# chsl/PLADE

Hardware: AMD Instinct MI355X
Metric: scan-pair registrations/sec, 1M-pt synthetic pairs (higher is better)
Workload: dtype f32

## Files before the change

### include/plade_hip.h

```cpp
#ifndef PLADE_HIP_H
#define PLADE_HIP_H
#include <stddef.h>
#include <stdint.h>
#ifdef __cplusplus
extern "C" {
#endif

#define PLADE_OK 0
#define PLADE_EINVAL (-1)
#define PLADE_EDEVICE (-2)
#define PLADE_ECAP (-3)
#define PLADE_EFAIL (-4)
#define PLADE_ELIMIT (-5)

#define PLADE_GROUP_MAX 8

typedef struct plade_ctx plade_ctx;
typedef struct plade_cloud plade_cloud;
typedef struct plade_comm plade_comm;

int plade_ctx_create(int device, plade_ctx **out);
void plade_ctx_destroy(plade_ctx *ctx);
const char *plade_last_error(const plade_ctx *ctx);
const char *plade_version(void);
// ... 101 lines not shown
int plade_estimate_normals(plade_ctx *ctx, const float *xyz, uint32_t n, uint32_t stride, int32_t k, const float *viewpoint,
                           float *pos_nrm_out, float *curvature_out, int32_t *nbr_out);
int plade_cloud_upload_xyz(plade_ctx *ctx, const float *xyz, uint32_t n, uint32_t stride, int32_t k, const float *viewpoint,
                           plade_cloud **out);

#define PLADE_ICP_TOO_FEW 1
#define PLADE_ICP_DEGENERATE 2
typedef struct plade_icp_params {
    double source_leaf;
    double max_dist;
    double min_dist;
    double eps_rotation;
    double eps_translation;
    int32_t max_iterations;
    int32_t min_correspondences;
} plade_icp_params;
typedef struct plade_icp_result {
    int32_t iterations;
    int32_t stages;
    int32_t converged;
    int32_t failure;
    uint32_t correspondences;
    uint32_t samples;
    double rmse, fitness;
    double final_dist;
} plade_icp_result;
void plade_icp_default_params(plade_icp_params *p);
int plade_refine_icp(plade_ctx *ctx, const float *tgt_pos_nrm, uint32_t n_t, const float *src_pos_nrm, uint32_t n_s,
                     const float *T_in16, const plade_icp_params *params, float *T_out16, plade_icp_result *result);
int plade_refine_icp_dev(plade_ctx *ctx, plade_cloud *tgt, plade_cloud *src, const float *T_in16, const plade_icp_params *params,
                         float *T_out16, plade_icp_result *result);
int plade_icp_linearize(plade_ctx *ctx, const float *tgt_pos_nrm, uint32_t n_t, const float *src_xyz, uint32_t n_s, uint32_t stride,
                        const double *T16, const double *center, float dist, int32_t *corr_out, double *moments_out);

typedef struct plade_gicp_params {
    double source_leaf;
    double max_dist;
    double min_dist;
    double eps_rotation;
    double eps_translation;
    int32_t max_iterations;
    int32_t min_correspondences;
    double epsilon;
} plade_gicp_params;
typedef struct plade_gicp_result {
    int32_t iterations;
    int32_t stages;
    int32_t converged;
    int32_t failure;
    uint32_t correspondences;
    uint32_t samples;
    double rmse, fitness;
    double final_dist;
    double cost;
} plade_gicp_result;
void plade_gicp_default_params(plade_gicp_params *p);
int plade_refine_gicp(plade_ctx *ctx, const float *tgt_pos_nrm, uint32_t n_t, const float *src_pos_nrm, uint32_t n_s,
                      const float *T_in16, const plade_gicp_params *params, float *T_out16, plade_gicp_result *result);
int plade_refine_gicp_dev(plade_ctx *ctx, plade_cloud *tgt, plade_cloud *src, const float *T_in16, const plade_gicp_params *params,
                          float *T_out16, plade_gicp_result *result);
int plade_gicp_linearize(plade_ctx *ctx, const float *tgt_pos_nrm, uint32_t n_t, const float *src_pos_nrm, uint32_t n_s,
                         const double *T16, const double *center, float dist, double epsilon, int32_t *corr_out, double *moments_out);

typedef struct plade_distance_summary {
    uint64_t n, count, plane_count;
    double fitness, rmse, mean, max, plane_rmse;
} plade_distance_summary;
int plade_cloud_distances(plade_ctx *ctx, const float *tgt_pos_nrm, uint32_t n_t, const float *src_xyz, uint32_t n_s,
                          uint32_t stride, const float *T16, float max_dist, int32_t *idx_out, float *d2_out,
                          float *plane_out, plade_distance_summary *summary);
int plade_cloud_distances_dev(plade_ctx *ctx, plade_cloud *tgt, plade_cloud *src, const float *T16, float max_dist,
                              int32_t *idx_out, float *d2_out, float *plane_out, plade_distance_summary *summary);

#define PLADE_OUTLIER_STATISTICAL 0
#define PLADE_OUTLIER_RADIUS 1
typedef struct plade_outlier_params {
    int32_t mode;
    int32_t k;
    double alpha;
    double radius;
    int32_t min_neighbours;
    int32_t reserved;
} plade_outlier_params;
typedef struct plade_outlier_summary {
    uint64_t n, kept;
    double mu, sigma, threshold;
} plade_outlier_summary;
void plade_outlier_default_params(plade_outlier_params *p);
int plade_filter_outliers(plade_ctx *ctx, const float *rows, uint32_t n, uint32_t stride, const plade_outlier_params *params,
                          uint8_t *keep_out, uint32_t *kept_index_out, float *rows_out, double *mean_dist_out, uint32_t *count_out,
                          plade_outlier_summary *summary);
int plade_cloud_filter_outliers_dev(plade_ctx *ctx, plade_cloud *cloud, const plade_outlier_params *params, plade_cloud **out,
                                    uint8_t *keep_out, uint32_t *kept_index_out, plade_outlier_summary *summary);

typedef struct plade_component_params {
    double radius;
    int32_t min_size;
    int32_t max_size;
    int32_t keep_largest;
    int32_t reserved;
} plade_component_params;
typedef struct plade_component_summary {
    uint64_t n, components, kept_components, kept;
    uint32_t largest;
    uint32_t reserved;
} plade_component_summary;
void plade_component_default_params(plade_component_params *p);
int plade_label_components(plade_ctx *ctx, const float *rows, uint32_t n, uint32_t stride, const plade_component_params *params,
                           int32_t *label_out, uint32_t *size_out, uint8_t *keep_out, uint32_t *kept_index_out, float *rows_out,
                           plade_component_summary *summary);
int plade_cloud_filter_components_dev(plade_ctx *ctx, plade_cloud *cloud, const plade_component_params *params, plade_cloud **out,
                                      int32_t *label_out, uint32_t *kept_index_out, plade_component_summary *summary);

typedef struct plade_smooth_params {
    double radius;
    int32_t min_neighbours;
    float viewpoint[3];
    int32_t reserved;
} plade_smooth_params;
typedef struct plade_smooth_summary {
    uint64_t n, fitted;
    double rms, max;
    uint32_t max_count;
    uint32_t reserved;
} plade_smooth_summary;
void plade_smooth_default_params(plade_smooth_params *p);
int plade_smooth_cloud(plade_ctx *ctx, const float *rows, uint32_t n, uint32_t stride, const plade_smooth_params *params,
                       float *out_xyz, float *out_normal, float *curvature_out, double *displacement_out, uint32_t *count_out,
                       uint8_t *fitted_out, double *moments_out, plade_smooth_summary *summary);
int plade_cloud_smooth_dev(plade_ctx *ctx, plade_cloud *cloud, const plade_smooth_params *params, int32_t use_fit_normals,
                           plade_cloud **out, plade_smooth_summary *summary);

typedef struct plade_merge_summary {
    uint64_t n_in, n_out, n_shared;
    uint32_t max_count;
    uint32_t reserved;
} plade_merge_summary;
int plade_merge_clouds(plade_ctx *ctx, uint32_t k, const float *const *clouds, const uint32_t *n, const float *T ,
                       float leaf, float *out_rows, uint32_t *out_count, uint32_t *out_mask, plade_merge_summary *summary);
int plade_merge_clouds_dev(plade_ctx *ctx, uint32_t k, plade_cloud *const *clouds, const float *T , float leaf,
                           plade_cloud **out, uint32_t *out_count, uint32_t *out_mask, plade_merge_summary *summary);
int plade_cloud_download(plade_ctx *ctx, const plade_cloud *cloud, float *rows, uint32_t capacity_rows, uint32_t *n);

int plade_dump_get(plade_ctx *ctx, const char *name, const void **ptr, int64_t *nbytes);
int plade_stats_get(plade_ctx *ctx, const char **names, const double **values, int32_t *count);
int plade_sort_pairs(plade_ctx *ctx, const void *keys, const uint32_t *vals, uint32_t n, int key_bytes, int bits,
                     void *keys_out, uint32_t *vals_out);
int plade_sort_segments(plade_ctx *ctx, const uint32_t *keys, const uint32_t *vals, const uint32_t *seg_off, uint32_t nseg, int bits,
                        uint32_t *keys_out, uint32_t *vals_out);

int plade_selftest_readback(plade_ctx *ctx, uint32_t n_ranges, uint32_t words, uint32_t *mismatches);

int plade_diag_launches(plade_ctx *ctx, uint32_t count, uint32_t blocks, uint32_t mbytes);
int plade_ply_read(const char *path, float **pos_nrm, uint64_t *n, char *err, size_t err_cap);
int plade_ply_read_points(const char *path, float **pos_nrm, uint64_t *n, int32_t *has_normals, char *err, size_t err_cap);
void plade_ply_free(float *pos_nrm);
int plade_diag_cluster_order(const float *sizes, uint32_t n, int32_t mode, int32_t depth_limit, int32_t *order);
int plade_diag_line_solver_host(int32_t kind, const float *a, const float *b, const float *c, const float *d, uint32_t n,
                                float *o1, float *o2, int32_t *ok);
int plade_kernel_time(plade_ctx *ctx, const char *which, int iters, double *avg_seconds,
                      double *algorithmic_bytes_per_launch);

#ifdef __cplusplus
}
#endif
#endif
```

### plade_amd/__init__.py

```python
import ctypes as C
import os
import numpy as np

_HERE = os.path.dirname(os.path.abspath(__file__))
LIB_PATH = os.path.join(_HERE, "libplade_hip.so")

PLADE_OK = 0
PLADE_EINVAL, PLADE_EDEVICE, PLADE_ECAP, PLADE_EFAIL, PLADE_ELIMIT = -1, -2, -3, -4, -5

ABI_SYMBOLS = [
    "plade_ctx_create", "plade_ctx_destroy", "plade_last_error", "plade_version", "plade_default_params",
    "plade_set_params", "plade_score_planes", "plade_extract_planes", "plade_match_descriptors",
    "plade_overlap_counts", "plade_average_spacing", "plade_voxel_downsample", "plade_registration_planes",
    "plade_registration", "plade_registration_minsupport", "plade_cloud_upload", "plade_cloud_free",
    "plade_registration_dev", "plade_dump_get", "plade_stats_get", "plade_kernel_time", "plade_plane_component",
    "plade_sort_pairs", "plade_host_pin", "plade_host_unpin", "plade_score_planes_subset", "plade_registration_next", "plade_cluster_transforms", "plade_device_synchronize", "plade_selftest_readback",
    "plade_registration_pairs", "plade_registration_pairs_dev", "plade_pair_ctx", "plade_set_candidate_shard", "plade_diag_launches", "plade_diag_cluster_order", "plade_diag_line_solver_host", "plade_sort_segments",
    "plade_closest_points", "plade_lines_meet", "plade_ply_read", "plade_ply_free",
    "plade_device_count", "plade_comm_unique_id", "plade_comm_create", "plade_comm_all_gather", "plade_comm_destroy", "plade_comm_last_error",
    "plade_set_candidate_shard_comm",
    "plade_estimate_normals", "plade_cloud_upload_xyz", "plade_ply_read_points",
    "plade_icp_default_params", "plade_refine_icp", "plade_refine_icp_dev", "plade_icp_linearize",
    "plade_cloud_distances", "plade_cloud_distances_dev",
    "plade_outlier_default_params", "plade_filter_outliers", "plade_cloud_filter_outliers_dev",
    "plade_merge_clouds", "plade_merge_clouds_dev", "plade_cloud_download",
    "plade_component_default_params", "plade_label_components", "plade_cloud_filter_components_dev",
    "plade_smooth_default_params", "plade_smooth_cloud", "plade_cloud_smooth_dev",
    "plade_gicp_default_params", "plade_refine_gicp", "plade_refine_gicp_dev", "plade_gicp_linearize",
]


class PladeError(RuntimeError):
    def __init__(self, code, msg):
        super().__init__(f"libplade_hip error {code}: {msg}")
        self.code = code


class Params(C.Structure):
    _fields_ = [("max_planes", C.c_int32), ("min_planes", C.c_int32), ("max_candidates", C.c_int32),
                ("init_min_support", C.c_int32), ("orient_normals", C.c_int32), ("dump", C.c_int32),
                ("ransac_seed", C.c_uint64), ("host_wait", C.c_int32), ("unoriented_normals", C.c_int32),
                ("ransac_topup", C.c_int32), ("match_window", C.c_int32), ("match_cell_budget", C.c_uint32),
                ("group_max_points", C.c_uint32), ("prepare_sides", C.c_int32), ("closest_point_mode", C.c_int32)]


class IcpParams(C.Structure):
    _fields_ = [("source_leaf", C.c_double), ("max_dist", C.c_double), ("min_dist", C.c_double), ("eps_rotation", C.c_double),
                ("eps_translation", C.c_double), ("max_iterations", C.c_int32), ("min_correspondences", C.c_int32)]


class IcpResult(C.Structure):
    _fields_ = [("iterations", C.c_int32), ("stages", C.c_int32), ("converged", C.c_int32), ("failure", C.c_int32),
                ("correspondences", C.c_uint32), ("samples", C.c_uint32), ("rmse", C.c_double), ("fitness", C.c_double),
                ("final_dist", C.c_double)]


class GicpParams(C.Structure):
    _fields_ = IcpParams._fields_ + [("epsilon", C.c_double)]


class GicpResult(C.Structure):
    _fields_ = IcpResult._fields_ + [("cost", C.c_double)]


class DistanceSummary(C.Structure):
    _fields_ = [("n", C.c_uint64), ("count", C.c_uint64), ("plane_count", C.c_uint64), ("fitness", C.c_double), ("rmse", C.c_double),
                ("mean", C.c_double), ("max", C.c_double), ("plane_rmse", C.c_double)]


class OutlierParams(C.Structure):
    _fields_ = [("mode", C.c_int32), ("k", C.c_int32), ("alpha", C.c_double), ("radius", C.c_double), ("min_neighbours", C.c_int32),
                ("reserved", C.c_int32)]


class OutlierSummary(C.Structure):
    _fields_ = [("n", C.c_uint64), ("kept", C.c_uint64), ("mu", C.c_double), ("sigma", C.c_double), ("threshold", C.c_double)]


class MergeSummary(C.Structure):
    _fields_ = [("n_in", C.c_uint64), ("n_out", C.c_uint64), ("n_shared", C.c_uint64), ("max_count", C.c_uint32),
                ("reserved", C.c_uint32)]


class ComponentParams(C.Structure):
    _fields_ = [("radius", C.c_double), ("min_size", C.c_int32), ("max_size", C.c_int32), ("keep_largest", C.c_int32),
                ("reserved", C.c_int32)]


class ComponentSummary(C.Structure):
    _fields_ = [("n", C.c_uint64), ("components", C.c_uint64), ("kept_components", C.c_uint64), ("kept", C.c_uint64),
                ("largest", C.c_uint32), ("reserved", C.c_uint32)]


class SmoothParams(C.Structure):
    _fields_ = [("radius", C.c_double), ("min_neighbours", C.c_int32), ("viewpoint", C.c_float * 3), ("reserved", C.c_int32)]


class SmoothSummary(C.Structure):
    _fields_ = [("n", C.c_uint64), ("fitted", C.c_uint64), ("rms", C.c_double), ("max", C.c_double), ("max_count", C.c_uint32),
                ("reserved", C.c_uint32)]


PLADE_OUTLIER_STATISTICAL, PLADE_OUTLIER_RADIUS = 0, 1
OUTLIER_MODES = {"statistical": PLADE_OUTLIER_STATISTICAL, "radius": PLADE_OUTLIER_RADIUS}

PLADE_ICP_TOO_FEW, PLADE_ICP_DEGENERATE = 1, 2
ICP_FAILURES = {0: None, PLADE_ICP_TOO_FEW: "too few correspondences", PLADE_ICP_DEGENERATE: "degenerate"}

EXCHANGE_FN = C.CFUNCTYPE(C.c_int, C.c_void_p, C.POINTER(C.c_int32), C.c_uint32, C.c_uint32, C.c_uint32)

_lib = None


def load_library(path=LIB_PATH):
    global _lib
    if _lib is not None:
        return _lib
    if not os.path.exists(path):
        raise FileNotFoundError(f"{path} is missing: build it with `make lib` or __graft_entry__.build(); "
                                "plade_amd has no CPU fallback")
    L = C.CDLL(path)
    p, f, i32, u32, u64 = C.c_void_p, C.c_float, C.c_int32, C.c_uint32, C.c_uint64
    def sig(name, argtypes=None, restype=None):
        fn = getattr(L, name, None)
        if fn is None:
            return
        if argtypes is not None:
            fn.argtypes = argtypes
        if restype is not None:
            fn.restype = restype

    sig("plade_version", restype=C.c_char_p)
    sig("plade_last_error", restype=C.c_char_p)
    sig("plade_last_error", argtypes=[p])
    sig("plade_device_synchronize", argtypes=[C.c_int])
    sig("plade_ctx_create", argtypes=[C.c_int, C.POINTER(p)])
    sig("plade_ctx_destroy", argtypes=[p])
    sig("plade_default_params", argtypes=[C.POINTER(Params)])
    sig("plade_set_params", argtypes=[p, C.POINTER(Params)])
    sig("plade_score_planes", argtypes=[p, p, p, u32, p, u32, f, f, p, p, u32])
    sig("plade_score_planes_subset", argtypes=[p, p, p, u32, p, u32, p, u32, f, f, p, p])
    sig("plade_extract_planes", argtypes=[p, p, u32, u32, f, f, f, f, p, p, p, u32, p])
    sig("plade_match_descriptors", argtypes=[p, p, u32, p, u32, f, p, p, p, u64, p])
    sig("plade_cluster_transforms", argtypes=[p, p, p, u32, f, f, p, p])
    sig("plade_overlap_counts", argtypes=[p, p, u32, p, u32, p, u32, p, f, f, p])
    sig("plade_average_spacing", argtypes=[p, p, u32, u32, u32, u32, p])
    sig("plade_voxel_downsample", argtypes=[p, p, u32, u32, f, p, p])
    sig("plade_registration_planes", argtypes=[p, p, u32, p, u32, p, p, p, u32, p, p, p, u32, p])
    sig("plade_registration", argtypes=[p, p, u32, p, u32, p])
    sig("plade_registration_next", argtypes=[p, p, u32, p, u32, p, u32, p, u32, p])
    sig("plade_registration_pairs", argtypes=[p, u32, p, p, p, p, u32, p, p, p, p, p, p])
    sig("plade_registration_pairs_dev", argtypes=[p, u32, p, p, p, p])
    sig("plade_pair_ctx", argtypes=[p, u32], restype=p)
    sig("plade_closest_points", argtypes=[p, i32, p, p, p, p, u32, p, p, p, p])
    sig("plade_lines_meet", argtypes=[p, i32, p, p, p, p, u32, p, p])
    sig("plade_diag_launches", argtypes=[p, u32, u32, u32])
    sig("plade_diag_cluster_order", argtypes=[p, u32, i32, i32, p])
    sig("plade_diag_line_solver_host", argtypes=[i32, p, p, p, p, u32, p, p, p])
    sig("plade_ply_read", argtypes=[C.c_char_p, C.POINTER(C.POINTER(C.c_float)), C.POINTER(u64), C.c_char_p, C.c_size_t])
    sig("plade_ply_free", argtypes=[C.POINTER(C.c_float)], restype=None)
    sig("plade_ply_read_points", argtypes=[C.c_char_p, C.POINTER(C.POINTER(C.c_float)), C.POINTER(u64), C.POINTER(i32), C.c_char_p,
                                           C.c_size_t])
    sig("plade_estimate_normals", argtypes=[p, p, u32, u32, i32, p, p, p, p])
    sig("plade_cloud_upload_xyz", argtypes=[p, p, u32, u32, i32, p, C.POINTER(p)])
    sig("plade_icp_default_params", argtypes=[C.POINTER(IcpParams)], restype=None)
    sig("plade_refine_icp", argtypes=[p, p, u32, p, u32, p, C.POINTER(IcpParams), p, C.POINTER(IcpResult)])
    sig("plade_refine_icp_dev", argtypes=[p, p, p, p, C.POINTER(IcpParams), p, C.POINTER(IcpResult)])
    sig("plade_icp_linearize", argtypes=[p, p, u32, p, u32, u32, p, p, f, p, p])
    sig("plade_gicp_default_params", argtypes=[C.POINTER(GicpParams)], restype=None)
    sig("plade_refine_gicp", argtypes=[p, p, u32, p, u32, p, C.POINTER(GicpParams), p, C.POINTER(GicpResult)])
    sig("plade_refine_gicp_dev", argtypes=[p, p, p, p, C.POINTER(GicpParams), p, C.POINTER(GicpResult)])
    sig("plade_gicp_linearize", argtypes=[p, p, u32, p, u32, p, p, f, C.c_double, p, p])
    sig("plade_cloud_distances", argtypes=[p, p, u32, p, u32, u32, p, f, p, p, p, C.POINTER(DistanceSummary)])
    sig("plade_cloud_distances_dev", argtypes=[p, p, p, p, f, p, p, p, C.POINTER(DistanceSummary)])
    sig("plade_outlier_default_params", argtypes=[C.POINTER(OutlierParams)], restype=None)
    sig("plade_filter_outliers", argtypes=[p, p, u32, u32, C.POINTER(OutlierParams), p, p, p, p, p, C.POINTER(OutlierSummary)])
    sig("plade_cloud_filter_outliers_dev", argtypes=[p, p, C.POINTER(OutlierParams), C.POINTER(p), p, p, C.POINTER(OutlierSummary)])
    sig("plade_merge_clouds", argtypes=[p, u32, p, p, p, f, p, p, p, C.POINTER(MergeSummary)])
    sig("plade_merge_clouds_dev", argtypes=[p, u32, p, p, f, C.POINTER(p), p, p, C.POINTER(MergeSummary)])
    sig("plade_cloud_download", argtypes=[p, p, p, u32, C.POINTER(u32)])
    sig("plade_component_default_params", argtypes=[C.POINTER(ComponentParams)], restype=None)
    sig("plade_label_components", argtypes=[p, p, u32, u32, C.POINTER(ComponentParams), p, p, p, p, p, C.POINTER(ComponentSummary)])
    sig("plade_cloud_filter_components_dev", argtypes=[p, p, C.POINTER(ComponentParams), C.POINTER(p), p, p, C.POINTER(ComponentSummary)])
    sig("plade_smooth_default_params", argtypes=[C.POINTER(SmoothParams)], restype=None)
    sig("plade_smooth_cloud", argtypes=[p, p, u32, u32, C.POINTER(SmoothParams), p, p, p, p, p, p, p, C.POINTER(SmoothSummary)])
    sig("plade_cloud_smooth_dev", argtypes=[p, p, C.POINTER(SmoothParams), i32, C.POINTER(p), C.POINTER(SmoothSummary)])
    sig("plade_sort_segments", argtypes=[p, p, p, p, u32, C.c_int, p, p])
    sig("plade_set_candidate_shard", argtypes=[p, u32, u32, u32, EXCHANGE_FN, p])
    sig("plade_registration_minsupport", argtypes=[p, p, u32, p, u32, i32, i32, p])
    sig("plade_cloud_upload", argtypes=[p, p, u32, C.POINTER(p)])
    sig("plade_cloud_free", argtypes=[p, p])
    sig("plade_registration_dev", argtypes=[p, p, p, p])
    sig("plade_dump_get", argtypes=[p, C.c_char_p, C.POINTER(p), C.POINTER(C.c_int64)])
    sig("plade_stats_get", argtypes=[p, C.POINTER(C.c_char_p), C.POINTER(C.POINTER(C.c_double)), C.POINTER(i32)])
    sig("plade_kernel_time", argtypes=[p, C.c_char_p, C.c_int, C.POINTER(C.c_double), C.POINTER(C.c_double)])
    sig("plade_plane_component", argtypes=[p, p, u32, p, p, p, u32, f, C.c_int, f, p, p, p, p])
    sig("plade_sort_pairs", argtypes=[p, p, p, u32, C.c_int, C.c_int, p, p])
    sig("plade_selftest_readback", argtypes=[p, u32, u32, C.POINTER(u32)])
    sig("plade_host_pin", argtypes=[p, p, C.c_size_t])
    sig("plade_host_unpin", argtypes=[p, p])
    _lib = L
    return L


def _f32(a):
    return np.ascontiguousarray(a, dtype=np.float32)


def _i32(a):
    return np.ascontiguousarray(a, dtype=np.int32)


def _ptr(a):
    return a.ctypes.data_as(C.c_void_p) if a is not None else None


DUMP_FIELDS = {
    "average_spacing": np.float32, "scale": np.float32,
    "tgt_ds": np.float32, "src_ds": np.float32, "tgt_bcenter": np.float32, "src_bcenter": np.float32,
    "tgt_radius": np.float64, "src_radius": np.float64,
    "tgt_plane_center_radius": np.float32, "src_plane_center_radius": np.float32,
    "tgt_plane_four": np.float32, "src_plane_four": np.float32,
    "tgt_plane_ds_offsets": np.int32, "src_plane_ds_offsets": np.int32,
    "tgt_plane_ds": np.float32, "src_plane_ds": np.float32,
    "tgt_lines": np.float32, "src_lines": np.float32,
    "tgt_desc": np.float32, "src_desc": np.float32,
    "match_offsets": np.int64, "match_nbr": np.int32, "match_dist2": np.float64,
    "initial_RT": np.float32, "cluster_sizes": np.int32, "cluster_seeds": np.int32,
    "plane_match_counts": np.int32, "pen_tested": np.int32, "pen_flags": np.int32,
    "candidates": np.float32, "candidate_centers": np.float32, "overlap_counts": np.int32,
    "scores": np.float32, "best_index": np.int32,
    "tgt_planes": np.float32, "tgt_plane_offsets": np.int32, "tgt_plane_idx": np.int32,
    "src_planes": np.float32, "src_plane_offsets": np.int32, "src_plane_idx": np.int32,
}


def device_synchronize(device=0):
    rc = load_library().plade_device_synchronize(int(device))
    if rc != 0:
        raise PladeError(rc, "plade_device_synchronize failed")


def default_params():
    prm = Params()
    load_library().plade_default_params(C.byref(prm))
    return prm


def icp_default_params():
    prm = IcpParams()
    load_library().plade_icp_default_params(C.byref(prm))
    return {k: getattr(prm, k) for k, _ in IcpParams._fields_}


def outlier_default_params():
    prm = OutlierParams()
    load_library().plade_outlier_default_params(C.byref(prm))
    return {k: getattr(prm, k) for k, _ in OutlierParams._fields_ if k != "reserved"}


def _outlier_params(mode, k, alpha, radius, min_neighbours):
    prm = OutlierParams()
    load_library().plade_outlier_default_params(C.byref(prm))
    if mode not in OUTLIER_MODES:
        raise ValueError(f"mode: 'statistical' or 'radius', got {mode!r}")
    prm.mode = OUTLIER_MODES[mode]
    if k is not None:
        prm.k = int(k)
    if alpha is not None:
        prm.alpha = float(alpha)
    if radius is not None:
        prm.radius = float(radius)
    if min_neighbours is not None:
        prm.min_neighbours = int(min_neighbours)
    return prm


def _outlier_info(summ, keep):
    info = {k: getattr(summ, k) for k, _ in OutlierSummary._fields_}
    info["keep"] = keep.view(np.bool_)
    return info


def component_default_params():
    prm = ComponentParams()
    load_library().plade_component_default_params(C.byref(prm))
    return {k: getattr(prm, k) for k, _ in ComponentParams._fields_ if k != "reserved"}


def _component_params(radius, min_size, max_size, keep_largest):
    prm = ComponentParams()
    load_library().plade_component_default_params(C.byref(prm))
    prm.radius = float(radius)
    prm.min_size, prm.max_size, prm.keep_largest = int(min_size), int(max_size), int(keep_largest)
    return prm


def _component_info(summ, label, size, keep):
    info = {k: getattr(summ, k) for k, _ in ComponentSummary._fields_ if k != "reserved"}
    info["label"] = label
    if size is not None:
        info["size"] = size[:summ.components].copy()
    if keep is not None:
        info["keep"] = keep.view(np.bool_)
    return info


def smooth_default_params():
    prm = SmoothParams()
# ... 267 lines not shown
                                                C.byref(npl)))
        p = npl.value
        return planes[:p].copy(), offs[: p + 1].copy(), idx[: offs[p]].copy()

    def match_descriptors(self, qry, tgt, radius=0.04):
        q = _f32(qry).reshape(-1, 8)
        t = _f32(tgt).reshape(-1, 8)
        off = np.zeros(len(q) + 1, np.int64)
        total = C.c_uint64()
        self._check(self.L.plade_match_descriptors(self.h, _ptr(q), len(q), _ptr(t), len(t), radius, _ptr(off), None,
                                                   None, 0, C.byref(total)))
        m = total.value
        nbr = np.zeros(max(m, 1), np.uint32)
        d2 = np.zeros(max(m, 1), np.float64)
        self._check(self.L.plade_match_descriptors(self.h, _ptr(q), len(q), _ptr(t), len(t), radius, _ptr(off),
                                                   _ptr(nbr), _ptr(d2), m, C.byref(total)))
        return off, nbr[:m].astype(np.int32), d2[:m]

    def cluster_transforms(self, t_xyz, euler, dist_threshold, angle_gate):
        t, e = _f32(t_xyz).reshape(-1, 3), _f32(euler).reshape(-1, 3)
        out = np.full(len(t), -1, np.int32)
        n = C.c_uint32()
        self._check(self.L.plade_cluster_transforms(self.h, _ptr(t), _ptr(e), len(t), dist_threshold, angle_gate, _ptr(out), C.byref(n)))
        return out, n.value

    def overlap_counts(self, src_ds, tgt_ds, T, centers, src_radius, inlier_dist):
        s, t = _f32(src_ds), _f32(tgt_ds)
        T = _f32(T).reshape(-1, 16)
        c = _f32(centers).reshape(-1, 3)
        counts = np.zeros(len(T), np.int32)
        self._check(self.L.plade_overlap_counts(self.h, _ptr(s), len(s), _ptr(t), len(t), _ptr(T), len(T), _ptr(c),
                                                src_radius, inlier_dist, _ptr(counts)))
        return counts

    def average_spacing(self, pts, k=6, samples=10000):
        a = _f32(pts)
        out = C.c_float()
        self._check(self.L.plade_average_spacing(self.h, _ptr(a), len(a), a.shape[1], k, samples, C.byref(out)))
        return np.float32(out.value)

    def voxel_downsample(self, pts, leaf):
        a = _f32(pts)
        out = np.zeros((len(a), 3), np.float32)
        n = C.c_uint32()
        self._check(self.L.plade_voxel_downsample(self.h, _ptr(a), len(a), a.shape[1], leaf, _ptr(out), C.byref(n)))
        return out[: n.value].copy()

    def registration_planes(self, tgt, src, tgt_planes, src_planes):
        tgt, src = _f32(tgt), _f32(src)
        tc, to, ti = _f32(tgt_planes[0]), _i32(tgt_planes[1]), _i32(tgt_planes[2])
        sc, so, si = _f32(src_planes[0]), _i32(src_planes[1]), _i32(src_planes[2])
        T = np.zeros((4, 4), np.float32)
        rc = self._check(self.L.plade_registration_planes(self.h, _ptr(tgt), len(tgt), _ptr(src), len(src), _ptr(tc),
                                                          _ptr(to), _ptr(ti), len(tc), _ptr(sc), _ptr(so), _ptr(si),
                                                          len(sc), _ptr(T)), allow=(PLADE_EFAIL,))
        return rc == 0, T

    def registration(self, tgt, src):
        tgt, src = _f32(tgt), _f32(src)
        self._check_cloud(tgt, "registration"); self._check_cloud(src, "registration")
        T = np.zeros((4, 4), np.float32)
        rc = self._check(self.L.plade_registration(self.h, _ptr(tgt), len(tgt), _ptr(src), len(src), _ptr(T)),
                         allow=(PLADE_EFAIL,))
        return rc == 0, T

    def registration_next(self, tgt, src, next_tgt=None, next_src=None):
        for a in (tgt, src, next_tgt, next_src):
            if a is not None:
                self._check_cloud(a, "registration_next")
        T = np.zeros((4, 4), np.float32)
        nt, ns = (next_tgt, next_src) if next_tgt is not None and next_src is not None else (None, None)
        self._announced = [(nt, ns)] if nt is not None else None
        rc = self._check(self.L.plade_registration_next(self.h, _ptr(tgt), len(tgt), _ptr(src), len(src), _ptr(nt),
                                                        len(nt) if nt is not None else 0, _ptr(ns),
                                                        len(ns) if ns is not None else 0, _ptr(T)), allow=(PLADE_EFAIL,))
        return rc == 0, T

    @staticmethod
    def _cloud_table(arrs):
        ptrs = (C.c_void_p * len(arrs))(*[a.ctypes.data for a in arrs])
        ns = (C.c_uint32 * len(arrs))(*[len(a) for a in arrs])
        return ptrs, ns

    @staticmethod
    def _check_cloud(a, what):
        if not isinstance(a, np.ndarray) or a.dtype != np.float32 or a.ndim != 2 or a.shape[1] != 6 or not a.flags["C_CONTIGUOUS"]:
            raise ValueError(f"{what}: a C-contiguous float32 array of shape (N, 6) is required, got "
                             f"{getattr(a, 'dtype', type(a))} {getattr(a, 'shape', '')}")
        if len(a) == 0:
            raise ValueError(f"{what}: empty cloud")

    def registration_pairs(self, pairs, next_pairs=None, raise_on_error=True):
        if not 1 <= len(pairs) <= 8 or (next_pairs and len(next_pairs) > 8):
            raise ValueError("registration_pairs: a group holds 1..8 pairs")
        for pr in list(pairs) + list(next_pairs or []):
            for a in pr[:2]:
                self._check_cloud(a, "registration_pairs")
        self._announced = [(p[0], p[1]) for p in next_pairs] if next_pairs else None
        k = len(pairs)
        tp, tn = self._cloud_table([p[0] for p in pairs])
        sp, sn = self._cloud_table([p[1] for p in pairs])
        nk = len(next_pairs) if next_pairs else 0
        if nk:
            ntp, ntn = self._cloud_table([p[0] for p in next_pairs])
            nsp, nsn = self._cloud_table([p[1] for p in next_pairs])
        else:
            ntp = ntn = nsp = nsn = None
        T = np.zeros((k, 4, 4), np.float32)
        st = np.zeros(k, np.int32)
        self._check(self.L.plade_registration_pairs(self.h, k, tp, tn, sp, sn, nk, ntp, ntn, nsp, nsn, _ptr(T), _ptr(st)))
        if not raise_on_error:
            return [(int(st[i]), T[i].copy()) for i in range(k)]
        for i in range(k):
            if st[i] not in (0, PLADE_EFAIL):
                raise PladeError(int(st[i]), self.pair_error(i))
        return [(bool(st[i] == 0), T[i].copy()) for i in range(k)]

    def registration_pairs_dev(self, clouds, raise_on_error=True):
        k = len(clouds)
        if not 1 <= k <= 8:
            raise ValueError("registration_pairs_dev: a group holds 1..8 pairs")
        tp = (C.c_void_p * k)(*[c[0].h.value for c in clouds])
        sp = (C.c_void_p * k)(*[c[1].h.value for c in clouds])
        T = np.zeros((k, 4, 4), np.float32)
        st = np.zeros(k, np.int32)
        self._check(self.L.plade_registration_pairs_dev(self.h, k, tp, sp, _ptr(T), _ptr(st)))
        if not raise_on_error:
            return [(int(st[i]), T[i].copy()) for i in range(k)]
        for i in range(k):
            if st[i] not in (0, PLADE_EFAIL):
                raise PladeError(int(st[i]), self.pair_error(i))
        return [(bool(st[i] == 0), T[i].copy()) for i in range(k)]

    def set_candidate_shard(self, rank, world, exchange=None, min_candidates=0):
        if world <= 1 or exchange is None:
            self._shard_cb = None
            self._check(self.L.plade_set_candidate_shard(self.h, 0, 1, 0, EXCHANGE_FN(0), None))
            return

        def cb(user, values, count, r, w):
            try:
                exchange(np.ctypeslib.as_array(values, shape=(count,)), int(r), int(w))
                return 0
            except Exception:
                import traceback
                traceback.print_exc()
                return -1
        self._shard_cb = EXCHANGE_FN(cb)
        self._check(self.L.plade_set_candidate_shard(self.h, int(rank), int(world), int(min_candidates), self._shard_cb, None))

    def diag_launches(self, count, blocks=1, mbytes=0):
        self._check(self.L.plade_diag_launches(self.h, int(count), int(blocks), int(mbytes)))

    def _pair_handle(self, index):
        h = self.L.plade_pair_ctx(self.h, int(index))
        if not h:
            raise PladeError(PLADE_EINVAL, f"no pair {index} on this context")
        return C.c_void_p(h)

    def pair_error(self, index):
        return self.L.plade_last_error(self._pair_handle(index)).decode(errors="replace")

    def registration_minsupport(self, tgt, src, ms_t, ms_s):
        tgt, src = _f32(tgt), _f32(src)
        T = np.zeros((4, 4), np.float32)
        rc = self._check(self.L.plade_registration_minsupport(self.h, _ptr(tgt), len(tgt), _ptr(src), len(src), ms_t,
                                                              ms_s, _ptr(T)), allow=(PLADE_EFAIL,))
        return rc == 0, T

    def upload(self, pos_nrm):
        return Cloud(self, pos_nrm)

    def estimate_normals(self, xyz, k=16, viewpoint=(0.0, 0.0, 0.0), curvature=False, neighbours=False):
        a, n, stride = _xyz_view(xyz)
        v = _viewpoint(viewpoint)
        out = np.empty((n, 6), np.float32)
        curv = np.empty(n, np.float32) if curvature else None
        nbr = np.empty((n, max(int(k), 0)), np.int32) if neighbours else None
        self._check(self.L.plade_estimate_normals(self.h, _ptr(a), n, stride, int(k), _ptr(v), _ptr(out), _ptr(curv), _ptr(nbr)))
        res = (out,) + ((curv,) if curvature else ()) + ((nbr,) if neighbours else ())
        return res[0] if len(res) == 1 else res

    def upload_xyz(self, xyz, k=16, viewpoint=(0.0, 0.0, 0.0)):
        a, n, stride = _xyz_view(xyz)
        v = _viewpoint(viewpoint)
        h = C.c_void_p()
        self._check(self.L.plade_cloud_upload_xyz(self.h, _ptr(a), n, stride, int(k), _ptr(v), C.byref(h)))
        return Cloud(self, None, handle=(n, h))

    def _refine(self, call, T, icp_params):
        T_in = _f32(T).reshape(4, 4).copy()
        prm = _icp_params(icp_params)
        T_out = np.zeros((4, 4), np.float32)
        res = IcpResult()
        rc = call(T_in, prm, T_out, res)
        info = _icp_info(res)
        if rc != 0:
            err = PladeError(rc, self.L.plade_last_error(self.h).decode(errors="replace"))
            err.info, err.T = info, T_out
            raise err
        return T_out, info

    def refine_icp(self, tgt, src, T, **icp_params):
        tgt, src = _f32(tgt), _f32(src)
        self._check_cloud(tgt, "refine_icp"); self._check_cloud(src, "refine_icp")
        return self._refine(lambda T_in, prm, T_out, res: self.L.plade_refine_icp(
            self.h, _ptr(tgt), len(tgt), _ptr(src), len(src), _ptr(T_in), C.byref(prm), _ptr(T_out), C.byref(res)), T, icp_params)

    def refine_icp_dev(self, tgt_cloud, src_cloud, T, **icp_params):
        return self._refine(lambda T_in, prm, T_out, res: self.L.plade_refine_icp_dev(
            self.h, tgt_cloud.h, src_cloud.h, _ptr(T_in), C.byref(prm), _ptr(T_out), C.byref(res)), T, icp_params)

    def icp_linearize(self, tgt, src_xyz, T, dist, center=None):
        tgt = _f32(tgt)
        self._check_cloud(tgt, "icp_linearize")
        a, n, stride = _xyz_view(src_xyz)
        T64 = np.ascontiguousarray(T, dtype=np.float64).reshape(4, 4)
        c64 = np.ascontiguousarray((0.0, 0.0, 0.0) if center is None else center, dtype=np.float64).reshape(3)
        corr = np.empty(n, np.int32)
        mom = np.zeros(29, np.float64)
        self._check(self.L.plade_icp_linearize(self.h, _ptr(tgt), len(tgt), _ptr(a), n, stride, _ptr(T64), _ptr(c64), float(dist),
                                               _ptr(corr), _ptr(mom)))
        return corr, mom

    def _refine_gicp(self, call, T, gicp_params):
        T_in = _f32(T).reshape(4, 4).copy()
        prm = _gicp_params(gicp_params)
        T_out = np.zeros((4, 4), np.float32)
        res = GicpResult()
        rc = call(T_in, prm, T_out, res)
        info = _gicp_info(res)
        if rc != 0:
            err = PladeError(rc, self.L.plade_last_error(self.h).decode(errors="replace"))
            err.info, err.T = info, T_out
            raise err
        return T_out, info

    def refine_gicp(self, tgt, src, T, **gicp_params):
        tgt, src = _f32(tgt), _f32(src)
        self._check_cloud(tgt, "refine_gicp"); self._check_cloud(src, "refine_gicp")
        return self._refine_gicp(lambda T_in, prm, T_out, res: self.L.plade_refine_gicp(
            self.h, _ptr(tgt), len(tgt), _ptr(src), len(src), _ptr(T_in), C.byref(prm), _ptr(T_out), C.byref(res)), T, gicp_params)

    def refine_gicp_dev(self, tgt_cloud, src_cloud, T, **gicp_params):
        return self._refine_gicp(lambda T_in, prm, T_out, res: self.L.plade_refine_gicp_dev(
            self.h, tgt_cloud.h, src_cloud.h, _ptr(T_in), C.byref(prm), _ptr(T_out), C.byref(res)), T, gicp_params)

    def gicp_linearize(self, tgt, src, T, dist, epsilon=0.0, center=None):
        tgt, src = _f32(tgt), _f32(src)
        self._check_cloud(tgt, "gicp_linearize"); self._check_cloud(src, "gicp_linearize")
        T64 = np.ascontiguousarray(T, dtype=np.float64).reshape(4, 4)
        c64 = np.ascontiguousarray((0.0, 0.0, 0.0) if center is None else center, dtype=np.float64).reshape(3)
        corr = np.empty(len(src), np.int32)
        mom = np.zeros(30, np.float64)
        self._check(self.L.plade_gicp_linearize(self.h, _ptr(tgt), len(tgt), _ptr(src), len(src), _ptr(T64), _ptr(c64), float(dist),
                                                float(epsilon), _ptr(corr), _ptr(mom)))
        return corr, mom

    def _distances(self, call, n, max_dist, T, per_point):
        T_in = None if T is None else _f32(T).reshape(4, 4).copy()
        idx = np.empty(n, np.int32) if per_point else None
        d2 = np.empty(n, np.float32) if per_point else None
        plane = np.empty(n, np.float32) if per_point else None
        summ = DistanceSummary()
        self._check(call(_ptr(T_in), float(max_dist), _ptr(idx), _ptr(d2), _ptr(plane), C.byref(summ)))
        return idx, d2, plane, {k: getattr(summ, k) for k, _ in DistanceSummary._fields_}

    def cloud_distances(self, tgt, src, max_dist, T=None, per_point=True):
        tgt = _f32(tgt)
        self._check_cloud(tgt, "cloud_distances")
        a, n, stride = _xyz_view(src)
        return self._distances(lambda T_in, d, i, d2, pl, summ: self.L.plade_cloud_distances(
            self.h, _ptr(tgt), len(tgt), _ptr(a), n, stride, T_in, d, i, d2, pl, summ), n, max_dist, T, per_point)

    def cloud_distances_dev(self, tgt_cloud, src_cloud, max_dist, T=None, per_point=True):
        return self._distances(lambda T_in, d, i, d2, pl, summ: self.L.plade_cloud_distances_dev(
            self.h, tgt_cloud.h, src_cloud.h, T_in, d, i, d2, pl, summ), src_cloud.n, max_dist, T, per_point)

    def evaluate_registration(self, tgt, src, T, max_dist):
        return self.cloud_distances(tgt, src, max_dist, T=T, per_point=False)[3]

    def remove_outliers(self, points, mode="statistical", k=None, alpha=None, radius=None, min_neighbours=None, per_point=True):
        a, n, stride = _xyz_view(points)
        prm = _outlier_params(mode, k, alpha, radius, min_neighbours)
        stat = prm.mode == PLADE_OUTLIER_STATISTICAL
        keep = np.zeros(n, np.uint8)
        kept = np.empty(n, np.uint32)
        rows = np.empty((n, stride), np.float32)
        mean = np.empty(n, np.float64) if per_point and stat else None
        count = np.empty(n, np.uint32) if per_point and not stat else None
        summ = OutlierSummary()
        self._check(self.L.plade_filter_outliers(self.h, _ptr(a), n, stride, C.byref(prm), _ptr(keep), _ptr(kept), _ptr(rows),
                                                 _ptr(mean), _ptr(count), C.byref(summ)))
        info = _outlier_info(summ, keep)
        if mean is not None:
            info["mean_dist"] = mean
        if count is not None:
            info["count"] = count
        return rows[:summ.kept].copy(), kept[:summ.kept].copy(), info

    def remove_outliers_dev(self, cloud, mode="statistical", k=None, alpha=None, radius=None, min_neighbours=None, info=False):
        prm = _outlier_params(mode, k, alpha, radius, min_neighbours)
        keep = np.zeros(cloud.n, np.uint8) if info else None
        kept = np.empty(cloud.n, np.uint32) if info else None
        summ = OutlierSummary()
        h = C.c_void_p()
# ... 150 lines not shown
```

### plade_amd/csrc/api.hip

```cpp
#include "ctx.h"
#include "components.h"
#include "distances.h"
#include "exact_sort.h"
#include "icp.h"
#include "merge.h"
#include "normals.h"
#include "outliers.h"
#include "pipeline.h"
#include "ransac.h"
#include "smooth.h"
#include "gicp.h"

using namespace plade;

extern "C" void plade_default_params(plade_params *p) {
    if (!p) return;
    p->max_planes = 40;
    p->min_planes = 10;
    p->max_candidates = 200;
    p->init_min_support = 10000;
    p->orient_normals = 0;
    p->dump = 0;
    p->ransac_seed = 0x9E3779B97F4A7C15ull;
    p->host_wait = 0;
    p->unoriented_normals = 0;
    p->ransac_topup = 1;
    p->match_window = 0;
    p->match_cell_budget = 0;
    p->group_max_points = 48000000u;
    p->prepare_sides = 0;
    p->closest_point_mode = 1;
}

namespace plade {
namespace {
struct Slab { char *base = nullptr; size_t used = 0; uint32_t live = 0; int device = 0; };
struct SmallPool {
    static constexpr size_t SLAB = 32u << 20, SMALL = 1u << 20, GRAN = 256;
    std::mutex m;
    std::vector<Slab> slabs;
    std::vector<size_t> empty;
    std::map<int, size_t> current;
    bool enabled = getenv("PLADE_EXP_NO_POOL") == nullptr;
    void *alloc(size_t bytes) {
        int dev = 0;
        HIP_TRY(hipGetDevice(&dev));
        const size_t need = (bytes + GRAN - 1) & ~(GRAN - 1);
        std::lock_guard<std::mutex> lk(m);
        auto it = current.find(dev);
        if (it == current.end() || slabs[it->second].used + need > SLAB) {
            size_t pick = (size_t)-1;
            if (it != current.end() && slabs[it->second].live == 0) pick = it->second;
            for (size_t q = 0; q < empty.size() && pick == (size_t)-1; ++q)
                if (slabs[empty[q]].device == dev) { pick = empty[q]; empty.erase(empty.begin() + (long)q); }
            if (pick == (size_t)-1) {
                Slab s;
                s.device = dev;
                HIP_TRY(hipMalloc((void **)&s.base, SLAB));
                slabs.push_back(s);
                pick = slabs.size() - 1;
            } else {
                HIP_TRY(hipDeviceSynchronize());
                slabs[pick].used = 0;
            }
            if (it != current.end() && it->second != pick && slabs[it->second].live == 0) empty.push_back(it->second);
            current[dev] = pick;
            it = current.find(dev);
        }
        Slab &s = slabs[it->second];
        void *p = s.base + s.used;
        s.used += need;
        ++s.live;
        return p;
    }
    bool release(void *p) {
        std::lock_guard<std::mutex> lk(m);
        for (size_t q = 0; q < slabs.size(); ++q) {
            Slab &s = slabs[q];
            if ((char *)p >= s.base && (char *)p < s.base + SLAB) {
                if (--s.live == 0) {
                    auto it = current.find(s.device);
                    if (it == current.end() || it->second != q) empty.push_back(q);
                }
                return true;
            }
        }
        return false;
    }
};
SmallPool &small_pool() { static SmallPool *p = new SmallPool; return *p; }
}

void *dev_alloc(size_t bytes) {
    const auto t0 = std::chrono::steady_clock::now();
    void *p = nullptr;
    SmallPool &sp = small_pool();
    if (sp.enabled && bytes <= SmallPool::SMALL) p = sp.alloc(bytes);
    else HIP_TRY(hipMalloc(&p, bytes));
    AllocStats &as = alloc_stats();
    as.calls += 1; as.bytes += bytes;
    as.nanos += (uint64_t)std::chrono::duration_cast<std::chrono::nanoseconds>(std::chrono::steady_clock::now() - t0).count();
    return p;
}
void dev_free(void *p) {
    if (!p) return;
    if (small_pool().release(p)) return;
    (void)hipFree(p);
}
}

extern "C" const char *plade_version(void) { return "plade-hip 0.1 (gfx950)"; }

extern "C" int plade_ctx_create(int device, plade_ctx **out) {
    if (!out) return PLADE_EINVAL;
    *out = nullptr;
    int count = 0;
    if (hipGetDeviceCount(&count) != hipSuccess || count <= 0 || device < 0 || device >= count) return PLADE_EDEVICE;
    if (hipSetDevice(device) != hipSuccess) return PLADE_EDEVICE;
    plade_ctx *c = new plade_ctx;
    c->device = device;
    plade_default_params(&c->params);
    if (hipStreamCreateWithFlags(&c->stream, hipStreamNonBlocking) != hipSuccess) { delete c; return PLADE_EDEVICE; }
    *out = c;
    return PLADE_OK;
}

extern "C" void plade_ctx_destroy(plade_ctx *ctx) {
    if (!ctx) return;
    if (ctx->aux) { plade_ctx_destroy(ctx->aux); ctx->aux = nullptr; }
    for (plade_ctx *&p : ctx->peers) if (p) { plade_ctx_destroy(p); p = nullptr; }
    if (ctx->ev_group) { (void)hipEventDestroy(ctx->ev_group); ctx->ev_group = nullptr; }
    (void)hipSetDevice(ctx->device);
    (void)hipStreamSynchronize(ctx->stream);
    if (ctx->reg_work) plade::registration_work_destroy(ctx->reg_work);
    if (ctx->ransac_work) plade::ransac_work_destroy(ctx->ransac_work);
    if (ctx->normals_work) plade::normals_work_destroy(ctx->normals_work);
    if (ctx->icp_work) plade::icp_work_destroy(ctx->icp_work);
    if (ctx->dist_work) plade::dist_work_destroy(ctx->dist_work);
    if (ctx->outlier_work) plade::outlier_work_destroy(ctx->outlier_work);
    if (ctx->merge_work) plade::merge_work_destroy(ctx->merge_work);
    if (ctx->component_work) plade::component_work_destroy(ctx->component_work);
    if (ctx->smooth_work) plade::smooth_work_destroy(ctx->smooth_work);
    if (ctx->gicp_work) plade::gicp_work_destroy(ctx->gicp_work);
    (void)hipStreamDestroy(ctx->stream);
    if (ctx->pf.stream) { (void)hipStreamSynchronize(ctx->pf.stream); (void)hipStreamDestroy(ctx->pf.stream); }
    delete ctx;
    if (getenv("PLADE_DEBUG_ALLOC")) {
        plade::AllocStats &as = plade::alloc_stats();
        fprintf(stderr, "[plade] device allocations so far: %llu calls, %.1f MB, %.1f ms in hipMalloc\n", (unsigned long long)as.calls.load(),
                as.bytes.load() / 1e6, as.nanos.load() / 1e6);
    }
}

extern "C" int plade_device_synchronize(int device) {
    if (hipSetDevice(device) != hipSuccess) return PLADE_EDEVICE;
    return hipDeviceSynchronize() == hipSuccess ? PLADE_OK : PLADE_EDEVICE;
}

extern "C" int plade_device_count(void) {
    int count = 0;
    return hipGetDeviceCount(&count) == hipSuccess && count > 0 ? count : 0;
}

extern "C" const char *plade_last_error(const plade_ctx *ctx) { return ctx ? ctx->last_error.c_str() : "null ctx"; }

extern "C" int plade_set_params(plade_ctx *ctx, const plade_params *p) {
    if (!ctx || !p) return PLADE_EINVAL;
    if (p->max_planes < 1 || p->min_planes < 0 || p->max_candidates < 1 || p->init_min_support < 1 || p->match_window < -1 || p->match_window > 1 ||
        p->closest_point_mode < 0 || p->closest_point_mode > 1) return PLADE_EINVAL;
    ctx->params = *p;
    return PLADE_OK;
}

extern "C" int plade_set_candidate_shard(plade_ctx *ctx, uint32_t rank, uint32_t world, uint32_t min_candidates, plade_exchange_fn exchange,
                                         void *user) {
    if (!ctx || (world > 1 && (rank >= world || !exchange))) return PLADE_EINVAL;
    ctx->shard.rank = world > 1 ? rank : 0; ctx->shard.world = world > 1 ? world : 1; ctx->shard.min_candidates = min_candidates;
    ctx->shard.exchange = world > 1 ? exchange : nullptr; ctx->shard.user = user;
    return PLADE_OK;
}

namespace plade {
__global__ void k_diag_load(const float4 *__restrict__ buf, size_t n16, float *__restrict__ sink) {
    float acc = 0.f;
    for (size_t i = (size_t)blockIdx.x * blockDim.x + threadIdx.x; i < n16; i += (size_t)gridDim.x * blockDim.x) { const float4 v = buf[i]; acc += v.x + v.y + v.z + v.w; }
    if (acc == 12345.678f) *sink = acc;
}
}
extern "C" int plade_diag_launches(plade_ctx *ctx, uint32_t count, uint32_t blocks, uint32_t mbytes) {
    return guarded(ctx, [&]() -> int {
        PLADE_REQUIRE(blocks >= 1 && blocks <= (1u << 20) && mbytes <= 4096, PLADE_EINVAL, "plade_diag_launches: bad argument");
        const size_t n16 = (size_t)mbytes << 16;
        float4 *buf = reinterpret_cast<float4 *>(ctx->scratch[0].ensure(n16 * 16 + 256));
        for (uint32_t i = 0; i < count; ++i)
            hipLaunchKernelGGL(plade::k_diag_load, dim3(blocks), dim3(256), 0, ctx->stream, buf, n16, reinterpret_cast<float *>(buf));
        HIP_TRY(hipGetLastError());
        ctx->sync();
        return PLADE_OK;
    });
}

extern "C" int plade_diag_cluster_order(const float *sizes, uint32_t n, int32_t mode, int32_t depth_limit, int32_t *order) {
    if ((n && (!sizes || !order)) || mode < 0 || mode > 3) return PLADE_EINVAL;
    try {
        std::vector<plade::exact_sort::Item> v(n);
        for (uint32_t i = 0; i < n; ++i) { v[i].index = (int)i; v[i].length = sizes[i]; }
        if (mode == 0) plade::exact_sort::sort_descending(v.data(), v.data() + n);
        else if (mode == 1) std::sort(v.begin(), v.end(), plade::exact_sort::greater);
        else if (mode == 2) plade::exact_sort::sort_descending<true>(v.data(), v.data() + n, depth_limit);
        else plade::exact_sort::sort_descending<false>(v.data(), v.data() + n, depth_limit);
        for (uint32_t i = 0; i < n; ++i) order[i] = v[i].index;
    } catch (...) { return PLADE_ELIMIT; }
    return PLADE_OK;
}

extern "C" int plade_dump_get(plade_ctx *ctx, const char *name, const void **ptr, int64_t *nbytes) {
    if (!ctx || !name || !ptr || !nbytes) return PLADE_EINVAL;
    auto it = ctx->dump.find(name);
    if (it == ctx->dump.end()) return PLADE_EINVAL;
    *ptr = it->second.data();
    *nbytes = (int64_t)it->second.size();
    return PLADE_OK;
}

extern "C" int plade_stats_get(plade_ctx *ctx, const char **names, const double **values, int32_t *count) {
    if (!ctx || !names || !values || !count) return PLADE_EINVAL;
    ctx->stats.joined.clear();
    for (auto &n : ctx->stats.names) { ctx->stats.joined += n; ctx->stats.joined += ";"; }
    *names = ctx->stats.joined.c_str();
    *values = ctx->stats.values.data();
    *count = (int32_t)ctx->stats.values.size();
    return PLADE_OK;
}
```

### plade_amd/csrc/cloud.hip

```cpp
#include "ctx.h"
#include "voxel.h"
#include <utility>

namespace plade {

namespace {
void shape_cloud(CloudDev &out, uint32_t n) {
    out.n = n;
    out.pitch = ((size_t)n + 3) & ~(size_t)3;
    out.soa.ensure(6 * out.pitch + 4);
    out.aos.ensure((size_t)n * 6 + 8);
}
struct FinishArgs {
    const float *aos[2 * PLADE_GROUP_MAX];
    float *soa[2 * PLADE_GROUP_MAX];
    uint32_t n[2 * PLADE_GROUP_MAX];
    uint32_t pitch[2 * PLADE_GROUP_MAX];
};
__global__ __launch_bounds__(256) void k_finish_uploads(const FinishArgs A, int *__restrict__ slots ) {
    __shared__ float s_lds[6][8];
    const int c = blockIdx.y;
    const uint32_t n = A.n[c];
    const float *__restrict__ aos = A.aos[c];
    float *__restrict__ soa = A.soa[c];
    const size_t pitch = A.pitch[c];
    int *out = slots + 8 * c;
    float mn[3] = {INFINITY, INFINITY, INFINITY}, mx[3] = {-INFINITY, -INFINITY, -INFINITY};
    bool bad = false;
    for (uint32_t i = blockIdx.x * blockDim.x + threadIdx.x; i < n; i += gridDim.x * blockDim.x) {
        const float2 *p = reinterpret_cast<const float2 *>(aos + 6 * (size_t)i);
        const float2 a = p[0], b = p[1], d = p[2];
        soa[i] = a.x; soa[pitch + i] = a.y; soa[2 * pitch + i] = b.x;
        soa[3 * pitch + i] = b.y; soa[4 * pitch + i] = d.x; soa[5 * pitch + i] = d.y;
        const float v[3] = {a.x, a.y, b.x};
        for (int k = 0; k < 3; ++k) {
            bad = bad || !(fabsf(v[k]) <= FLT_MAX);
            mn[k] = fminf(mn[k], v[k]);
            mx[k] = fmaxf(mx[k], v[k]);
        }
    }
    if (bad) out[6] = 1;
    block_minmax_commit<3>(mn, mx, out, s_lds);
}

void finish_uploads(plade_ctx *ctx, CloudDev *const clouds[], int count) {
    plade_ctx::Prefetch &P = ctx->pf;
    constexpr int MAXC = 2 * PLADE_GROUP_MAX;
    if (!P.h.p) {
        int *h = P.h.ensure(8 * MAXC + 8 * MAXC);
        for (int i = 0; i < MAXC; ++i) bbox_init_pattern(h + 8 * i);
        P.d.ensure(8 * MAXC);
    }
    PLADE_REQUIRE(count >= 1 && count <= MAXC, PLADE_EINVAL, "finish_uploads: too many clouds");
    FinishArgs A;
    memset(&A, 0, sizeof(A));
    uint32_t n_max = 0;
    for (int i = 0; i < count; ++i) {
        A.aos[i] = clouds[i]->aos.p; A.soa[i] = clouds[i]->soa.p; A.n[i] = clouds[i]->n; A.pitch[i] = (uint32_t)clouds[i]->pitch;
        n_max = std::max(n_max, clouds[i]->n);
    }
    int *h_out = P.h.p + 8 * MAXC;
    HIP_TRY(hipMemcpyAsync(P.d.p, P.h.p, 32 * (size_t)count, hipMemcpyHostToDevice, ctx->stream));
    if (n_max) hipLaunchKernelGGL(k_finish_uploads, dim3(std::min(cdiv(n_max, 1024), 1024u), count), dim3(256), 0, ctx->stream, A, P.d.p);
    HIP_TRY(hipMemcpyAsync(h_out, P.d.p, 32 * (size_t)count, hipMemcpyDeviceToHost, ctx->stream));
    HIP_TRY(hipGetLastError());
    ctx->sync();
    for (int i = 0; i < count; ++i) bbox_decode(h_out + 8 * i, clouds[i]->bbmin, clouds[i]->bbmax);
}
}

void cloud_upload(plade_ctx *ctx, const float *pos_nrm, uint32_t n, CloudDev &out) {
    shape_cloud(out, n);
    if (n == 0) return;
    HIP_TRY(hipMemcpyAsync(out.aos.p, pos_nrm, (size_t)n * 24, hipMemcpyHostToDevice, ctx->stream));
    ctx->sync();
    CloudDev *cl[1] = {&out};
    finish_uploads(ctx, cl, 1);
}

void cloud_shape(CloudDev &out, uint32_t n) { shape_cloud(out, n); }

void cloud_finish_device(plade_ctx *ctx, CloudDev &out) {
    CloudDev *cl[1] = {&out};
    finish_uploads(ctx, cl, 1);
}

void cloud_upload_many(plade_ctx *ctx, int count, const float *const ptr[], const uint32_t n[], CloudDev *const out[]) {
    PLADE_REQUIRE(count >= 1 && count <= 2 * PLADE_GROUP_MAX, PLADE_EINVAL, "cloud_upload_many: too many clouds");
    for (int i = 0; i < count; ++i) {
        shape_cloud(*out[i], n[i]);
        if (n[i]) HIP_TRY(hipMemcpyAsync(out[i]->aos.p, ptr[i], (size_t)n[i] * 24, hipMemcpyHostToDevice, ctx->stream));
    }
    ctx->sync();
    CloudDev *cl[2 * PLADE_GROUP_MAX];
    for (int i = 0; i < count; ++i) cl[i] = out[i];
    finish_uploads(ctx, cl, count);
}

void cloud_upload_pair(plade_ctx *ctx, const float *tgt, uint32_t n_t, CloudDev &out_t, const float *src, uint32_t n_s, CloudDev &out_s) {
    const float *ptr[2] = {tgt, src};
    const uint32_t n[2] = {n_t, n_s};
    CloudDev *out[2] = {&out_t, &out_s};
    cloud_upload_many(ctx, 2, ptr, n, out);
}

namespace {
void swap_clouds(CloudDev &a, CloudDev &b) {
    std::swap(a.n, b.n);
    std::swap(a.pitch, b.pitch);
    a.soa.swap(b.soa);
    a.aos.swap(b.aos);
    for (int k = 0; k < 3; ++k) { std::swap(a.bbmin[k], b.bbmin[k]); std::swap(a.bbmax[k], b.bbmax[k]); }
}
}

void cloud_drop_prefetch(plade_ctx *ctx) {
    plade_ctx::Prefetch &P = ctx->pf;
    if (!P.valid) return;
    P.valid = false;
    if (P.stream) ctx->sync(P.stream);
}

void cloud_prefetch(plade_ctx *ctx, int count, const float *const ptr[], const uint32_t n[]) {
    plade_ctx::Prefetch &P = ctx->pf;
    cloud_drop_prefetch(ctx);
    if (count < 2 || count > 2 * PLADE_GROUP_MAX || (count & 1)) return;
    for (int i = 0; i < count; ++i) if (!ptr[i] || !n[i]) return;
    if (!P.stream) HIP_TRY(hipStreamCreateWithFlags(&P.stream, hipStreamNonBlocking));
    for (int i = 0; i < count; ++i) {
        shape_cloud(P.cl[i], n[i]);
        HIP_TRY(hipMemcpyAsync(P.cl[i].aos.p, ptr[i], (size_t)n[i] * 24, hipMemcpyHostToDevice, P.stream));
        P.ptr[i] = ptr[i]; P.n[i] = n[i];
    }
    P.count = count;
    P.valid = true;
}

bool cloud_take_prefetched(plade_ctx *ctx, int count, const float *const ptr[], const uint32_t n[], CloudDev *const out[]) {
    plade_ctx::Prefetch &P = ctx->pf;
    if (!P.valid) return false;
    P.valid = false;
    ctx->sync(P.stream);
    if (P.count != count) return false;
    for (int i = 0; i < count; ++i) if (P.ptr[i] != ptr[i] || P.n[i] != n[i]) return false;
    CloudDev *cl[2 * PLADE_GROUP_MAX];
    for (int i = 0; i < count; ++i) { swap_clouds(*out[i], P.cl[i]); cl[i] = out[i]; }
    finish_uploads(ctx, cl, count);
    return true;
}

}
```

### plade_amd/csrc/k_voxel.hip

```cpp
#include "voxel.h"
#include "overlap.h"
#include "prims.h"

namespace plade {

template <class K>
__global__ void k_voxel_keys(const float *__restrict__ xyz, uint32_t stride, const float *__restrict__ sx,
                             const float *__restrict__ sy, const float *__restrict__ sz, int soa_indexed,
                             const uint32_t *__restrict__ item_point, const uint32_t *__restrict__ item_group,
                             uint32_t n_items, float inv, int lminx, int lminy, int lminz, int bx, int by, int bz,
                             K *__restrict__ keys, uint32_t *__restrict__ vals, uint32_t n_group_offsets) {
    __shared__ uint32_t s_off[1026];
    if (n_group_offsets) {
        for (uint32_t q = threadIdx.x; q < n_group_offsets; q += blockDim.x) s_off[q] = item_group[q];
        __syncthreads();
    }
    uint32_t i = blockIdx.x * blockDim.x + threadIdx.x;
    if (i >= n_items) return;
    float x, y, z;
    if (!item_point && sx) { x = sx[i]; y = sy[i]; z = sz[i]; }
    else if (soa_indexed) { const uint32_t p = item_point[i]; x = sx[p]; y = sy[p]; z = sz[p]; }
    else {
        const uint32_t p = item_point ? item_point[i] : i;
        x = xyz[(size_t)p * stride]; y = xyz[(size_t)p * stride + 1]; z = xyz[(size_t)p * stride + 2];
// ... 93 lines not shown
    }
    __syncthreads();
    uint32_t rank = s_excl + woff + incl - sum;
#pragma unroll
    for (int q = 0; q < VR_I; ++q)
        if (fl & (1u << q)) {
            heads[rank] = first + q;
            seg_group[rank] = (uint32_t)(k[q + 1] >> group_shift);
            ++rank;
        }
    if ((uint64_t)tile * VR_TILE + VR_TILE >= n && tid == VR_T - 1) *n_seg = s_excl + agg;
#pragma unroll
    for (int q = 0; q < VR_I; ++q) {
        const uint32_t j = tile * VR_TILE + q * VR_T + tid;
        if (j < n) { ox[j] = gx[q]; oy[j] = gy[q]; oz[j] = gz[q]; }
    }
}

__global__ __launch_bounds__(128) void k_voxel_centroids(const float *__restrict__ sx, const float *__restrict__ sy,
                                                         const float *__restrict__ sz, const uint32_t *__restrict__ heads,
                                                         const uint32_t *__restrict__ seg_group, const uint32_t *__restrict__ n_seg_p,
                                                         uint32_t n_items, uint32_t n_groups, float *__restrict__ out_xyz,
                                                         uint32_t *__restrict__ group_offsets, float *__restrict__ out_soa) {
    const uint32_t n_seg = *n_seg_p;
    if (blockIdx.x == 0)
        for (uint32_t g = threadIdx.x; g <= n_groups; g += blockDim.x) {
            uint32_t lo = 0, hi = n_seg;
            while (lo < hi) { const uint32_t mid = (lo + hi) >> 1; if (seg_group[mid] < g) lo = mid + 1; else hi = mid; }
            group_offsets[g] = lo;
        }
    constexpr uint32_t CH = 2048;
    __shared__ float s_x[CH], s_y[CH], s_z[CH];
    __shared__ uint32_t s_span[2];
    const uint32_t s0 = blockIdx.x * blockDim.x;
    if (s0 >= n_seg) return;
    const uint32_t s = s0 + threadIdx.x;
    const bool live = s < n_seg;
    const uint32_t b = live ? heads[s] : 0u, e = live ? ((s + 1 < n_seg) ? heads[s + 1] : n_items) : 0u;
    if (threadIdx.x == 0) s_span[0] = b;
    if (s == min(n_seg, s0 + (uint32_t)blockDim.x) - 1) s_span[1] = e;
    __syncthreads();
    const uint32_t span_b = s_span[0], span_e = s_span[1];
    float ax = 0.f, ay = 0.f, az = 0.f;
    for (uint32_t c0 = span_b; c0 < span_e; c0 += CH) {
        const uint32_t c1 = min(span_e, c0 + CH);
        for (uint32_t j = c0 + threadIdx.x; j < c1; j += blockDim.x) { s_x[j - c0] = sx[j]; s_y[j - c0] = sy[j]; s_z[j - c0] = sz[j]; }
        __syncthreads();
        const uint32_t jb = max(b, c0), je = min(e, c1);
        for (uint32_t j = jb; j < je; ++j) { ax += s_x[j - c0]; ay += s_y[j - c0]; az += s_z[j - c0]; }
        __syncthreads();
    }
    if (!live) return;
    const float cnt = (float)(e - b);
    const float cx = ax / cnt, cy = ay / cnt, cz = az / cnt;
    out_xyz[3 * (size_t)s] = cx;
    out_xyz[3 * (size_t)s + 1] = cy;
    out_xyz[3 * (size_t)s + 2] = cz;
    if (out_soa) { out_soa[s] = cx; out_soa[(size_t)n_seg + s] = cy; out_soa[2 * (size_t)n_seg + s] = cz; }
}

void VoxelWork::enqueue(plade_ctx *ctx, const float *d_xyz, uint32_t stride, const float *d_soa_x, const float *d_soa_y,
                        const float *d_soa_z, const uint32_t *d_item_point, const uint32_t *d_item_group, uint32_t n_items,
                        uint32_t n_groups, float leaf, const float bbox_min[3], const float bbox_max[3], bool soa_indexed,
                        bool groups_are_offsets, float *d_out_soa) {
    PLADE_REQUIRE(!soa_indexed || (d_item_point && d_soa_x), PLADE_EINVAL, "voxel: an indexed SoA source needs items and planes");
    n_out = 0;
    n_pending = 0;
    PLADE_REQUIRE(leaf > 0.f, PLADE_EINVAL, "voxel: leaf must be positive");
    PLADE_REQUIRE(n_groups >= 1 && n_groups <= 1024, PLADE_ELIMIT, "voxel: at most 1024 point groups");
    if (n_items == 0) {
        group_offsets.ensure((size_t)n_groups + 2);
        count.ensure(4);
        out_xyz.ensure(4);
        ctx->fill_async(group_offsets.p, 0, ((size_t)n_groups + 2) * 4);
        ctx->fill_async(count.p, 0, 4);
        return;
    }
    const float inv = 1.f / leaf;
    const int lmin[3] = {(int)floorf(bbox_min[0] * inv), (int)floorf(bbox_min[1] * inv), (int)floorf(bbox_min[2] * inv)};
    const int lmax[3] = {(int)floorf(bbox_max[0] * inv), (int)floorf(bbox_max[1] * inv), (int)floorf(bbox_max[2] * inv)};
    for (int k = 0; k < 3; ++k)
        PLADE_REQUIRE((int64_t)lmax[k] - lmin[k] < (1 << 18), PLADE_ELIMIT,
                      "voxel: more than 2^18 leaves along one axis (PCL would refuse this leaf size too)");
    {
        int64_t dx = (int64_t)((bbox_max[0] - bbox_min[0]) * inv) + 1, dy = (int64_t)((bbox_max[1] - bbox_min[1]) * inv) + 1,
                dz = (int64_t)((bbox_max[2] - bbox_min[2]) * inv) + 1;
        PLADE_REQUIRE(dx * dy * dz <= (int64_t)INT32_MAX, PLADE_ELIMIT, "voxel: leaf size too small for the data extent");
    }
    auto bits_for = [](int64_t range) { int b = 1; while (((int64_t)1 << b) <= range) ++b; return b; };
    const int bx = bits_for((int64_t)lmax[0] - lmin[0]), by = bits_for((int64_t)lmax[1] - lmin[1]), bz = bits_for((int64_t)lmax[2] - lmin[2]);
    keys.ensure(n_items); keys2.ensure(n_items); vals.ensure(n_items); vals2.ensure(n_items);
    sorted_xyz.ensure(3 * (size_t)n_items + 4);
    heads.ensure((size_t)n_items + 1);
    seg_group.ensure((size_t)n_items + 1);
    out_xyz.ensure((size_t)n_items * 3 + 4);
    group_offsets.ensure((size_t)n_groups + 2);
    count.ensure(4);
    const unsigned nb = cdiv(n_items, 256);
    int gbits = 0;
    while ((1u << gbits) < n_groups) ++gbits;
    const int key_bits = bx + by + bz + gbits;
    const bool narrow = key_bits <= 31;
    uint32_t *k32 = reinterpret_cast<uint32_t *>(keys.p), *k32b = reinterpret_cast<uint32_t *>(keys2.p);
    if (narrow)
        launch_raw(ctx, k_voxel_keys<uint32_t>, dim3(nb), dim3(256), 0, d_xyz, stride, d_soa_x, d_soa_y, d_soa_z, soa_indexed ? 1 : 0,
                           d_item_point, d_item_group, n_items, inv, lmin[0], lmin[1], lmin[2], bx, by, bz, k32, vals.p,
                           groups_are_offsets ? n_groups + 1 : 0u);
    else
        launch_raw(ctx, k_voxel_keys<uint64_t>, dim3(nb), dim3(256), 0, d_xyz, stride, d_soa_x, d_soa_y, d_soa_z, soa_indexed ? 1 : 0,
                           d_item_point, d_item_group, n_items, inv, lmin[0], lmin[1], lmin[2], bx, by, bz, keys.p, vals.p,
                           groups_are_offsets ? n_groups + 1 : 0u);
    if (narrow) sort_pairs_u32(ctx, k32, k32b, vals.p, vals2.p, n_items, key_bits);
    else sort_pairs_u64(ctx, keys.p, keys2.p, vals.p, vals2.p, n_items, key_bits);
    const ScanTicket t = scan_ticket(ctx, n_items, VR_TILE);
    float *ox = sorted_xyz.p, *oy = ox + n_items, *oz = oy + n_items;
    if (narrow)
        launch_raw(ctx, k_voxel_runs<uint32_t>, dim3(t.tiles), dim3(VR_T), 0, k32b, vals2.p, n_items, d_xyz, stride,
                           soa_indexed ? d_soa_x : nullptr, soa_indexed ? d_soa_y : nullptr, soa_indexed ? d_soa_z : nullptr, d_item_point,
                           bx + by + bz, t.state, t.ticket, t.base, t.gen, heads.p, seg_group.p, count.p, ox, oy, oz);
    else
        launch_raw(ctx, k_voxel_runs<uint64_t>, dim3(t.tiles), dim3(VR_T), 0, keys2.p, vals2.p, n_items, d_xyz, stride,
                           soa_indexed ? d_soa_x : nullptr, soa_indexed ? d_soa_y : nullptr, soa_indexed ? d_soa_z : nullptr, d_item_point,
                           bx + by + bz, t.state, t.ticket, t.base, t.gen, heads.p, seg_group.p, count.p, ox, oy, oz);
    launch_raw(ctx, k_voxel_centroids, dim3(cdiv(n_items, 128)), dim3(128), 0, ox, oy, oz, heads.p, seg_group.p,
                       count.p, n_items, n_groups, out_xyz.p, group_offsets.p, d_out_soa);
    HIP_TRY(hipGetLastError());
    ctx->d2h(&n_pending_host, count.p, 4);
    n_pending = 1;
}

void VoxelWork::adopt_batch(plade_ctx *ctx) {
    n_out = 0;
    ctx->d2h(&n_pending_host, count.p, 4);
    n_pending = 1;
}

constexpr int VB_MAX = 16;
struct VBCloud {
    const float *sx, *sy, *sz, *aos;
    const uint32_t *items;
    const uint32_t *offs;
    uint32_t n, P;
    float inv;
    int lminx, lminy, lminz, bx, by, gshift;
    float *out_xyz, *out_soa;
    uint32_t *count, *group_offsets;
};
struct VBArgs {
    VBCloud c[VB_MAX];
    uint32_t ncl;
    uint32_t start[VB_MAX + 1];
    uint32_t tile_start[VB_MAX + 1];
    uint32_t cblk_start[VB_MAX + 1];
    uint32_t total;
};
__device__ __forceinline__ uint32_t vb_find(const uint32_t *start, uint32_t ncl, uint32_t v) {
    uint32_t g = 0;
#pragma unroll
    for (int q = 1; q < VB_MAX; ++q) g += (q < (int)ncl && v >= start[q]) ? 1u : 0u;
    return g;
}

__global__ void k_vb_keys(const VBArgs A, uint32_t *__restrict__ keys, uint32_t *__restrict__ vals) {
    const uint32_t t = blockIdx.x * blockDim.x + threadIdx.x;
    if (t >= A.total) return;
    const uint32_t g = vb_find(A.start, A.ncl, t);
    const VBCloud &C = A.c[g];
    const uint32_t i = t - A.start[g];
    const uint32_t p = C.items ? C.items[i] : i;
    const float x = C.sx[p], y = C.sy[p], z = C.sz[p];
    const uint32_t lx = (uint32_t)((int)floorf(x * C.inv) - C.lminx);
    const uint32_t ly = (uint32_t)((int)floorf(y * C.inv) - C.lminy);
    const uint32_t lz = (uint32_t)((int)floorf(z * C.inv) - C.lminz);
    uint32_t grp = 0;
    if (C.offs) {
        uint32_t lo = 0, hi = C.P;
        while (lo < hi) { const uint32_t mid = (lo + hi + 1) >> 1; if (C.offs[mid] <= i) lo = mid; else hi = mid - 1; }
        grp = lo;
    }
    keys[t] = (grp << C.gshift) | (lz << (C.bx + C.by)) | (ly << C.bx) | lx;
    vals[t] = i;
}

__global__ __launch_bounds__(VR_T) void k_vb_runs(const VBArgs A, const uint32_t *__restrict__ keys_all, const uint32_t *__restrict__ vals_all,
                                                  uint64_t *__restrict__ state_all, uint32_t *__restrict__ ticket, uint32_t base, uint32_t gen,
                                                  uint32_t *__restrict__ heads_all, uint32_t *__restrict__ seg_group_all,
                                                  float *__restrict__ sorted_all) {
    __shared__ uint32_t s_tile, s_w[VR_T / 64], s_excl;
    const int tid = threadIdx.x, lane = tid & 63, wave = tid >> 6;
    if (tid == 0) s_tile = atomicAdd(ticket, 1u) - base;
    __syncthreads();
    const uint32_t gtile = s_tile;
    const uint32_t g = vb_find(A.tile_start, A.ncl, gtile);
    const VBCloud &C = A.c[g];
    const uint32_t tile = gtile - A.tile_start[g], n = C.n;
    const uint32_t *__restrict__ keys = keys_all + A.start[g];
    const uint32_t *__restrict__ vals = vals_all + A.start[g];
    uint64_t *__restrict__ state = state_all + A.tile_start[g];
    uint32_t *__restrict__ heads = heads_all + A.start[g] + g;
    uint32_t *__restrict__ seg_group = seg_group_all + A.start[g] + g;
    float *__restrict__ ox = sorted_all + A.start[g], *__restrict__ oy = ox + A.total, *__restrict__ oz = oy + A.total;
    float gx[VR_I], gy[VR_I], gz[VR_I];
#pragma unroll
    for (int q = 0; q < VR_I; ++q) {
        const uint32_t j = tile * VR_TILE + q * VR_T + tid;
        if (j < n) {
            if (C.items) { const uint32_t p = C.items[vals[j]]; gx[q] = C.sx[p]; gy[q] = C.sy[p]; gz[q] = C.sz[p]; }
            else { const float *r = C.aos + (size_t)vals[j] * 6; gx[q] = r[0]; gy[q] = r[1]; gz[q] = r[2]; }
        }
    }
    const uint32_t first = tile * VR_TILE + tid * VR_I;
    uint32_t k[VR_I + 1];
    k[0] = (first > 0 && first <= n) ? keys[first - 1] : 0xffffffffu;
#pragma unroll
    for (int q = 0; q < VR_I; ++q) k[q + 1] = first + q < n ? keys[first + q] : 0xffffffffu;
    uint32_t fl = 0, sum = 0;
#pragma unroll
    for (int q = 0; q < VR_I; ++q) {
        const bool head = first + q < n && (first + q == 0 || k[q + 1] != k[q]);
        fl |= (head ? 1u : 0u) << q;
        sum += head;
    }
    uint32_t incl = sum;
#pragma unroll
    for (int d = 1; d < 64; d <<= 1) {
        const uint32_t o = __shfl_up(incl, d, 64);
        if (lane >= d) incl += o;
    }
    if (lane == 63) s_w[wave] = incl;
    __syncthreads();
    uint32_t agg = 0, woff = 0;
    for (int w = 0; w < VR_T / 64; ++w) { if (w < wave) woff += s_w[w]; agg += s_w[w]; }
    const uint64_t tag = (uint64_t)gen << 34;
    if (wave == 0) {
        if (lane == 0)
            __hip_atomic_store(state + tile, tag | (tile == 0 ? VR_PREFIX : VR_AGG) | agg, __ATOMIC_RELAXED, __HIP_MEMORY_SCOPE_AGENT);
        uint32_t excl = 0;
        if (tile > 0) {
            int t = (int)tile - 1;
            for (;;) {
                const int idx = t - lane;
                uint64_t st = tag | VR_PREFIX;
                if (idx >= 0) st = __hip_atomic_load(state + idx, __ATOMIC_RELAXED, __HIP_MEMORY_SCOPE_AGENT);
                const bool ready = (st >> 34) == gen && (st & VR_STATUS) != 0ull;
                const unsigned long long not_ready = __ballot(!ready), is_prefix = __ballot(ready && (st & VR_PREFIX));
                const int first_bad = not_ready ? __ffsll((long long)not_ready) - 1 : 64;
                const int first_pre = is_prefix ? __ffsll((long long)is_prefix) - 1 : 64;
                const int take = first_pre < first_bad ? first_pre + 1 : first_bad;
                uint32_t part = lane < take ? (uint32_t)st : 0u;
                for (int d = 32; d >= 1; d >>= 1) part += __shfl_xor(part, d, 64);
                excl += part;
                if (first_pre < first_bad) break;
                t -= take;
            }
            if (lane == 0)
                __hip_atomic_store(state + tile, tag | VR_PREFIX | (uint64_t)(excl + agg), __ATOMIC_RELAXED, __HIP_MEMORY_SCOPE_AGENT);
        }
        if (lane == 0) s_excl = excl;
    }
    __syncthreads();
    uint32_t rank = s_excl + woff + incl - sum;
#pragma unroll
    for (int q = 0; q < VR_I; ++q)
        if (fl & (1u << q)) { heads[rank] = first + q; seg_group[rank] = k[q + 1] >> C.gshift; ++rank; }
    if ((uint64_t)tile * VR_TILE + VR_TILE >= n && tid == VR_T - 1) *C.count = s_excl + agg;
#pragma unroll
    for (int q = 0; q < VR_I; ++q) {
        const uint32_t j = tile * VR_TILE + q * VR_T + tid;
        if (j < n) { ox[j] = gx[q]; oy[j] = gy[q]; oz[j] = gz[q]; }
    }
}

__global__ __launch_bounds__(128) void k_vb_centroids(const VBArgs A, const uint32_t *__restrict__ heads_all,
                                                      const uint32_t *__restrict__ seg_group_all, const float *__restrict__ sorted_all) {
    constexpr uint32_t CH = 2048;
    __shared__ float s_x[CH], s_y[CH], s_z[CH];
    __shared__ uint32_t s_span[2];
    const uint32_t g = vb_find(A.cblk_start, A.ncl, blockIdx.x);
    const VBCloud &C = A.c[g];
    const uint32_t blk = blockIdx.x - A.cblk_start[g];
    const uint32_t n_seg = *C.count, n_items = C.n;
    const uint32_t *__restrict__ heads = heads_all + A.start[g] + g;
    if (blk == 0) {
        const uint32_t *__restrict__ seg_group = seg_group_all + A.start[g] + g;
        for (uint32_t q = threadIdx.x; q <= C.P; q += blockDim.x) {
            uint32_t lo = 0, hi = n_seg;
            while (lo < hi) { const uint32_t mid = (lo + hi) >> 1; if (seg_group[mid] < q) lo = mid + 1; else hi = mid; }
            C.group_offsets[q] = lo;
        }
    }
    const float *__restrict__ sx = sorted_all + A.start[g], *__restrict__ sy = sx + A.total, *__restrict__ sz = sy + A.total;
    const uint32_t s0 = blk * blockDim.x;
    if (s0 >= n_seg) return;
    const uint32_t s = s0 + threadIdx.x;
    const bool live = s < n_seg;
    const uint32_t b = live ? heads[s] : 0u, e = live ? ((s + 1 < n_seg) ? heads[s + 1] : n_items) : 0u;
    if (threadIdx.x == 0) s_span[0] = b;
    if (s == min(n_seg, s0 + (uint32_t)blockDim.x) - 1) s_span[1] = e;
    __syncthreads();
    const uint32_t span_b = s_span[0], span_e = s_span[1];
    float ax = 0.f, ay = 0.f, az = 0.f;
    for (uint32_t c0 = span_b; c0 < span_e; c0 += CH) {
        const uint32_t c1 = min(span_e, c0 + CH);
        for (uint32_t j = c0 + threadIdx.x; j < c1; j += blockDim.x) { s_x[j - c0] = sx[j]; s_y[j - c0] = sy[j]; s_z[j - c0] = sz[j]; }
        __syncthreads();
        const uint32_t jb = max(b, c0), je = min(e, c1);
        for (uint32_t j = jb; j < je; ++j) { ax += s_x[j - c0]; ay += s_y[j - c0]; az += s_z[j - c0]; }
        __syncthreads();
    }
    if (!live) return;
    const float cnt = (float)(e - b);
    const float cx = ax / cnt, cy = ay / cnt, cz = az / cnt;
    C.out_xyz[3 * (size_t)s] = cx; C.out_xyz[3 * (size_t)s + 1] = cy; C.out_xyz[3 * (size_t)s + 2] = cz;
    if (C.out_soa) { C.out_soa[s] = cx; C.out_soa[(size_t)n_seg + s] = cy; C.out_soa[2 * (size_t)n_seg + s] = cz; }
}

bool voxel_whole_batch(plade_ctx *ctx, VoxBatchWork &B, int count, const VoxBatchItem *items) {
    if (count < 1 || count > VB_MAX) return false;
    VBArgs A;
    memset(&A, 0, sizeof(A));
    A.ncl = (uint32_t)count;
    auto bits_for = [](int64_t range) { int b = 1; while (((int64_t)1 << b) <= range) ++b; return b; };
    int max_bits = 1;
    uint64_t total = 0;
    size_t n_offs = 0;
    for (int g = 0; g < count; ++g) {
        const VoxBatchItem &it = items[g];
        if (it.n == 0 || !(it.leaf > 0.f) || !it.work || (!it.items && !it.out_soa)) return false;
        if (it.items && (!it.offsets_host || it.P < 1 || it.P > 1024)) return false;
        const float inv = 1.f / it.leaf;
        const int lmin[3] = {(int)floorf(it.bbmin[0] * inv), (int)floorf(it.bbmin[1] * inv), (int)floorf(it.bbmin[2] * inv)};
        const int lmax[3] = {(int)floorf(it.bbmax[0] * inv), (int)floorf(it.bbmax[1] * inv), (int)floorf(it.bbmax[2] * inv)};
        for (int k = 0; k < 3; ++k)
            if ((int64_t)lmax[k] - lmin[k] >= (1 << 18)) return false;
        const int64_t dx = (int64_t)((it.bbmax[0] - it.bbmin[0]) * inv) + 1, dy = (int64_t)((it.bbmax[1] - it.bbmin[1]) * inv) + 1,
                      dz = (int64_t)((it.bbmax[2] - it.bbmin[2]) * inv) + 1;
        if (dx * dy * dz > (int64_t)INT32_MAX) return false;
        const int bx = bits_for((int64_t)lmax[0] - lmin[0]), by = bits_for((int64_t)lmax[1] - lmin[1]), bz = bits_for((int64_t)lmax[2] - lmin[2]);
        int gbits = 0;
        if (it.items) while ((1u << gbits) < it.P) ++gbits;
        if (bx + by + bz + gbits > 31) return false;
        max_bits = std::max(max_bits, bx + by + bz + gbits);
        n_offs += it.items ? it.P + 1 : 0;
        VBCloud &C = A.c[g];
        C.sx = it.sx; C.sy = it.sy; C.sz = it.sz; C.aos = it.aos; C.n = it.n; C.inv = inv;
        C.items = it.items; C.P = it.items ? it.P : 1u; C.gshift = bx + by + bz;
        C.lminx = lmin[0]; C.lminy = lmin[1]; C.lminz = lmin[2]; C.bx = bx; C.by = by;
        VoxelWork &w = *it.work;
        w.out_xyz.ensure((size_t)it.n * 3 + 4);
        w.group_offsets.ensure((size_t)C.P + 2);
        w.count.ensure(4);
        w.n_out = 0; w.n_pending = 0;
        C.out_xyz = w.out_xyz.p; C.out_soa = it.out_soa; C.count = w.count.p; C.group_offsets = w.group_offsets.p;
        A.start[g + 1] = A.start[g] + it.n;
        A.tile_start[g + 1] = A.tile_start[g] + cdiv(it.n, VR_TILE);
        A.cblk_start[g + 1] = A.cblk_start[g] + cdiv(it.n, 128);
        total += it.n;
    }
    if (total >= (1ull << 30)) return false;
    for (int g = count; g < VB_MAX; ++g) { A.c[g] = A.c[0]; A.start[g + 1] = A.start[g]; A.tile_start[g + 1] = A.tile_start[g]; A.cblk_start[g + 1] = A.cblk_start[g]; }
    A.total = (uint32_t)total;
    B.keys.ensure(total); B.keys2.ensure(total); B.vals.ensure(total); B.vals2.ensure(total);
    B.heads.ensure(total + VB_MAX + 1);
    B.seg_group.ensure(total + VB_MAX + 1);
    B.sorted_xyz.ensure(3 * total + 4);
    hipStream_t st = ctx->stream;
    if (n_offs) {
        B.offs.ensure(n_offs + 4);
        std::vector<uint32_t> h(n_offs);
        size_t o = 0;
        for (int g = 0; g < count; ++g) {
            if (!items[g].items) continue;
            for (uint32_t q = 0; q <= items[g].P; ++q) h[o + q] = (uint32_t)items[g].offsets_host[q];
            A.c[g].offs = B.offs.p + o;
            o += items[g].P + 1;
        }
        const bool staged = ctx->h2d(B.offs.p, h.data(), 4 * n_offs);
        if (!staged) ctx->sync();
    }
    hipLaunchKernelGGL(k_vb_keys, dim3(cdiv(total, 256)), dim3(256), 0, st, A, B.keys.p, B.vals.p);
    radix_sort_segments_u32(ctx, B.keys.p, B.keys2.p, B.vals.p, B.vals2.p, A.start, count, max_bits);
    const uint32_t tiles = A.tile_start[count];
    const ScanTicket t = scan_ticket(ctx, (size_t)tiles * VR_TILE, VR_TILE);
    hipLaunchKernelGGL(k_vb_runs, dim3(tiles), dim3(VR_T), 0, st, A, B.keys2.p, B.vals2.p, t.state, t.ticket, t.base, t.gen, B.heads.p,
                       B.seg_group.p, B.sorted_xyz.p);
    hipLaunchKernelGGL(k_vb_centroids, dim3(A.cblk_start[count]), dim3(128), 0, st, A, B.heads.p, B.seg_group.p, B.sorted_xyz.p);
    HIP_TRY(hipGetLastError());
    return true;
}

uint32_t VoxelWork::finish(plade_ctx *ctx) {
    if (!n_pending) return n_out;
    ctx->sync();
    n_pending = 0;
    n_out = n_pending_host;
    return n_out;
}

uint32_t VoxelWork::run(plade_ctx *ctx, const float *d_xyz, uint32_t stride, const uint32_t *d_item_point,
                        const uint32_t *d_item_group, uint32_t n_items, uint32_t n_groups, float leaf,
                        const float bbox_min[3], const float bbox_max[3]) {
    enqueue(ctx, d_xyz, stride, nullptr, nullptr, nullptr, d_item_point, d_item_group, n_items, n_groups, leaf, bbox_min, bbox_max);
    return finish(ctx);
}

constexpr int SP_K = 8;

struct SpGrid { float mnx, mny, mnz, inv, cell; int dx, dy, dz; };

__global__ __launch_bounds__(256) void k_knn_grid(const float4 *__restrict__ pts, const uint32_t *__restrict__ cstart,
                                                  const uint32_t *__restrict__ cend, SpGrid g,
                                                  const float *__restrict__ aos, uint32_t stride_f, uint32_t n,
                                                  uint32_t step, uint32_t nq, int k, double *__restrict__ avg_out,
                                                  uint32_t *__restrict__ nbs_out) {
    const int lane = threadIdx.x & 63;
    const uint32_t qi = blockIdx.x * (blockDim.x >> 6) + (threadIdx.x >> 6);
    if (qi >= nq) return;
    const uint32_t pi = min(n - 1, qi * step);
    const f3 q(aos[(size_t)pi * stride_f], aos[(size_t)pi * stride_f + 1], aos[(size_t)pi * stride_f + 2]);
    const int cx = min(max((int)floorf((q.x - g.mnx) * g.inv), 0), g.dx - 1);
    const int cy = min(max((int)floorf((q.y - g.mny) * g.inv), 0), g.dy - 1);
    const int cz = min(max((int)floorf((q.z - g.mnz) * g.inv), 0), g.dz - 1);
    float best[SP_K];
#pragma unroll
    for (int b = 0; b < SP_K; ++b) best[b] = INFINITY;
    float kth[SP_K];
    int found = 0;
    const int max_ring = max(g.dx, max(g.dy, g.dz));
    for (int ring = 0; ring <= max_ring; ++ring) {
        const int w = 2 * ring + 1;
        for (int t = lane; t < w * w * w; t += 64) {
            const int ddx = t % w - ring, ddy = (t / w) % w - ring, ddz = t / (w * w) - ring;
            if (max(abs(ddx), max(abs(ddy), abs(ddz))) != ring) continue;
            const int x = cx + ddx, y = cy + ddy, z = cz + ddz;
            if (x < 0 || y < 0 || z < 0 || x >= g.dx || y >= g.dy || z >= g.dz) continue;
            const int c = x + g.dx * (y + g.dy * z);
            for (uint32_t j = cstart[c]; j < cend[c]; ++j) {
                const float4 p4 = pts[j];
                float d = flann_d2(q, f3(p4.x, p4.y, p4.z));
                if (d < best[SP_K - 1]) {
#pragma unroll
                    for (int b = 0; b < SP_K; ++b)
                        if (d < best[b]) { float tt = best[b]; best[b] = d; d = tt; }
                }
            }
        }
        int head = 0;
        found = 0;
        for (int r = 0; r < k; ++r) {
            float v = INFINITY;
#pragma unroll
            for (int b = 0; b < SP_K; ++b) if (b == head) v = best[b];
            float mv = v;
            int ml = lane;
            for (int d = 32; d >= 1; d >>= 1) {
                const float ov = __shfl_xor(mv, d, 64);
                const int ol = __shfl_xor(ml, d, 64);
                if (ov < mv || (ov == mv && ol < ml)) { mv = ov; ml = ol; }
            }
            if (mv == INFINITY) break;
            if (lane == ml) ++head;
            kth[r] = mv;
            ++found;
        }
        const float bound = (float)ring * g.cell * 0.999f;
        if (found == k && kth[k - 1] < bound * bound) break;
    }
    if (lane == 0) {
        double avg = 0.0;
        for (int r = 1; r < found; ++r) avg += (double)sqrtf(kth[r]);
        avg_out[qi] = avg;
        nbs_out[qi] = (uint32_t)found;
    }
}

__global__ __launch_bounds__(256) void k_grid_occupancy(const uint32_t *__restrict__ keys, uint32_t n, uint32_t run,
                                                        uint32_t *__restrict__ flag) {
    __shared__ uint32_t s_c[4];
    uint32_t c = 0;
    bool dense = false;
    for (uint32_t i = blockIdx.x * blockDim.x + threadIdx.x; i < n; i += gridDim.x * blockDim.x) {
        const uint32_t k = keys[i];
        if (i + run < n && k == keys[i + run]) dense = true;
        c += (i == 0 || k != keys[i - 1]) ? 1u : 0u;
    }
    for (int d = 32; d >= 1; d >>= 1) c += __shfl_xor(c, d, 64);
    if (__ballot(dense) && (threadIdx.x & 63) == 0) flag[0] = 1u;
    if ((threadIdx.x & 63) == 0) s_c[threadIdx.x >> 6] = c;
    __syncthreads();
    if (threadIdx.x == 0) {
        const uint32_t t = s_c[0] + s_c[1] + s_c[2] + s_c[3];
        if (t) atomicAdd(&flag[1], t);
    }
}

float average_spacing_dev(plade_ctx *ctx, const float *d_aos, uint32_t stride_f, uint32_t n, const float *bbmin,
                          const float *bbmax, int k, uint32_t samples, TargetGrid &grid) {
    PLADE_REQUIRE(k >= 1 && k <= SP_K, PLADE_ELIMIT, "average_spacing: k must be in [1, 8]");
    if (n == 0) return 0.f;
    size_t step = 1;
    if (n > samples) step = n / samples;
    const uint32_t nq = (uint32_t)((n + step - 1) / step);
    const double ex = std::max(1e-9, (double)bbmax[0] - bbmin[0]), ey = std::max(1e-9, (double)bbmax[1] - bbmin[1]),
                 ez = std::max(1e-9, (double)bbmax[2] - bbmin[2]);
    const double area = 2 * (ex * ey + ey * ez + ex * ez);
    float cell = (float)(2.0 * std::sqrt(area / (double)n));
    if (!(cell > 0.f)) cell = 1.f;
    int last_dir = 0;
    for (int attempt = 0; attempt < 12; ++attempt) {
        grid.build(ctx, d_aos, n, stride_f, cell, bbmin, bbmax);
        if (n <= 256) break;
        uint32_t *d_flag = reinterpret_cast<uint32_t *>(ctx->scratch[2].ensure(64));
        ctx->fill_async(d_flag, 0, 8);
        launch_raw(ctx, k_grid_occupancy, dim3(std::min(cdiv(n, 1024), 512u)), dim3(256), 0, grid.keys2.p, n, 256u, d_flag);
        uint32_t occ[2] = {0, 0};
        ctx->d2h(occ, d_flag, 8);
        ctx->sync();
        const float built = 1.f / grid.gp.inv;
        int dir = 0;
        if (occ[0] && built <= cell * 1.01f) dir = -1;
        else if (!occ[0] && (double)occ[1] > 0.5 * (double)n) dir = +1;
        if (dir == 0 || dir == -last_dir) break;
        cell = dir < 0 ? built * 0.25f : built * 4.f;
        last_dir = dir;
    }
    SpGrid g{grid.gp.mnx, grid.gp.mny, grid.gp.mnz, grid.gp.inv, 1.f / grid.gp.inv, grid.gp.dx, grid.gp.dy, grid.gp.dz};
    double *d_avg = reinterpret_cast<double *>(ctx->scratch[1].ensure((size_t)nq * 8 + 8));
    uint32_t *d_nbs = reinterpret_cast<uint32_t *>(ctx->scratch[2].ensure((size_t)nq * 4 + 8));
    ctx->ev_begin("knn_spacing", 12.0 * n);
    launch_raw(ctx, k_knn_grid, dim3(cdiv(nq, 4)), dim3(256), 0, grid.sorted.p, grid.cell_start.p,
                       grid.cell_end.p, g, d_aos, stride_f, n, (uint32_t)step, nq, k, d_avg, d_nbs);
    ctx->ev_end();
    HIP_TRY(hipGetLastError());
// ... 117 lines not shown
```

### plade_amd/csrc/radix_sort.hip

```cpp
#include "prims.h"

#if defined(__HIP_DEVICE_COMPILE__) && !defined(__gfx950__)
#error "radix_sort.hip is written for gfx950 (160 KB LDS per workgroup); build with --offload-arch=gfx950"
#endif

namespace plade {

namespace {

constexpr int RS_THREADS = 512;
constexpr int RS_WAVES = RS_THREADS / 64;
constexpr int RS_HBLOCKS = 128;
constexpr int RS_MAXP = 8;
constexpr int RS_LOOK = 8;
constexpr uint32_t RS_VALID = 1u << 31, RS_VALUE = RS_VALID - 1;
constexpr int RS_MAXSEG = 16;
constexpr uint32_t RS_GH_SEG = RS_MAXP * 512;
struct RSSegs {
    uint32_t nseg;
    uint32_t off[RS_MAXSEG + 1];
    uint32_t tile_start[RS_MAXSEG + 1];
    uint32_t sup_start[RS_MAXSEG + 1];
};
__device__ __forceinline__ uint32_t seg_of_tile(const RSSegs &S, uint32_t tile) {
// ... 91 lines not shown
    for (int r = 0; r < RS_IPT; ++r) {
        const bool ok = base + r * 64 + lane < n;
        const uint32_t d = digit_of<DB>(key[r], shift);
        unsigned long long peers = __ballot(ok);
#pragma unroll
        for (int b = 0; b < DB; ++b) {
            const unsigned long long m = __ballot((d >> b) & 1u);
            peers &= ((d >> b) & 1u) ? m : ~m;
        }
        const uint32_t c = ok ? cnt[d] : 0u;
        rank[r] = c + (uint32_t)__popcll(peers & lt);
        if (ok && (peers & lt) == 0ull) cnt[d] = c + (uint32_t)__popcll(peers);
    }
    __syncthreads();

    const uint32_t d = tid & (NB - 1);
    uint32_t tile_count = 0;
    if (owner)
        for (int w = 0; w < RS_WAVES; ++w) { const uint32_t c = s_cnt[w][d]; s_cnt[w][d] = tile_count; tile_count += c; }
    if (owner) {
        __hip_atomic_store(look + (size_t)tile * NB + d, RS_VALID | tile_count, __ATOMIC_RELAXED, __HIP_MEMORY_SCOPE_AGENT);
        __hip_atomic_fetch_add(sup + (size_t)(tile >> st_shift) * NB + d, RS_SUP_ONE | (unsigned long long)tile_count, __ATOMIC_RELAXED,
                               __HIP_MEMORY_SCOPE_AGENT);
    }
    uint32_t inc_g = total, inc_t = tile_count;
    for (int o = 1; o < 64; o <<= 1) {
        const uint32_t a = __shfl_up(inc_g, o, 64), b = __shfl_up(inc_t, o, 64);
        if (lane >= o) { inc_g += a; inc_t += b; }
    }
    __shared__ uint32_t s_wg[NB / 64], s_wt[NB / 64];
    if (owner && lane == 63) { s_wg[wave] = inc_g; s_wt[wave] = inc_t; }
    __syncthreads();
    if (owner) {
        uint32_t off_g = 0, off_t = 0;
        for (int w = 0; w < wave; ++w) { off_g += s_wg[w]; off_t += s_wt[w]; }
        const uint32_t gbase = off_g + inc_g - total;
        const uint32_t tstart = off_t + inc_t - tile_count;
        uint32_t excl = 0;
        const uint32_t my_sup = tile >> st_shift, st_tiles = 1u << st_shift;
        for (uint32_t s0 = 0; s0 < my_sup; s0 += RS_LOOK) {
            unsigned long long w[RS_LOOK];
#pragma unroll
            for (int j = 0; j < RS_LOOK; ++j)
                w[j] = (s0 + j < my_sup) ? __hip_atomic_load(sup + (size_t)(s0 + j) * NB + d, __ATOMIC_RELAXED, __HIP_MEMORY_SCOPE_AGENT)
                                         : ((unsigned long long)st_tiles << 40);
#pragma unroll
            for (int j = 0; j < RS_LOOK; ++j) {
                while ((w[j] >> 40) != st_tiles) w[j] = __hip_atomic_load(sup + (size_t)(s0 + j) * NB + d, __ATOMIC_RELAXED, __HIP_MEMORY_SCOPE_AGENT);
                excl += (uint32_t)(w[j] & RS_SUP_VALUE);
            }
        }
        for (uint32_t t0 = my_sup << st_shift; t0 < tile; t0 += RS_LOOK) {
            uint32_t w[RS_LOOK];
#pragma unroll
            for (int j = 0; j < RS_LOOK; ++j)
                w[j] = (t0 + j < tile) ? __hip_atomic_load(look + (size_t)(t0 + j) * NB + d, __ATOMIC_RELAXED, __HIP_MEMORY_SCOPE_AGENT) : RS_VALID;
#pragma unroll
            for (int j = 0; j < RS_LOOK; ++j) {
                while (!(w[j] & RS_VALID)) w[j] = __hip_atomic_load(look + (size_t)(t0 + j) * NB + d, __ATOMIC_RELAXED, __HIP_MEMORY_SCOPE_AGENT);
                excl += w[j] & RS_VALUE;
            }
        }
        s_start[d] = tstart;
        s_dest[d] = gbase + excl;
    }
    __syncthreads();

#pragma unroll
    for (int r = 0; r < RS_IPT; ++r) {
        if (base + r * 64 + lane < n) {
            const uint32_t dg = digit_of<DB>(key[r], shift);
            const uint32_t pos = s_start[dg] + s_cnt[wave][dg] + rank[r];
            s_keys[pos] = key[r];
            s_vals[pos] = val[r];
        }
    }
    __syncthreads();
    const uint32_t in_tile = min((uint32_t)RS_TILE, n - tile * RS_TILE);
    for (uint32_t pos = tid; pos < in_tile; pos += RS_THREADS) {
        const K k = s_keys[pos];
        const uint32_t dg = digit_of<DB>(k, shift);
        const uint32_t out = s_dest[dg] + (pos - s_start[dg]);
        kout[out] = k;
        vout[out] = s_vals[pos];
    }
}

template <class K, int DB, int RS_IPT>
void radix_sort_run_ipt(plade_ctx *ctx, const K *ki, K *ko, const uint32_t *vi, uint32_t *vo, const uint32_t *seg_off, int nseg, int passes) {
    constexpr int NB = 1 << DB;
    constexpr int RS_TILE = RS_THREADS * RS_IPT;
    const size_t n = seg_off[nseg] - seg_off[0];
    if (n == 0) return;
    RSSegs S;
    memset(&S, 0, sizeof(S));
    S.nseg = (uint32_t)nseg;
    uint32_t max_tiles = 1;
    for (int q = 0; q <= RS_MAXSEG; ++q) S.off[q] = seg_off[std::min(q, nseg)] - seg_off[0];
    for (int q = 0; q < nseg; ++q) {
        const uint32_t t = cdiv(S.off[q + 1] - S.off[q], RS_TILE);
        S.tile_start[q + 1] = S.tile_start[q] + t;
        max_tiles = std::max(max_tiles, t);
    }
    for (int q = nseg; q < RS_MAXSEG; ++q) S.tile_start[q + 1] = S.tile_start[q];
    const uint32_t tiles = S.tile_start[nseg];
    uint32_t st_shift = 2;
    while ((1u << (2 * st_shift)) < max_tiles && st_shift < 8) ++st_shift;
    for (int q = 0; q < RS_MAXSEG; ++q)
        S.sup_start[q + 1] = S.sup_start[q] + (q < nseg ? ((S.tile_start[q + 1] - S.tile_start[q]) >> st_shift) + 1 : 0u);
    const uint32_t nsup = S.sup_start[nseg];
    const size_t pass_words = (size_t)tiles * NB + 2 * (size_t)nsup * NB, look_words = (size_t)passes * pass_words;
    const size_t off_ctr = 0, off_look = off_ctr + 64, off_keys = (off_look + look_words + 3) & ~(size_t)3;
    const size_t key_words = (n * sizeof(K) + 3) / 4, off_vals = (off_keys + key_words + 3) & ~(size_t)3;
    uint32_t *t = reinterpret_cast<uint32_t *>(ctx->scratch[7].ensure((off_vals + n + 64) * 4 + 256));
    K *tk = reinterpret_cast<K *>(t + off_keys);
    uint32_t *tv = t + off_vals;
    hipStream_t st = ctx->stream;
    constexpr size_t GH = (size_t)RS_MAXSEG * RS_GH_SEG;
    if (!ctx->sort_ghist.p) {
        ctx->sort_ghist.ensure(2 * GH);
        ctx->fill_async(ctx->sort_ghist.p, 0, 2 * GH * 4);
        ctx->sort_segs[0] = ctx->sort_segs[1] = 0;
    }
    const uint32_t cur = ctx->sort_seq & 1u, nxt = cur ^ 1u;
    uint32_t *gh = ctx->sort_ghist.p + cur * GH, *gh_next = ctx->sort_ghist.p + nxt * GH;
    const uint32_t zero_words = ctx->sort_segs[nxt] * RS_GH_SEG;
    ctx->sort_segs[nxt] = 0;
    ctx->sort_segs[cur] = (uint32_t)nseg;
    ctx->sort_seq += 1;
    ki += seg_off[0]; ko += seg_off[0]; vi += seg_off[0]; vo += seg_off[0];
    ctx->ev_begin("sort_hist", (double)n * sizeof(K));
    launch<k_rs_histogram<K, DB>, RS_THREADS>(ctx, dim3(RS_HBLOCKS * nseg), 0, ki, S, passes, gh, t + off_ctr,
                       t + off_look, look_words);
    ctx->ev_end();
    const K *src_k = ki;
    const uint32_t *src_v = vi;
    for (int p = 0; p < passes; ++p) {
        const bool to_out = ((passes - 1 - p) & 1) == 0;
        K *dst_k = to_out ? ko : tk;
        uint32_t *dst_v = to_out ? vo : tv;
        uint32_t *pass_look = t + off_look + (size_t)p * pass_words;
        ctx->ev_begin("sort_pass", (double)n * 2.0 * (sizeof(K) + 4));
        launch<k_rs_pass<K, DB, RS_IPT>, RS_THREADS>(ctx, dim3(tiles), 0, src_k, dst_k, src_v, dst_v, S, p, gh,
                           gh_next, zero_words, t + off_ctr, pass_look, reinterpret_cast<unsigned long long *>(pass_look + (size_t)tiles * NB), st_shift);
        ctx->ev_end();
        src_k = dst_k;
        src_v = dst_v;
    }
    HIP_TRY(hipGetLastError());
}

template <class K, int DB>
void radix_sort_run(plade_ctx *ctx, const K *ki, K *ko, const uint32_t *vi, uint32_t *vo, const uint32_t *seg_off, int nseg, int passes) {
    uint32_t largest = 0;
    for (int q = 0; q < nseg; ++q) largest = std::max(largest, seg_off[q + 1] - seg_off[q]);
    if (largest <= 3000000) radix_sort_run_ipt<K, DB, 8>(ctx, ki, ko, vi, vo, seg_off, nseg, passes);
    else radix_sort_run_ipt<K, DB, 16>(ctx, ki, ko, vi, vo, seg_off, nseg, passes);
}

template <class K>
void radix_sort_impl(plade_ctx *ctx, const K *ki, K *ko, const uint32_t *vi, uint32_t *vo, const uint32_t *seg_off, int nseg, int bits) {
    PLADE_REQUIRE(nseg >= 1 && nseg <= RS_MAXSEG, PLADE_EINVAL, "sort: one to sixteen segments");
    for (int q = 0; q < nseg; ++q) PLADE_REQUIRE(seg_off[q] <= seg_off[q + 1], PLADE_EINVAL, "sort: segment offsets must ascend");
    PLADE_REQUIRE((uint64_t)seg_off[nseg] - seg_off[0] < (1ull << 30), PLADE_ELIMIT, "sort: too many items");
    PLADE_REQUIRE(bits >= 1 && bits <= (int)sizeof(K) * 8, PLADE_EINVAL, "sort: bit range");
    const int p8 = (bits + 7) / 8, p9 = (bits + 8) / 9;
    static const bool no9 = getenv("PLADE_SORT_DIGIT8") != nullptr;
    if (p9 < p8 && !no9 && (p9 - 1) * 9 < (int)sizeof(K) * 8) radix_sort_run<K, 9>(ctx, ki, ko, vi, vo, seg_off, nseg, p9);
    else {
        PLADE_REQUIRE(p8 <= RS_MAXP, PLADE_EINVAL, "sort: bit range");
        radix_sort_run<K, 8>(ctx, ki, ko, vi, vo, seg_off, nseg, p8);
    }
}

}

void radix_sort_pairs_u32(plade_ctx *ctx, const uint32_t *ki, uint32_t *ko, const uint32_t *vi, uint32_t *vo, size_t n, int bits) {
    PLADE_REQUIRE(n < (1ull << 30), PLADE_ELIMIT, "sort: too many items");
    const uint32_t off[2] = {0u, (uint32_t)n};
    radix_sort_impl<uint32_t>(ctx, ki, ko, vi, vo, off, 1, bits);
}
void radix_sort_pairs_u64(plade_ctx *ctx, const uint64_t *ki, uint64_t *ko, const uint32_t *vi, uint32_t *vo, size_t n, int bits) {
    PLADE_REQUIRE(n < (1ull << 30), PLADE_ELIMIT, "sort: too many items");
    const uint32_t off[2] = {0u, (uint32_t)n};
    radix_sort_impl<uint64_t>(ctx, ki, ko, vi, vo, off, 1, bits);
}
void radix_sort_segments_u32(plade_ctx *ctx, const uint32_t *ki, uint32_t *ko, const uint32_t *vi, uint32_t *vo, const uint32_t *seg_off,
                             int nseg, int bits) {
    radix_sort_impl<uint32_t>(ctx, ki, ko, vi, vo, seg_off, nseg, bits);
}

}
```

### plade_amd/csrc/ransac.h

```cpp
#pragma once
#include "ctx.h"

namespace plade {

struct RansacParams {
    uint32_t min_support = 10000;
    float dist_rel = 0.005f, bitmap_rel = 0.02f, cos_thresh = 0.8f, overlook_p = 0.001f;
    int orient_normals = 0;
    uint64_t seed = 0;
    bool host_indices = true;
};

struct PlaneSetOut {
    std::vector<float> coef;
    std::vector<int32_t> offsets;
    std::vector<int32_t> idx;
    const uint32_t *d_idx = nullptr;
    const uint32_t *d_pos = nullptr;
    const float *m_x = nullptr, *m_y = nullptr, *m_z = nullptr;
    uint32_t n_score_passes = 0;
    double score_bytes = 0;
    uint32_t remaining = 0;
    uint32_t P() const { return (uint32_t)(coef.size() / 4); }
    void fetch_indices(hipStream_t stream) {
        const size_t m = offsets.empty() ? 0 : (size_t)offsets.back();
        if (idx.size() == m || !d_idx) return;
        idx.resize(m);
        if (m) {
            (void)hipMemcpyAsync(idx.data(), d_idx, 4 * m, hipMemcpyDeviceToHost, stream);
            (void)hipStreamSynchronize(stream);
        }
    }
};

struct RansacWork;
RansacWork *ransac_work_create();
void ransac_work_destroy(RansacWork *w);

struct ComponentOut {
    std::vector<int32_t> kept;
    float fit[7];
    double wscore;
    uint32_t err;
};
void plane_component(plade_ctx *ctx, RansacWork &W, const CloudDev &cloud, const float normal[3], const float point[3],
                     const int32_t *idx, uint32_t m, float bitmap_eps, bool closing_filter, float w_eps, ComponentOut &out);

constexpr int RANSAC_SLOTS = 2 * PLADE_GROUP_MAX;

void ransac_prepare(plade_ctx *ctx, RansacWork &W, const CloudDev *const clouds[RANSAC_SLOTS], int n_clouds);

void ransac_spacing_enqueue(plade_ctx *ctx, RansacWork &W, const int *slots, int count, int k, uint32_t samples);
bool ransac_spacing_finish(plade_ctx *ctx, RansacWork &W, int slot, float *spacing_out);

struct RansacJob {
    bool active = false;
    RansacParams rp;
    PlaneSetOut *out = nullptr;
    Stats *stats = nullptr;
};
void ransac_detect_prepared(plade_ctx *ctx, RansacWork &W, RansacJob jobs[RANSAC_SLOTS]);

void ransac_detect(plade_ctx *ctx, RansacWork &W, const CloudDev &cloud, const RansacParams &rp, PlaneSetOut &out);

void score_planes_seam(plade_ctx *ctx, RansacWork &W, const CloudDev &cloud, const int32_t *d_assigned, const float *planes,
                       uint32_t h, float eps, float cos_t, uint32_t *counts, uint32_t *idx_out, uint32_t cap);
void score_subset_seam(plade_ctx *ctx, RansacWork &W, const CloudDev &cloud, const int32_t *d_assigned, const uint32_t *sub_index,
                       uint32_t m, const float *planes, uint32_t h, float eps, float cos_t, uint32_t *counts, uint32_t *n_unassigned);

}
```

### plade_amd/csrc/ransac.hip

```cpp
#include "ransac.h"
#include "k1_point_test.h"
#include "prims.h"
#include "voxel.h"
#include <algorithm>
#include <map>
#include <memory>

namespace plade {

namespace {

constexpr uint32_t R_H = 4096;
constexpr uint32_t R_TOP = 48;
constexpr int R_B = 8;
constexpr int R_G = RANSAC_SLOTS;
constexpr uint32_t R_MAXP = 4096;
constexpr uint32_t R_MAX_ROUNDS = 4000;
constexpr int R_MIN_LEVEL = 1, R_MAX_LEVEL = 8;
constexpr int TPB = K1_TPB, PPT = K1_PPT, TILE = K1_TILE;
constexpr int HCHUNK = 64;
constexpr int FIT_COLS = 14;
constexpr uint32_t CC_MAXPIX = 1u << 20;
constexpr int CC_LDS_PIX = 4096;

// ... 54 lines not shown
    uint32_t topup;
    float eps, eps3, bitmap_eps, cos_t, overlook_p, bbmin[3], bbmax[3];
    uint64_t seed;
    uint32_t done, sampling, fresh, round, it;
    uint32_t n_remaining, sub_unassigned;
    uint32_t view_sel, view_n, view_dirty, view_next_n;
    float drawn;
    uint32_t npool, nc;
    uint32_t batch_idx[R_B];
    uint32_t pool_cnt[R_TOP];
    float4 pool_pl[R_TOP], pool_pos[R_TOP];
    uint32_t n_acc, out_off, err;
    uint32_t aj_n, aj_chain[R_B], aj_slot[R_B], aj_out[R_B];
    int32_t aj_id[R_B];
    uint32_t n_rounds, n_rescores[2], n_batches, n_accepts, n_mark_launches, n_mark_chains, n_deferred;
    uint32_t n_final[4], n_stop[5];
    float acc_coef[R_MAXP][4];
    uint32_t acc_support[R_MAXP], acc_offset[R_MAXP];
    uint32_t acc_dbg[R_MAXP];
};

struct RResult {
    uint32_t flag;
    uint32_t n_acc, out_off, err, remaining;
    uint32_t n_rounds, n_rescores, n_batches, n_accepts, n_mark_launches, n_mark_chains, pad;
    uint32_t n_final[4], n_stop[5], n_deferred, pad2[2];
    float coef[R_MAXP][4];
    uint32_t support[R_MAXP];
    uint32_t dbg[R_MAXP];
    uint32_t offset[R_MAXP];
};

struct CloudView {
    const float *x, *y, *z, *nx, *ny, *nz;
    uint32_t n;
};

struct RCloudArgs {
    CloudView cv;
    const uint32_t *codes;
    const uint32_t *cells6;
    const uint32_t *orig;
    int32_t *assigned;
    uint8_t *taken;
    const float *tile_box;
    float *view[2];
    uint32_t *view_map[2];
    uint32_t *view_cnt, *view_sup;
    const float *sub;
    const uint32_t *sub_index;
    uint32_t sub_pitch, n_sub;
    int32_t *sub_assigned;
    uint32_t sub_stride, pad0_;
    RState *st;
    RResult *res;
    float4 *hyp, *hyp_pos;
    uint32_t *hyp_counts;
    int32_t *out_idx;
    uint32_t *out_pos;
    char *fixed, *var;
    const uint32_t *list_values;
    ChainLayout L;
};
struct RKArgs {
    const RCloudArgs *c;
    uint32_t ng, topup;
    uint32_t tile_start[R_G + 1];
    uint32_t pad_;
};
typedef const RCloudArgs __attribute__((address_space(4))) RCloudArgsK;
__device__ __forceinline__ RCloudArgsK &cloud_args(const RKArgs &A, uint32_t g) { return *(RCloudArgsK *)(A.c + g); }
struct RArgs {
    RCloudArgs c[R_G];
    uint32_t ng, topup;
    uint32_t tile_start[R_G + 1];
    uint32_t pad_;
    const RCloudArgs *dev;
    operator RKArgs() const {
        RKArgs k;
        k.c = dev; k.ng = ng; k.topup = topup; k.pad_ = 0;
        for (int g = 0; g <= R_G; ++g) k.tile_start[g] = tile_start[g];
        return k;
    }
};

struct ClockScope {
    unsigned long long *p;
    __device__ explicit ClockScope(unsigned long long *q) : p(q ? q + 2 * (blockIdx.x % plade_ctx::CLK_WAYS) : nullptr) {
        if (p && threadIdx.x == 0) atomicMin(p, (unsigned long long)wall_clock64());
    }
    __device__ ~ClockScope() { if (p && (threadIdx.x & 63) == 0) atomicMax(p + 1, (unsigned long long)wall_clock64()); }
};

struct ChainPtr {
    ChainHdr *hdr;
    uint8_t *masks1; uint32_t *bc1; double *part; ChainAgg *agg;
    uint8_t *bmp, *tmp; uint32_t *label, *sizes;
    char *base; const ChainLayout __attribute__((address_space(4))) *L;
    __device__ __forceinline__ uint32_t *idxA(int k) const { return reinterpret_cast<uint32_t *>(base + L->idxA + k * L->idxA_stride); }
    __device__ __forceinline__ uint8_t *masks2(int k) const { return reinterpret_cast<uint8_t *>(base + L->masks2 + k * L->masks2_stride); }
    __device__ __forceinline__ uint32_t *bc2(int k) const { return reinterpret_cast<uint32_t *>(base + L->bc2 + k * L->bc2_stride); }
};
template <class CA>
__device__ __forceinline__ ChainPtr chain_of(const CA &C, uint32_t b) {
    ChainPtr p;
    char *base = C.var + (size_t)b * C.L.bytes, *fx = C.fixed + (size_t)b * F_BYTES;
    p.base = base; p.L = &C.L;
    p.hdr = reinterpret_cast<ChainHdr *>(fx);
    p.masks1 = reinterpret_cast<uint8_t *>(base + C.L.masks1);
    p.bc1 = reinterpret_cast<uint32_t *>(base + C.L.bc1);
    p.agg = reinterpret_cast<ChainAgg *>(fx + F_AGG);
    p.part = reinterpret_cast<double *>(base + C.L.part);
    p.bmp = reinterpret_cast<uint8_t *>(fx + F_BMP);
    p.tmp = reinterpret_cast<uint8_t *>(fx + F_TMP);
    p.label = reinterpret_cast<uint32_t *>(fx + F_LABEL);
    p.sizes = reinterpret_cast<uint32_t *>(fx + F_SIZES);
    return p;
}

ChainLayout make_layout(uint32_t n) {
    ChainLayout L;
    memset(&L, 0, sizeof(L));
    const uint64_t nb = cdiv(n, TILE), n4 = ((uint64_t)n + 7) & ~(uint64_t)3;
    L.nb = (uint32_t)nb;
    static_assert(sizeof(ChainHdr) <= F_BMP, "chain header must fit in front of the bitmap");
    uint64_t o = 0;
    auto take = [&](uint64_t bytes) { const uint64_t at = o; o = (o + bytes + 255) & ~(uint64_t)255; return at; };
    L.masks1 = take(nb * TPB);
    L.bc1 = take((nb + 4) * 4);
    L.part = take((nb + 1) * FIT_COLS * 8);
    L.idxA_stride = (n4 * 4 + 255) & ~(uint64_t)255;
    L.idxA = take(4 * L.idxA_stride);
    L.masks2_stride = (nb * TPB + 255) & ~(uint64_t)255;
    L.masks2 = take(4 * L.masks2_stride);
    L.bc2_stride = ((nb + 4) * 4 + 255) & ~(uint64_t)255;
    L.bc2 = take(4 * L.bc2_stride);
    L.bytes = o;
    return L;
}

__device__ __forceinline__ uint32_t spread3(uint32_t v) {
    v = (v | (v << 16)) & 0x030000FF;
    v = (v | (v << 8)) & 0x0300F00F;
    v = (v | (v << 4)) & 0x030C30C3;
    v = (v | (v << 2)) & 0x09249249;
    return v;
}

struct MortonIn {
    const float *x, *y, *z;
    uint32_t n;
    float mnx, mny, mnz, inv_cube;
};
struct MortonArgs { MortonIn c[R_G]; uint32_t ng; uint32_t start[R_G + 1]; };

__global__ void k_morton(const MortonArgs A, uint32_t *__restrict__ keys, uint32_t *__restrict__ vals) {
    const uint32_t t = blockIdx.x * blockDim.x + threadIdx.x;
    int g = 0;
#pragma unroll
    for (int q = 1; q < R_G; ++q) g += (q < (int)A.ng && t >= A.start[q]) ? 1 : 0;
    const MortonIn &C = A.c[g];
    const uint32_t i = t - A.start[g];
    if (i >= C.n) return;
    const uint32_t qx = min(255u, (uint32_t)max(0.f, (C.x[i] - C.mnx) * C.inv_cube * 256.f));
    const uint32_t qy = min(255u, (uint32_t)max(0.f, (C.y[i] - C.mny) * C.inv_cube * 256.f));
    const uint32_t qz = min(255u, (uint32_t)max(0.f, (C.z[i] - C.mnz) * C.inv_cube * 256.f));
    keys[t] = ((uint32_t)g << 24) | (spread3(qz) << 2) | (spread3(qy) << 1) | spread3(qx);
    vals[t] = t;
}

struct GatherOut {
    const float *aos;
    float *dst; uint32_t pitch;
    uint32_t *codes, *orig;
    int32_t *assigned;
    float *sub; uint32_t sub_pitch, n_sub, stride; uint32_t *sub_index;
    uint32_t n;
};
struct GatherArgs { GatherOut c[R_G]; uint32_t ng; uint32_t start[R_G + 1]; };

__global__ void k_gather_cloud(const GatherArgs A, const uint32_t *__restrict__ keys, const uint32_t *__restrict__ perm) {
    const uint32_t t = blockIdx.x * blockDim.x + threadIdx.x;
    int g = 0;
#pragma unroll
    for (int q = 1; q < R_G; ++q) g += (q < (int)A.ng && t >= A.start[q]) ? 1 : 0;
    const GatherOut &C = A.c[g];
    const uint32_t i = t - A.start[g];
    if (i >= C.n) return;
    const uint32_t src = perm[t] - A.start[g];
    const float2 *p = reinterpret_cast<const float2 *>(C.aos + 6 * (size_t)src);
    const float2 a = p[0], b = p[1], c = p[2];
    const size_t pitch = C.pitch;
    C.dst[i] = a.x; C.dst[pitch + i] = a.y; C.dst[2 * pitch + i] = b.x;
    C.dst[3 * pitch + i] = b.y; C.dst[4 * pitch + i] = c.x; C.dst[5 * pitch + i] = c.y;
    C.codes[i] = keys[t] & 0xffffffu;
    C.orig[i] = src;
    if (i % C.stride == 0) {
        const uint32_t s = i / C.stride;
        if (s < C.n_sub) {
            const size_t sp = C.sub_pitch;
            C.sub_index[s] = i;
            C.sub[s] = a.x; C.sub[sp + s] = a.y; C.sub[2 * sp + s] = b.x;
            C.sub[3 * sp + s] = b.y; C.sub[4 * sp + s] = c.x; C.sub[5 * sp + s] = c.y;
        }
    }
}

struct TileBoxArgs { const float *x[R_G], *y[R_G], *z[R_G]; float *box[R_G]; uint32_t n[R_G]; uint32_t ng; uint32_t tile_start[R_G + 1]; };
__global__ __launch_bounds__(K1_TPB) void k_tile_boxes(const TileBoxArgs A) {
    __shared__ float s_v[6][K1_TPB / 64];
    int g = 0;
#pragma unroll
    for (int q = 1; q < R_G; ++q) g += (q < (int)A.ng && blockIdx.x >= A.tile_start[q]) ? 1 : 0;
    const uint32_t tile = blockIdx.x - A.tile_start[g], n = A.n[g];
    float mn[3] = {INFINITY, INFINITY, INFINITY}, mx[3] = {-INFINITY, -INFINITY, -INFINITY};
    const uint32_t base = tile * K1_TILE + threadIdx.x * K1_PPT;
    for (int q = 0; q < K1_PPT; ++q)
        if (base + q < n) {
            const float v[3] = {A.x[g][base + q], A.y[g][base + q], A.z[g][base + q]};
            for (int k = 0; k < 3; ++k) { mn[k] = fminf(mn[k], v[k]); mx[k] = fmaxf(mx[k], v[k]); }
        }
    for (int k = 0; k < 3; ++k)
        for (int d = 32; d >= 1; d >>= 1) { mn[k] = fminf(mn[k], __shfl_xor(mn[k], d, 64)); mx[k] = fmaxf(mx[k], __shfl_xor(mx[k], d, 64)); }
    const int lane = threadIdx.x & 63, wave = threadIdx.x >> 6;
    if (lane == 0) for (int k = 0; k < 3; ++k) { s_v[k][wave] = mn[k]; s_v[3 + k][wave] = mx[k]; }
    __syncthreads();
    if (threadIdx.x < 6) {
        float v = s_v[threadIdx.x][0];
        for (int w = 1; w < K1_TPB / 64; ++w) v = threadIdx.x < 3 ? fminf(v, s_v[threadIdx.x][w]) : fmaxf(v, s_v[threadIdx.x][w]);
        A.box[g][8 * (size_t)tile + threadIdx.x] = v;
    }
}

__device__ __forceinline__ uint64_t mix64(uint64_t z) {
    z += 0x9E3779B97F4A7C15ull;
    z = (z ^ (z >> 30)) * 0xBF58476D1CE4E5B9ull;
    z = (z ^ (z >> 27)) * 0x94D049BB133111EBull;
    return z ^ (z >> 31);
}
struct Rng {
    uint64_t s;
    __device__ uint32_t next() { s = mix64(s); return (uint32_t)(s >> 32); }
};

__device__ __forceinline__ uint32_t lb_u32(const uint32_t *a, uint32_t n, uint32_t key) {
    uint32_t lo = 0, hi = n;
    while (lo < hi) { uint32_t mid = (lo + hi) >> 1; if (a[mid] < key) lo = mid + 1; else hi = mid; }
    return lo;
}


struct ScanSrc { const float *x, *y, *z, *nx, *ny, *nz; const uint32_t *map; uint32_t n; };
template <class CA>
__device__ __forceinline__ ScanSrc scan_src(const CA &C, const RState *S) {
    ScanSrc v;
    const uint32_t sel = C.view[0] ? S->view_sel : 0u;
    if (sel == 0u) { v.x = C.cv.x; v.y = C.cv.y; v.z = C.cv.z; v.nx = C.cv.nx; v.ny = C.cv.ny; v.nz = C.cv.nz; v.map = nullptr; v.n = C.cv.n; }
    else {
        const float *b = C.view[sel - 1];
        const size_t pitch = ((size_t)C.cv.n + 3) & ~(size_t)3;
        v.x = b; v.y = b + pitch; v.z = b + 2 * pitch; v.nx = b + 3 * pitch; v.ny = b + 4 * pitch; v.nz = b + 5 * pitch;
        v.map = C.view_map[sel - 1]; v.n = S->view_n;
    }
    return v;
}

__device__ __forceinline__ int scan_group(const RKArgs &A, uint32_t &tile) {
    int g = 0;
#pragma unroll
    for (int q = 1; q < R_G; ++q) g += (q < (int)A.ng && blockIdx.x >= A.tile_start[q]) ? 1 : 0;
    tile = blockIdx.x - A.tile_start[g];
    return g;
}

template <class CA>
__device__ __forceinline__ uint32_t scan_n(const CA &C, const RState *S) { return (C.view[0] && S->view_sel) ? S->view_n : C.cv.n; }

constexpr int CH_E = R_G * R_B;
__device__ __forceinline__ uint32_t cdiv_d(uint32_t a, uint32_t b) { return (a + b - 1) / b; }
constexpr uint32_t VGRID_WGS = 2048;
constexpr int OWN_MAX = 8;
__host__ __device__ inline uint32_t loop_grid(uint32_t nb) {
    const uint32_t a = (nb + OWN_MAX - 1) / OWN_MAX;
    return a > 1024u ? 1024u : (a < 32u ? 32u : a);
}
template <class F>
__device__ __forceinline__ uint32_t chain_grid_build(const RKArgs &A, uint32_t *s_start , uint32_t *s_carry, F need) {
    static_assert(CH_E == 128 && TPB >= 128, "one lane per chain, two wavefronts");
    const uint32_t e = threadIdx.x;
    uint32_t n = 0;
    if (e < (uint32_t)CH_E && e / R_B < A.ng) n = need(e / R_B, e % R_B);
    uint32_t incl = n;
    const int lane = threadIdx.x & 63;
#pragma unroll
    for (int d = 1; d < 64; d <<= 1) { const uint32_t o = __shfl_up(incl, d, 64); if (lane >= d) incl += o; }
    if (e == 63) *s_carry = incl;
    __syncthreads();
    if (e >= 64 && e < (uint32_t)CH_E) incl += *s_carry;
    if (e < (uint32_t)CH_E) s_start[e + 1] = incl;
    if (e == 0) s_start[0] = 0;
    __syncthreads();
    return s_start[CH_E];
}
__device__ __forceinline__ uint32_t chain_grid_find(const uint32_t *s_start, uint32_t vt) {
    uint32_t lo = 0, hi = CH_E;
    while (hi - lo > 1) { const uint32_t mid = (lo + hi) >> 1; if (s_start[mid] <= vt) lo = mid; else hi = mid; }
    return lo;
}

template <class F>
__device__ __forceinline__ uint32_t scan_grid_build(const RKArgs &A, uint32_t *s_start , F units) {
    static_assert(R_G <= 64, "one lane of the first wavefront per cloud");
    const uint32_t g = threadIdx.x;
    if (g < 64) {
        const uint32_t n = (g < (uint32_t)R_G && g < A.ng) ? units(g) : 0u;
        uint32_t incl = n;
#pragma unroll
        for (int d = 1; d < R_G; d <<= 1) { const uint32_t o = __shfl_up(incl, d, 64); if (g >= (uint32_t)d) incl += o; }
        if (g < (uint32_t)R_G) s_start[g + 1] = incl;
        if (g == 0) s_start[0] = 0;
    }
    __syncthreads();
    return s_start[R_G];
}
__device__ __forceinline__ int scan_grid_find(const uint32_t *s_start, uint32_t vt) {
    int g = 0;
#pragma unroll
    for (int q = 1; q < R_G; ++q) g += vt >= s_start[q] ? 1 : 0;
    return g;
}

__device__ __forceinline__ void hcs_axes(const float *n, float *a0, float *a1) {
    float t[3];
    if (fabsf(n[0]) < 0.015625f && fabsf(n[1]) < 0.015625f) {
        t[0] = 1.f * n[2] - 0.f * n[1]; t[1] = 0.f * n[0] - 0.f * n[2]; t[2] = 0.f * n[1] - 1.f * n[0];
    } else {
        t[0] = 0.f * n[2] - 1.f * n[1]; t[1] = 1.f * n[0] - 0.f * n[2]; t[2] = 0.f * n[1] - 0.f * n[0];
    }
    float l = t[0] * t[0];
    l += t[1] * t[1];
    l += t[2] * t[2];
    l = sqrtf(l);
    a0[0] = t[0] / l; a0[1] = t[1] / l; a0[2] = t[2] / l;
    float u[3] = {n[1] * a0[2] - n[2] * a0[1], n[2] * a0[0] - n[0] * a0[2], n[0] * a0[1] - n[1] * a0[0]};
    l = u[0] * u[0];
    l += u[1] * u[1];
    l += u[2] * u[2];
    l = sqrtf(l);
    a1[0] = u[0] / l; a1[1] = u[1] / l; a1[2] = u[2] / l;
}

__device__ __forceinline__ void plane_uv(const float *fr, float x, float y, float z, float &u, float &v) {
    const float pp[3] = {x - fr[0], y - fr[1], z - fr[2]};
    u = pp[0] * fr[3] + pp[1] * fr[4] + pp[2] * fr[5];
    v = pp[0] * fr[6] + pp[1] * fr[7] + pp[2] * fr[8];
}

__device__ void state_from_hyp(PlaneState *st, float4 hyp, float4 pos) {
    st->n[0] = hyp.x; st->n[1] = hyp.y; st->n[2] = hyp.z; st->dist = hyp.w;
    st->pos[0] = pos.x; st->pos[1] = pos.y; st->pos[2] = pos.z;
    hcs_axes(st->n, st->a0, st->a1);
    st->err = 0;
    st->converged = 0;
    st->n_list = st->n_kept = 0;
    st->wscore = 0.0;
}

struct RInitCloud {
    uint32_t active, min_support, orient, gen, topup;
    float eps, eps3, bitmap_eps, cos_t, overlook_p, bbmin[3], bbmax[3];
    uint64_t seed;
};
struct RInit { RInitCloud c[R_G]; };

__global__ __launch_bounds__(TPB) void k_r_init(const RKArgs A, const RInit I) {
    uint32_t tile;
    const int g = scan_group(A, tile);
    const RCloudArgsK &C = cloud_args(A, g);
    const RInitCloud &P = I.c[g];
    if (!P.active) {
        if (tile == 0 && threadIdx.x == 0) { C.st->active = 0; C.st->done = 1; C.st->nc = 0; C.st->aj_n = 0; C.st->npool = 0; C.st->sampling = 0; C.st->fresh = 0; }
        return;
    }
// ... 1663 lines not shown
        C.codes = s.codes.p; C.cells6 = s.cells6.p; C.orig = s.orig.p; C.assigned = nullptr; C.taken = s.taken.p; C.tile_box = s.tile_box.p;
        C.view[0] = s.view_a.p; C.view[1] = s.view_b.p; C.view_map[0] = s.view_map_a.p; C.view_map[1] = s.view_map_b.p;
        C.view_cnt = s.view_cnt.p; C.view_sup = s.view_sup.p;
        C.sub = s.sub.p; C.sub_index = s.sub_index.p; C.sub_pitch = s.sub_pitch; C.n_sub = s.n_sub;
        C.sub_assigned = s.sub_assigned.p; C.sub_stride = s.sub_stride;
        C.st = s.state.p; C.res = s.res_dev;
        C.hyp = reinterpret_cast<float4 *>(s.round_block.p);
        C.hyp_pos = C.hyp + R_H;
        C.hyp_counts = reinterpret_cast<uint32_t *>(C.hyp_pos + R_H);
        C.out_idx = s.out_idx.p;
        C.out_pos = s.out_pos.p;
        C.fixed = s.fixed.p; C.var = s.var.p;
        C.list_values = nullptr;
        memcpy(&C.L, &s.L, sizeof(ChainLayout));
    }
    for (int g = 0; g < R_G; ++g) A.tile_start[g + 1] = A.tile_start[g] + (g < ng ? A.c[g].L.nb : 0u);
    A.topup = topup ? 1u : 0u;
    return A;
}

uint64_t hash_bytes(const void *p, size_t n) {
    uint64_t h = 1469598103934665603ull;
    const unsigned char *b = static_cast<const unsigned char *>(p);
    for (size_t i = 0; i < n; ++i) { h ^= b[i]; h *= 1099511628211ull; }
    return h;
}

void args_commit(plade_ctx *ctx, RansacWork &W, RArgs &A) {
    W.args_dev.ensure(R_G);
    A.dev = W.args_dev.p;
    const uint64_t h = hash_bytes(A.c, sizeof(A.c)) | 1ull;
    if (h != W.args_hash) {
        const bool staged = ctx->h2d(W.args_dev.p, A.c, sizeof(A.c));
        if (!staged) ctx->sync();
        W.args_hash = h;
    }
}


void enqueue_iteration(plade_ctx *ctx, const RArgs &A) {
    hipStream_t st = ctx->stream;
    const uint32_t ng = A.ng;
    uint32_t tiles = 0, nb_max = 0, sub_tiles = 0;
    for (uint32_t g = 0; g < ng; ++g) {
        tiles += A.c[g].L.nb;
        nb_max = std::max(nb_max, A.c[g].L.nb);
        sub_tiles = std::max(sub_tiles, cdiv(A.c[g].n_sub, TILE));
    }
    if (!A.topup) {
        ctx->ev_begin("score_multi", 0.0);
        hipLaunchKernelGGL(k_r_rescore, dim3(std::min(VGRID_WGS, tiles)), dim3(TPB), 0, st, A, 0, ctx->ev_clock());
        ctx->ev_end();
        hipLaunchKernelGGL(k_r_select, dim3(ng), dim3(64), 0, st, A, 0);
    }
    hipLaunchKernelGGL(k_r_sample, dim3(cdiv(R_H, 256), ng), dim3(256), 0, st, A);
    hipLaunchKernelGGL(k_r_score_sub, dim3(std::min(VGRID_WGS, sub_tiles * (R_H / HCHUNK) * ng)), dim3(TPB), 0, st, A);
    hipLaunchKernelGGL(k_r_leaders, dim3(ng), dim3(1024), 0, st, A);
    ctx->ev_begin("score_multi", 0.0);
    hipLaunchKernelGGL(k_r_rescore, dim3(std::min(VGRID_WGS, tiles)), dim3(TPB), 0, st, A, 1, ctx->ev_clock());
    ctx->ev_end();
    hipLaunchKernelGGL(k_r_select, dim3(ng), dim3(64), 0, st, A, 1);
    for (int k = 0; k < 4; ++k) {
        ctx->ev_begin("score_mark", 0.0);
        hipLaunchKernelGGL(k_r_mark, dim3(std::min(VGRID_WGS, tiles)), dim3(TPB), 0, st, A, k, ctx->ev_clock());
        ctx->ev_end();
        hipLaunchKernelGGL(k_r_compact_raster, dim3(std::min(VGRID_WGS, loop_grid(nb_max) * R_B * ng)), dim3(TPB), 0, st, A, k);
        hipLaunchKernelGGL(k_r_label, dim3(R_B * ng), dim3(1024), 0, st, A, k, 1);
        hipLaunchKernelGGL(k_r_select_cc, dim3(std::min(VGRID_WGS, loop_grid(nb_max) * R_B * ng)), dim3(TPB), 0, st, A, k);
        hipLaunchKernelGGL(k_r_fit, dim3(R_B * ng), dim3(256), 0, st, A, k);
    }
    hipLaunchKernelGGL(k_r_decide, dim3(ng), dim3(DEC_T), 0, st, A);
    hipLaunchKernelGGL(k_r_assign, dim3(std::min(VGRID_WGS, loop_grid(nb_max) * R_B * ng)), dim3(TPB), 0, st, A);
    hipLaunchKernelGGL(k_view_count, dim3(std::min(VGRID_WGS, tiles)), dim3(TPB), 0, st, A);
    hipLaunchKernelGGL(k_view_compact, dim3(std::min(VGRID_WGS, tiles)), dim3(TPB), 0, st, A);
    hipLaunchKernelGGL(k_view_commit, dim3(ng), dim3(256), 0, st, A);
}

void launch_iteration(plade_ctx *ctx, RansacWork &W, const RArgs &A) {
    const bool stamped = ctx->graph_clocks();
    static const bool no_graph = getenv("PLADE_NO_GRAPH") != nullptr;
    if ((ctx->profiling() && !stamped) || no_graph) { enqueue_iteration(ctx, A); HIP_TRY(hipGetLastError()); return; }
    const uint64_t key = hash_bytes(&A, sizeof(A)) ^ (stamped ? 0x9e3779b97f4a7c15ull : 0ull);
    auto it = W.graphs.find(key);
    if (it == W.graphs.end()) {
        if (W.graphs.size() > 64) {
            for (auto &kv : W.graphs) if (kv.second) (void)hipGraphExecDestroy(kv.second);
            W.graphs.clear();
            W.graph_tags.clear();
        }
        hipGraph_t graph = nullptr;
        if (stamped) { ctx->ensure_clk(); ctx->capturing = true; ctx->cap_slot = 0; ctx->cap_tags.clear(); }
        HIP_TRY(hipStreamBeginCapture(ctx->stream, hipStreamCaptureModeThreadLocal));
        try { enqueue_iteration(ctx, A); }
        catch (...) { ctx->capturing = false; (void)hipStreamEndCapture(ctx->stream, &graph); if (graph) (void)hipGraphDestroy(graph); throw; }
        ctx->capturing = false;
        HIP_TRY(hipStreamEndCapture(ctx->stream, &graph));
        if (stamped) W.graph_tags[key] = ctx->cap_tags;
        hipGraphExec_t e = nullptr;
        HIP_TRY(hipGraphInstantiate(&e, graph, nullptr, nullptr, 0));
        (void)hipGraphDestroy(graph);
        it = W.graphs.emplace(key, e).first;
    }
    HIP_TRY(hipGraphLaunch(it->second, ctx->stream));
    if (stamped) ctx->ev_graph_launched(W.graph_tags[key]);
}

inline bool flag_done(const RResult *r, uint32_t gen) {
    const uint32_t f = *reinterpret_cast<const volatile uint32_t *>(&r->flag);
    return ((f >> 24) & 0x7fu) == (gen & 0x7fu) && (f & 0x80000000u);
}
void wait_iterations(plade_ctx *ctx, RResult *const *res, int nres, uint32_t want, uint32_t gen) {
    auto reached = [&]() {
        for (int i = 0; i < nres; ++i) {
            const uint32_t f = *reinterpret_cast<volatile uint32_t *>(&res[i]->flag);
            if (((f >> 24) & 0x7fu) != (gen & 0x7fu)) return false;
            if (!(f & 0x80000000u) && (f & 0xffffffu) < want) return false;
        }
        return true;
    };
    if (ctx->params.host_wait != 0) relax_timer_slack();
    const double cpu0 = thread_cpu_seconds();
    struct Acc { Stats &st; double c0; ~Acc() { st.add("cpu_ransac_wait_polls", thread_cpu_seconds() - c0); } } acc{ctx->stats, cpu0};
    const uint32_t query_mask = 15u;
    for (uint32_t polls = 0;; ++polls) {
        if (reached()) break;
        if ((polls & 63u) == 63u || (ctx->params.host_wait != 0 && (polls & query_mask) == query_mask)) {
            const hipError_t e = hipStreamQuery(ctx->stream);
            if (e == hipSuccess) { if (reached()) break; throw Err{PLADE_EDEVICE, "plane extraction: the device loop did not report"}; }
            if (e != hipErrorNotReady) throw Err{PLADE_EDEVICE, std::string("hipStreamQuery: ") + hipGetErrorString(e)};
        }
        if (ctx->params.host_wait != 0) poll_sleep((int)polls, ctx->in_group);
    }
    std::atomic_thread_fence(std::memory_order_acquire);
    ++ctx->wait_epoch;
}

}

void ransac_prepare(plade_ctx *ctx, RansacWork &W, const CloudDev *const clouds[RANSAC_SLOTS], int n_clouds) {
    PLADE_REQUIRE(n_clouds >= 1 && n_clouds <= R_G, PLADE_EINVAL, "ransac: too many clouds");
    W.ng = n_clouds;
    MortonArgs M;
    GatherArgs G;
    memset(&M, 0, sizeof(M));
    memset(&G, 0, sizeof(G));
    M.ng = G.ng = (uint32_t)n_clouds;
    uint64_t total = 0;
    for (int g = 0; g < n_clouds; ++g) {
        const CloudDev &c = *clouds[g];
        RansacSlot &s = W.slot[g];
        s.cloud = clouds[g];
        slot_buffers(ctx, s, c.n);
        M.start[g] = G.start[g] = (uint32_t)total;
        total += c.n;
        const float cube = std::max({c.bbmax[0] - c.bbmin[0], c.bbmax[1] - c.bbmin[1], c.bbmax[2] - c.bbmin[2], 1e-30f});
        M.c[g] = MortonIn{c.x(), c.y(), c.z(), c.n, c.bbmin[0], c.bbmin[1], c.bbmin[2], 1.f / cube};
        s.cube = cube; s.cube_inv = 1.f / cube;
        s.sorted.n = c.n;
        s.sorted.pitch = c.pitch;
        s.sorted.soa.ensure(6 * c.pitch + 4);
        for (int k = 0; k < 3; ++k) { s.sorted.bbmin[k] = c.bbmin[k]; s.sorted.bbmax[k] = c.bbmax[k]; }
        s.codes.ensure((size_t)c.n + 4); s.orig.ensure((size_t)c.n + 4);
        const uint32_t stride = std::max(1u, c.n / 16384u);
        s.n_sub = c.n ? (c.n + stride - 1) / stride : 0;
        s.sub_pitch = (s.n_sub + 3) & ~3u;
        s.sub.ensure(6 * (size_t)s.sub_pitch + 4);
        s.sub_index.ensure((size_t)s.sub_pitch + 4);
        s.sub_assigned.ensure((size_t)s.sub_pitch + 8);
        s.sub_stride = stride;
        G.c[g] = GatherOut{c.aos.p, s.sorted.soa.p, (uint32_t)c.pitch, s.codes.p, s.orig.p, nullptr, s.sub.p, s.sub_pitch, s.n_sub,
                           stride, s.sub_index.p, c.n};
    }
    PLADE_REQUIRE(total < (1ull << 31), PLADE_ELIMIT, "ransac: too many points");
    if (total == 0) return;
    for (int g = n_clouds; g < R_G; ++g) { M.c[g] = M.c[0]; G.c[g] = G.c[0]; }
    for (int g = n_clouds; g <= R_G; ++g) M.start[g] = G.start[g] = (uint32_t)total;
    W.keys_in.ensure(total); W.vals_in.ensure(total); W.keys.ensure(total); W.perm.ensure(total);
    hipLaunchKernelGGL(k_morton, dim3(cdiv(total, 256)), dim3(256), 0, ctx->stream, M, W.keys_in.p, W.vals_in.p);
    {
        uint32_t seg_off[R_G + 1];
        int nseg = 0;
        for (int g = 0; g < n_clouds; ++g) {
            if (M.start[g + 1] == M.start[g]) continue;
            seg_off[nseg] = M.start[g];
            seg_off[++nseg] = M.start[g + 1];
        }
        if (nseg) radix_sort_segments_u32(ctx, W.keys_in.p, W.keys.p, W.vals_in.p, W.perm.p, seg_off, nseg, 24);
    }
    hipLaunchKernelGGL(k_gather_cloud, dim3(cdiv(total, 256)), dim3(256), 0, ctx->stream, G, W.keys.p, W.perm.p);
    Cells6Args C6;
    memset(&C6, 0, sizeof(C6));
    for (int g = 0; g < n_clouds; ++g) {
        RansacSlot &s = W.slot[g];
        s.cells6.ensure((1u << 18) + 2);
        C6.codes[g] = s.codes.p; C6.n[g] = s.n; C6.table[g] = s.cells6.p;
    }
    hipLaunchKernelGGL(k_cells6, dim3(cdiv((1u << 18) + 1, 256), n_clouds), dim3(256), 0, ctx->stream, C6);
    TileBoxArgs TB;
    memset(&TB, 0, sizeof(TB));
    TB.ng = (uint32_t)n_clouds;
    for (int g = 0; g < R_G; ++g) {
        RansacSlot &s = W.slot[g < n_clouds ? g : 0];
        if (g < n_clouds) s.tile_box.ensure(8 * (size_t)s.L.nb + 8);
        TB.x[g] = s.sorted.x(); TB.y[g] = s.sorted.y(); TB.z[g] = s.sorted.z(); TB.box[g] = s.tile_box.p; TB.n[g] = s.n;
        TB.tile_start[g + 1] = TB.tile_start[g] + (g < n_clouds ? s.L.nb : 0u);
    }
    if (TB.tile_start[R_G]) hipLaunchKernelGGL(k_tile_boxes, dim3(TB.tile_start[R_G]), dim3(K1_TPB), 0, ctx->stream, TB);
    HIP_TRY(hipGetLastError());
}

void ransac_detect_prepared(plade_ctx *ctx, RansacWork &W, RansacJob jobs[RANSAC_SLOTS]) {
    const int ng = W.ng;
    PLADE_REQUIRE(ng >= 1, PLADE_EINVAL, "ransac: not prepared");
    Clock::time_point t0 = Clock::now();
    RArgs A = make_args(W, ng, ctx->params.ransac_topup != 0);
    args_commit(ctx, W, A);
    RInit I;
    memset(&I, 0, sizeof(I));
    RResult *res[R_G];
    int nres = 0;
    const uint32_t gen = (++W.generation) & 0x7fu;
    for (int g = 0; g < ng; ++g) {
        RansacJob &J = jobs[g];
        RansacSlot &s = W.slot[g];
        if (!J.active || s.n < 3) {
            if (J.active && J.out) {
                J.out->coef.clear(); J.out->offsets.assign(1, 0); J.out->idx.clear(); J.out->d_idx = nullptr; J.out->remaining = s.n;
                J.out->n_score_passes = 0; J.out->score_bytes = 0;
            }
            J.active = false;
            continue;
        }
        const CloudDev &c = *s.cloud;
        const float scale = std::max(c.bbmax[0] - c.bbmin[0], c.bbmax[1] - c.bbmin[1]);
        const float eps = J.rp.dist_rel * scale, bitmap_eps = J.rp.bitmap_rel * scale;
        PLADE_REQUIRE(eps > 0.f && bitmap_eps > 0.f, PLADE_EINVAL, "plane extraction: degenerate bounding box");
        RInitCloud &P = I.c[g];
        P.active = 1; P.min_support = J.rp.min_support; P.orient = J.rp.orient_normals ? 1u : 0u;
        P.eps = eps; P.eps3 = 3 * eps;
        P.bitmap_eps = bitmap_eps; P.cos_t = J.rp.cos_thresh; P.overlook_p = J.rp.overlook_p;
        for (int k = 0; k < 3; ++k) { P.bbmin[k] = c.bbmin[k]; P.bbmax[k] = c.bbmax[k]; }
        P.seed = J.rp.seed;
        P.gen = gen;
        P.topup = A.topup;
        *reinterpret_cast<volatile uint32_t *>(&s.res->flag) = 0u;
        res[nres++] = s.res;
    }
    if (nres == 0) return;
    uint32_t tiles = 0;
    for (int g = 0; g < ng; ++g) tiles += A.c[g].L.nb;
    hipLaunchKernelGGL(k_r_init, dim3(tiles), dim3(TPB), 0, ctx->stream, A, I);
    HIP_TRY(hipGetLastError());
    uint32_t iterations = 0;
    if (ctx->profiling()) {
        uint32_t seen_rescore[R_G][2] = {}, seen_mark[R_G] = {}, seen_chains[R_G] = {};
        const size_t hdr_bytes = offsetof(RState, acc_coef);
        std::vector<char> hdr(R_G * hdr_bytes);
        for (;; ++iterations) {
            const size_t ev0 = ctx->evs.size();
            launch_iteration(ctx, W, A);
            for (int g = 0; g < ng; ++g)
                if (jobs[g].active) ctx->d2h(hdr.data() + g * hdr_bytes, W.slot[g].state.p, hdr_bytes);
            ctx->sync();
            if (ctx->graph_clocks()) ctx->ev_graph_clocks(ev0);
            double rescore_bytes[2] = {0, 0}, mark_bytes = 0;
            uint32_t mark_launches = 0;
            for (int g = 0; g < ng; ++g) {
                if (!jobs[g].active) continue;
                const RState &S = *reinterpret_cast<const RState *>(hdr.data() + g * hdr_bytes);
                const double n = W.slot[g].n;
                for (int ph = 0; ph < 2; ++ph) {
                    rescore_bytes[ph] += 28.0 * n * (S.n_rescores[ph] - seen_rescore[g][ph]);
                    seen_rescore[g][ph] = S.n_rescores[ph];
                }
                mark_bytes += 28.0 * n * (S.n_mark_launches - seen_mark[g]) + 0.25 * n * (S.n_mark_chains - seen_chains[g]);
                mark_launches = std::max(mark_launches, S.n_mark_launches - seen_mark[g]);
                if (getenv("PLADE_TRACE_RANSAC"))
                    fprintf(stderr, "[ransac] it %u cloud %d: round %u sampling %u pool %u accepted %u remaining %u batches %u accepts %u (chains this it: %u) done %u\n",
                            iterations, g, S.round, S.sampling, S.npool, S.n_acc, S.n_remaining, S.n_batches, S.n_accepts,
                            S.n_mark_chains - seen_chains[g] ? (S.n_mark_chains - seen_chains[g]) : 0u, S.done);
                seen_mark[g] = S.n_mark_launches; seen_chains[g] = S.n_mark_chains;
            }
            uint32_t mk = 0, rs = 0;
            for (size_t e = ev0; e < ctx->evs.size(); ++e) {
                plade_ctx::EvRec &r = ctx->evs[e];
                if (r.tag == "score_multi") { r.bytes = rs < 2 && rescore_bytes[rs] > 0 ? rescore_bytes[rs] : -1.0; ++rs; }
                else if (r.tag == "score_mark") { r.bytes = mk < mark_launches ? mark_bytes / mark_launches : -1.0; ++mk; }
            }
            bool all = true;
            for (int i = 0; i < nres; ++i) all = all && flag_done(res[i], gen);
            if (all) break;
        }
    } else {
        const bool speculate = ctx->params.host_wait == 2;
        if (speculate) launch_iteration(ctx, W, A);
        for (;; ++iterations) {
            launch_iteration(ctx, W, A);
            wait_iterations(ctx, res, nres, iterations + 1, gen);
            bool all = true;
            for (int i = 0; i < nres; ++i) all = all && flag_done(res[i], gen);
            if (all) break;
            PLADE_REQUIRE(iterations < 100000, PLADE_EDEVICE, "plane extraction: the device loop does not end");
        }
    }
    std::atomic_thread_fence(std::memory_order_acquire);
    ctx->stats.add("ransac_iterations", iterations + 1);
    ctx->stats.add("ransac_t_detect", secs_since(t0));
    for (int g = 0; g < ng; ++g) {
        RansacJob &J = jobs[g];
        if (!J.active) continue;
        RansacSlot &s = W.slot[g];
        const RResult &R = *s.res;
        PLADE_REQUIRE(R.err != 1, PLADE_ELIMIT, "plane extraction: connected-component bitmap too large");
        PLADE_REQUIRE(R.err != 3, PLADE_ELIMIT, "plane extraction: too many shapes");
        PlaneSetOut &out = *J.out;
        if (getenv("PLADE_TRACE_RANSAC"))
            for (uint32_t i = 0; i < R.n_acc && i < 24; ++i)
                fprintf(stderr, "[ransac] cloud %d shape %u: iteration %u chain %u slot %u support %u offset %u coef %.4f %.4f %.4f %.4f\n", g, i,
                        R.dbg[i] >> 16, (R.dbg[i] >> 8) & 255u, R.dbg[i] & 255u, R.support[i], R.offset[i], R.coef[i][0], R.coef[i][1], R.coef[i][2], R.coef[i][3]);
        out.coef.clear(); out.offsets.assign(1, 0); out.idx.clear();
        for (uint32_t i = 0; i < R.n_acc; ++i) {
            if (!R.support[i]) continue;
            out.coef.insert(out.coef.end(), R.coef[i], R.coef[i] + 4);
            out.offsets.push_back((int32_t)(R.offset[i] + R.support[i]));
        }
        out.d_idx = reinterpret_cast<const uint32_t *>(s.out_idx.p);
        out.d_pos = s.out_pos.p;
        out.m_x = s.sorted.x(); out.m_y = s.sorted.y(); out.m_z = s.sorted.z();
        out.remaining = R.remaining;
        out.n_score_passes = R.n_rescores + R.n_mark_launches;
        out.score_bytes = 28.0 * s.n * (R.n_rescores + R.n_mark_launches) + 0.25 * s.n * R.n_mark_chains;
        Stats &jst = J.stats ? *J.stats : ctx->stats;
        jst.add("ransac_rounds", R.n_rounds);
        jst.add("ransac_accepts", R.n_accepts);
        jst.add("ransac_batches", R.n_batches);
        jst.add("ransac_rescore_launches", R.n_rescores);
        jst.add("ransac_mark_launches", R.n_mark_launches);
        jst.add("ransac_deferred_chains", R.n_deferred);
        for (int q = 0; q < 4; ++q) jst.add("ransac_final_slot" + std::to_string(q), R.n_final[q]);
        for (int q = 1; q < 5; ++q) jst.add("ransac_loop_stops_at" + std::to_string(q), R.n_stop[q]);
        if (J.rp.host_indices) {
            out.idx.resize(R.out_off);
            if (R.out_off) ctx->d2h(out.idx.data(), s.out_idx.p, 4 * (size_t)R.out_off);
        }
    }
    bool any_host = false;
    for (int g = 0; g < ng; ++g) any_host = any_host || (jobs[g].active && jobs[g].rp.host_indices);
    if (any_host) ctx->sync();
}

void ransac_detect(plade_ctx *ctx, RansacWork &W, const CloudDev &cloud, const RansacParams &rp, PlaneSetOut &out) {
    const CloudDev *cl[R_G] = {&cloud};
    ransac_prepare(ctx, W, cl, 1);
    RansacJob jobs[R_G];
    jobs[0].active = true; jobs[0].rp = rp; jobs[0].out = &out;
    ransac_detect_prepared(ctx, W, jobs);
}

void plane_component(plade_ctx *ctx, RansacWork &W, const CloudDev &cloud, const float normal[3], const float point[3],
                     const int32_t *idx, uint32_t m, float bitmap_eps, bool closing_filter, float w_eps, ComponentOut &out) {
    out.kept.clear();
// ... 227 lines not shown
```

Before: 775.6.

## Vectorize prepare kernels and fuse tile-box reduction into gather

The upload kernel now transposes AoS points to SoA four at a time using 16-byte loads and stores. The voxel-key and Morton kernels now handle quads per thread with vectorized reads and writes. The cloud gather is reorganized per tile so it also computes the per-tile bounding boxes, which removes the separate k_tile_boxes launch and its re-read of the sorted arrays. A diagnostic entry point that downloads the prepare outputs is added for validation. The cost is more complex tail and alignment handling in each kernel.

```diff
diff --git a/include/plade_hip.h b/include/plade_hip.h
--- a/include/plade_hip.h
+++ b/include/plade_hip.h
@@ -277,6 +277,16 @@
 int plade_selftest_readback(plade_ctx *ctx, uint32_t n_ranges, uint32_t words, uint32_t *mismatches);
 
 int plade_diag_launches(plade_ctx *ctx, uint32_t count, uint32_t blocks, uint32_t mbytes);
+typedef struct plade_diag_prepare_out {
+    float *soa, *box, *sorted;
+    uint32_t *codes, *orig;
+    float *tile_box, *sub;
+    uint32_t *sub_index;
+    float *voxels;
+    uint32_t n_voxels, reserved;
+} plade_diag_prepare_out;
+int plade_diag_prepare(plade_ctx *ctx, uint32_t count, const float *const *clouds, const uint32_t *n, float leaf,
+                       plade_diag_prepare_out *out);
 int plade_ply_read(const char *path, float **pos_nrm, uint64_t *n, char *err, size_t err_cap);
 int plade_ply_read_points(const char *path, float **pos_nrm, uint64_t *n, int32_t *has_normals, char *err, size_t err_cap);
 void plade_ply_free(float *pos_nrm);
diff --git a/plade_amd/__init__.py b/plade_amd/__init__.py
--- a/plade_amd/__init__.py
+++ b/plade_amd/__init__.py
@@ -15,7 +15,7 @@
     "plade_registration", "plade_registration_minsupport", "plade_cloud_upload", "plade_cloud_free",
     "plade_registration_dev", "plade_dump_get", "plade_stats_get", "plade_kernel_time", "plade_plane_component",
     "plade_sort_pairs", "plade_host_pin", "plade_host_unpin", "plade_score_planes_subset", "plade_registration_next", "plade_cluster_transforms", "plade_device_synchronize", "plade_selftest_readback",
-    "plade_registration_pairs", "plade_registration_pairs_dev", "plade_pair_ctx", "plade_set_candidate_shard", "plade_diag_launches", "plade_diag_cluster_order", "plade_diag_line_solver_host", "plade_sort_segments",
+    "plade_registration_pairs", "plade_registration_pairs_dev", "plade_pair_ctx", "plade_set_candidate_shard", "plade_diag_launches", "plade_diag_prepare", "plade_diag_cluster_order", "plade_diag_line_solver_host", "plade_sort_segments",
     "plade_closest_points", "plade_lines_meet", "plade_ply_read", "plade_ply_free",
     "plade_device_count", "plade_comm_unique_id", "plade_comm_create", "plade_comm_all_gather", "plade_comm_destroy", "plade_comm_last_error",
     "plade_set_candidate_shard_comm",
@@ -99,6 +99,12 @@
 class SmoothSummary(C.Structure):
     _fields_ = [("n", C.c_uint64), ("fitted", C.c_uint64), ("rms", C.c_double), ("max", C.c_double), ("max_count", C.c_uint32),
                 ("reserved", C.c_uint32)]
+
+
+class DiagPrepareOut(C.Structure):
+    _fields_ = [("soa", C.c_void_p), ("box", C.c_void_p), ("sorted", C.c_void_p), ("codes", C.c_void_p), ("orig", C.c_void_p),
+                ("tile_box", C.c_void_p), ("sub", C.c_void_p), ("sub_index", C.c_void_p), ("voxels", C.c_void_p),
+                ("n_voxels", C.c_uint32), ("reserved", C.c_uint32)]
 
 
 PLADE_OUTLIER_STATISTICAL, PLADE_OUTLIER_RADIUS = 0, 1
@@ -155,6 +161,7 @@
     sig("plade_closest_points", argtypes=[p, i32, p, p, p, p, u32, p, p, p, p])
     sig("plade_lines_meet", argtypes=[p, i32, p, p, p, p, u32, p, p])
     sig("plade_diag_launches", argtypes=[p, u32, u32, u32])
+    sig("plade_diag_prepare", argtypes=[p, u32, p, p, f, p])
     sig("plade_diag_cluster_order", argtypes=[p, u32, i32, i32, p])
     sig("plade_diag_line_solver_host", argtypes=[i32, p, p, p, p, u32, p, p, p])
     sig("plade_ply_read", argtypes=[C.c_char_p, C.POINTER(C.POINTER(C.c_float)), C.POINTER(u64), C.c_char_p, C.c_size_t])
@@ -728,6 +735,28 @@
     def diag_launches(self, count, blocks=1, mbytes=0):
         self._check(self.L.plade_diag_launches(self.h, int(count), int(blocks), int(mbytes)))
 
+    def diag_prepare(self, clouds, leaf):
+        cl = [_f32(c).reshape(-1, 6) for c in clouds]
+        count = len(cl)
+        ptrs = (C.c_void_p * count)(*[c.ctypes.data if len(c) else None for c in cl])
+        ns = (C.c_uint32 * count)(*[len(c) for c in cl])
+        outs = (DiagPrepareOut * count)()
+        res = []
+        for i, c in enumerate(cl):
+            n = len(c)
+            stride = max(1, n // 16384)
+            n_sub = (n + stride - 1) // stride
+            r = {"soa": np.zeros((6, n), np.float32), "box": np.zeros(6, np.float32), "sorted": np.zeros((6, n), np.float32),
+                 "codes": np.zeros(n, np.uint32), "orig": np.zeros(n, np.uint32), "tile_box": np.zeros(((n + 1023) // 1024, 6), np.float32),
+                 "sub": np.zeros((6, n_sub), np.float32), "sub_index": np.zeros(n_sub, np.uint32), "voxels": np.zeros((n, 3), np.float32)}
+            for k, a in r.items():
+                setattr(outs[i], k, a.ctypes.data)
+            res.append(r)
+        self._check(self.L.plade_diag_prepare(self.h, count, ptrs, ns, float(leaf), outs))
+        for i, r in enumerate(res):
+            r["voxels"] = r["voxels"][: outs[i].n_voxels].copy()
+        return res
+
     def _pair_handle(self, index):
         h = self.L.plade_pair_ctx(self.h, int(index))
         if not h:
diff --git a/plade_amd/csrc/api.hip b/plade_amd/csrc/api.hip
--- a/plade_amd/csrc/api.hip
+++ b/plade_amd/csrc/api.hip
@@ -9,6 +9,7 @@
 #include "pipeline.h"
 #include "ransac.h"
 #include "smooth.h"
+#include "voxel.h"
 #include "gicp.h"
 
 using namespace plade;
@@ -200,6 +201,52 @@
     });
 }
 
+extern "C" int plade_diag_prepare(plade_ctx *ctx, uint32_t count, const float *const *clouds, const uint32_t *n, float leaf,
+                                  plade_diag_prepare_out *out) {
+    return guarded(ctx, [&]() -> int {
+        PLADE_REQUIRE(count >= 1 && count <= (uint32_t)RANSAC_SLOTS && clouds && n && out && leaf > 0.f, PLADE_EINVAL, "plade_diag_prepare: bad argument");
+        for (uint32_t c = 0; c < count; ++c) PLADE_REQUIRE(clouds[c] || !n[c], PLADE_EINVAL, "plade_diag_prepare: null cloud");
+        std::vector<CloudDev> dev(count);
+        std::vector<VoxelWork> vox(count);
+        std::vector<DBuf<float>> vox_soa(count);
+        CloudDev *up[RANSAC_SLOTS];
+        const CloudDev *cl[RANSAC_SLOTS] = {};
+        for (uint32_t c = 0; c < count; ++c) { up[c] = &dev[c]; cl[c] = &dev[c]; }
+        cloud_upload_many(ctx, (int)count, clouds, n, up);
+        if (!ctx->ransac_work) ctx->ransac_work = ransac_work_create();
+        ransac_prepare(ctx, *ctx->ransac_work, cl, (int)count);
+        VoxBatchItem items[RANSAC_SLOTS];
+        int which[RANSAC_SLOTS], ni = 0;
+        for (uint32_t c = 0; c < count; ++c) {
+            out[c].n_voxels = 0;
+            if (!n[c]) continue;
+            const CloudDev &d = dev[c];
+            VoxBatchItem &it = items[ni];
+            it.aos = d.aos.p; it.sx = d.x(); it.sy = d.y(); it.sz = d.z(); it.n = d.n; it.leaf = leaf;
+            for (int k = 0; k < 3; ++k) { it.bbmin[k] = d.bbmin[k]; it.bbmax[k] = d.bbmax[k]; }
+            it.work = &vox[c]; it.out_soa = vox_soa[c].ensure(3 * (size_t)d.n + 4);
+            which[ni++] = (int)c;
+        }
+        const bool vox_ok = !ni || voxel_whole_batch(ctx, ctx->vox_batch, ni, items);
+        ctx->sync();
+        PLADE_REQUIRE(vox_ok, PLADE_ELIMIT, "plade_diag_prepare: the voxel grids do not fit the batch");
+        for (uint32_t c = 0; c < count; ++c) {
+            const CloudDev &d = dev[c];
+            plade_diag_prepare_out &o = out[c];
+            if (!d.n) continue;
+            if (o.soa) HIP_TRY(hipMemcpy2D(o.soa, (size_t)d.n * 4, d.soa.p, d.pitch * 4, (size_t)d.n * 4, 6, hipMemcpyDeviceToHost));
+            if (o.box) for (int k = 0; k < 3; ++k) { o.box[k] = d.bbmin[k]; o.box[3 + k] = d.bbmax[k]; }
+            ransac_prepared_download(ctx, *ctx->ransac_work, (int)c, o.sorted, o.codes, o.orig, o.sub, o.sub_index, o.tile_box);
+        }
+        for (int q = 0; q < ni; ++q) {
+            plade_diag_prepare_out &o = out[which[q]];
+            HIP_TRY(hipMemcpy(&o.n_voxels, vox[which[q]].count.p, 4, hipMemcpyDeviceToHost));
+            if (o.voxels) HIP_TRY(hipMemcpy(o.voxels, vox[which[q]].out_xyz.p, (size_t)o.n_voxels * 12, hipMemcpyDeviceToHost));
+        }
+        return PLADE_OK;
+    });
+}
+
 extern "C" int plade_diag_cluster_order(const float *sizes, uint32_t n, int32_t mode, int32_t depth_limit, int32_t *order) {
     if ((n && (!sizes || !order)) || mode < 0 || mode > 3) return PLADE_EINVAL;
     try {
diff --git a/plade_amd/csrc/cloud.hip b/plade_amd/csrc/cloud.hip
--- a/plade_amd/csrc/cloud.hip
+++ b/plade_amd/csrc/cloud.hip
@@ -17,6 +17,14 @@
     uint32_t n[2 * PLADE_GROUP_MAX];
     uint32_t pitch[2 * PLADE_GROUP_MAX];
 };
+struct Quad6 { float4 r[6]; };
+__device__ __forceinline__ Quad6 load_quad6(const float *__restrict__ aos, uint32_t q) {
+    const float4 *p = reinterpret_cast<const float4 *>(aos) + 6 * (size_t)q;
+    Quad6 v;
+#pragma unroll
+    for (int k = 0; k < 6; ++k) v.r[k] = p[k];
+    return v;
+}
 __global__ __launch_bounds__(256) void k_finish_uploads(const FinishArgs A, int *__restrict__ slots ) {
     __shared__ float s_lds[6][8];
     const int c = blockIdx.y;
@@ -27,17 +35,43 @@
     int *out = slots + 8 * c;
     float mn[3] = {INFINITY, INFINITY, INFINITY}, mx[3] = {-INFINITY, -INFINITY, -INFINITY};
     bool bad = false;
-    for (uint32_t i = blockIdx.x * blockDim.x + threadIdx.x; i < n; i += gridDim.x * blockDim.x) {
-        const float2 *p = reinterpret_cast<const float2 *>(aos + 6 * (size_t)i);
-        const float2 a = p[0], b = p[1], d = p[2];
-        soa[i] = a.x; soa[pitch + i] = a.y; soa[2 * pitch + i] = b.x;
-        soa[3 * pitch + i] = b.y; soa[4 * pitch + i] = d.x; soa[5 * pitch + i] = d.y;
-        const float v[3] = {a.x, a.y, b.x};
+    auto box = [&](float x, float y, float z) {
+        const float v[3] = {x, y, z};
         for (int k = 0; k < 3; ++k) {
             bad = bad || !(fabsf(v[k]) <= FLT_MAX);
             mn[k] = fminf(mn[k], v[k]);
             mx[k] = fmaxf(mx[k], v[k]);
         }
+    };
+    auto put_quad = [&](uint32_t q, const Quad6 &v) {
+        const float4 *r = v.r;
+        float4 *d = reinterpret_cast<float4 *>(soa) + q;
+        const size_t p4 = pitch >> 2;
+        d[0] = make_float4(r[0].x, r[1].z, r[3].x, r[4].z);
+        d[p4] = make_float4(r[0].y, r[1].w, r[3].y, r[4].w);
+        d[2 * p4] = make_float4(r[0].z, r[2].x, r[3].z, r[5].x);
+        d[3 * p4] = make_float4(r[0].w, r[2].y, r[3].w, r[5].y);
+        d[4 * p4] = make_float4(r[1].x, r[2].z, r[4].x, r[5].z);
+        d[5 * p4] = make_float4(r[1].y, r[2].w, r[4].y, r[5].w);
+        box(r[0].x, r[0].y, r[0].z); box(r[1].z, r[1].w, r[2].x); box(r[3].x, r[3].y, r[3].z); box(r[4].z, r[4].w, r[5].x);
+    };
+    const uint32_t lane0 = blockIdx.x * blockDim.x + threadIdx.x, step = gridDim.x * blockDim.x;
+    const bool aligned = ((reinterpret_cast<uintptr_t>(aos) | reinterpret_cast<uintptr_t>(soa)) & 15u) == 0;
+    const uint32_t nq = aligned ? n >> 2 : 0u;
+    for (uint32_t q = lane0; q < nq; q += 2 * step) {
+        const bool two = q + step < nq;
+        const Quad6 a = load_quad6(aos, q);
+        Quad6 b;
+        if (two) b = load_quad6(aos, q + step);
+        put_quad(q, a);
+        if (two) put_quad(q + step, b);
+    }
+    for (uint32_t i = 4 * nq + lane0; i < n; i += step) {
+        const float2 *p = reinterpret_cast<const float2 *>(aos + 6 * (size_t)i);
+        const float2 a = p[0], b = p[1], d = p[2];
+        soa[i] = a.x; soa[pitch + i] = a.y; soa[2 * pitch + i] = b.x;
+        soa[3 * pitch + i] = b.y; soa[4 * pitch + i] = d.x; soa[5 * pitch + i] = d.y;
+        box(a.x, a.y, b.x);
     }
     if (bad) out[6] = 1;
     block_minmax_commit<3>(mn, mx, out, s_lds);
diff --git a/plade_amd/csrc/k_voxel.hip b/plade_amd/csrc/k_voxel.hip
--- a/plade_amd/csrc/k_voxel.hip
+++ b/plade_amd/csrc/k_voxel.hip
@@ -269,6 +269,7 @@
     uint32_t start[VB_MAX + 1];
     uint32_t tile_start[VB_MAX + 1];
     uint32_t cblk_start[VB_MAX + 1];
+    uint32_t quad_start[VB_MAX + 1];
     uint32_t total;
 };
 __device__ __forceinline__ uint32_t vb_find(const uint32_t *start, uint32_t ncl, uint32_t v) {
@@ -278,25 +279,66 @@
     return g;
 }
 
-__global__ void k_vb_keys(const VBArgs A, uint32_t *__restrict__ keys, uint32_t *__restrict__ vals) {
-    const uint32_t t = blockIdx.x * blockDim.x + threadIdx.x;
-    if (t >= A.total) return;
-    const uint32_t g = vb_find(A.start, A.ncl, t);
+__global__ __launch_bounds__(256) void k_vb_keys(const VBArgs A, uint32_t *__restrict__ keys, uint32_t *__restrict__ vals) {
+    const uint32_t lq = blockIdx.x * blockDim.x + threadIdx.x;
+    if (lq >= A.quad_start[VB_MAX]) return;
+    const uint32_t g = vb_find(A.quad_start, A.ncl, lq);
     const VBCloud &C = A.c[g];
-    const uint32_t i = t - A.start[g];
-    const uint32_t p = C.items ? C.items[i] : i;
-    const float x = C.sx[p], y = C.sy[p], z = C.sz[p];
-    const uint32_t lx = (uint32_t)((int)floorf(x * C.inv) - C.lminx);
-    const uint32_t ly = (uint32_t)((int)floorf(y * C.inv) - C.lminy);
-    const uint32_t lz = (uint32_t)((int)floorf(z * C.inv) - C.lminz);
-    uint32_t grp = 0;
+    const uint32_t i0 = 4 * (lq - A.quad_start[g]), n = C.n;
+    if (i0 >= n) return;
+    const uint32_t t0 = A.start[g] + i0;
+    const bool full = i0 + 3 < n;
+    uint32_t p[4];
+    if (C.items && full && (reinterpret_cast<uintptr_t>(C.items) & 15u) == 0) {
+        const uint4 v = *reinterpret_cast<const uint4 *>(C.items + i0);
+        p[0] = v.x; p[1] = v.y; p[2] = v.z; p[3] = v.w;
+    } else {
+#pragma unroll
+        for (int q = 0; q < 4; ++q) { const uint32_t i = min(i0 + q, n - 1); p[q] = C.items ? C.items[i] : i; }
+    }
+    float x[4], y[4], z[4];
+    const bool in16 = ((reinterpret_cast<uintptr_t>(C.sx) | reinterpret_cast<uintptr_t>(C.sy) | reinterpret_cast<uintptr_t>(C.sz)) & 15u) == 0;
+    if (!C.items && full && in16) {
+        const float4 vx = *reinterpret_cast<const float4 *>(C.sx + i0), vy = *reinterpret_cast<const float4 *>(C.sy + i0),
+                     vz = *reinterpret_cast<const float4 *>(C.sz + i0);
+        x[0] = vx.x; x[1] = vx.y; x[2] = vx.z; x[3] = vx.w;
+        y[0] = vy.x; y[1] = vy.y; y[2] = vy.z; y[3] = vy.w;
+        z[0] = vz.x; z[1] = vz.y; z[2] = vz.z; z[3] = vz.w;
+    } else {
+#pragma unroll
+        for (int q = 0; q < 4; ++q) { x[q] = C.sx[p[q]]; y[q] = C.sy[p[q]]; z[q] = C.sz[p[q]]; }
+    }
+    uint32_t grp[4] = {0, 0, 0, 0};
     if (C.offs) {
-        uint32_t lo = 0, hi = C.P;
-        while (lo < hi) { const uint32_t mid = (lo + hi + 1) >> 1; if (C.offs[mid] <= i) lo = mid; else hi = mid - 1; }
-        grp = lo;
-    }
-    keys[t] = (grp << C.gshift) | (lz << (C.bx + C.by)) | (ly << C.bx) | lx;
-    vals[t] = i;
+        uint32_t hi[4] = {C.P, C.P, C.P, C.P};
+        bool go = C.P > 0;
+        while (go) {
+            go = false;
+#pragma unroll
+            for (int q = 0; q < 4; ++q) {
+                const uint32_t mid = (grp[q] + hi[q] + 1) >> 1;
+                const bool le = C.offs[mid] <= min(i0 + q, n - 1);
+                if (grp[q] < hi[q]) { if (le) grp[q] = mid; else hi[q] = mid - 1; }
+                go = go || grp[q] < hi[q];
+            }
+        }
+    }
+    uint32_t k[4];
+#pragma unroll
+    for (int q = 0; q < 4; ++q) {
+        const uint32_t lx = (uint32_t)((int)floorf(x[q] * C.inv) - C.lminx);
+        const uint32_t ly = (uint32_t)((int)floorf(y[q] * C.inv) - C.lminy);
+        const uint32_t lz = (uint32_t)((int)floorf(z[q] * C.inv) - C.lminz);
+        k[q] = (grp[q] << C.gshift) | (lz << (C.bx + C.by)) | (ly << C.bx) | lx;
+    }
+    if (full && (t0 & 3u) == 0) {
+        *reinterpret_cast<uint4 *>(keys + t0) = make_uint4(k[0], k[1], k[2], k[3]);
+        *reinterpret_cast<uint4 *>(vals + t0) = make_uint4(i0, i0 + 1, i0 + 2, i0 + 3);
+    } else {
+#pragma unroll
+        for (int q = 0; q < 4; ++q)
+            if (i0 + q < n) { keys[t0 + q] = k[q]; vals[t0 + q] = i0 + q; }
+    }
 }
 
 __global__ __launch_bounds__(VR_T) void k_vb_runs(const VBArgs A, const uint32_t *__restrict__ keys_all, const uint32_t *__restrict__ vals_all,
@@ -472,10 +514,11 @@
         A.start[g + 1] = A.start[g] + it.n;
         A.tile_start[g + 1] = A.tile_start[g] + cdiv(it.n, VR_TILE);
         A.cblk_start[g + 1] = A.cblk_start[g] + cdiv(it.n, 128);
+        A.quad_start[g + 1] = A.quad_start[g] + cdiv(it.n, 4);
         total += it.n;
     }
     if (total >= (1ull << 30)) return false;
-    for (int g = count; g < VB_MAX; ++g) { A.c[g] = A.c[0]; A.start[g + 1] = A.start[g]; A.tile_start[g + 1] = A.tile_start[g]; A.cblk_start[g + 1] = A.cblk_start[g]; }
+    for (int g = count; g < VB_MAX; ++g) { A.c[g] = A.c[0]; A.start[g + 1] = A.start[g]; A.tile_start[g + 1] = A.tile_start[g]; A.cblk_start[g + 1] = A.cblk_start[g]; A.quad_start[g + 1] = A.quad_start[g]; }
     A.total = (uint32_t)total;
     B.keys.ensure(total); B.keys2.ensure(total); B.vals.ensure(total); B.vals2.ensure(total);
     B.heads.ensure(total + VB_MAX + 1);
@@ -495,7 +538,7 @@
         const bool staged = ctx->h2d(B.offs.p, h.data(), 4 * n_offs);
         if (!staged) ctx->sync();
     }
-    hipLaunchKernelGGL(k_vb_keys, dim3(cdiv(total, 256)), dim3(256), 0, st, A, B.keys.p, B.vals.p);
+    hipLaunchKernelGGL(k_vb_keys, dim3(cdiv(A.quad_start[VB_MAX], 256)), dim3(256), 0, st, A, B.keys.p, B.vals.p);
     radix_sort_segments_u32(ctx, B.keys.p, B.keys2.p, B.vals.p, B.vals2.p, A.start, count, max_bits);
     const uint32_t tiles = A.tile_start[count];
     const ScanTicket t = scan_ticket(ctx, (size_t)tiles * VR_TILE, VR_TILE);
diff --git a/plade_amd/csrc/radix_sort.hip b/plade_amd/csrc/radix_sort.hip
--- a/plade_amd/csrc/radix_sort.hip
+++ b/plade_amd/csrc/radix_sort.hip
@@ -267,9 +267,8 @@
 
 template <class K, int DB>
 void radix_sort_run(plade_ctx *ctx, const K *ki, K *ko, const uint32_t *vi, uint32_t *vo, const uint32_t *seg_off, int nseg, int passes) {
-    uint32_t largest = 0;
-    for (int q = 0; q < nseg; ++q) largest = std::max(largest, seg_off[q + 1] - seg_off[q]);
-    if (largest <= 3000000) radix_sort_run_ipt<K, DB, 8>(ctx, ki, ko, vi, vo, seg_off, nseg, passes);
+    const uint32_t total = seg_off[nseg] - seg_off[0];
+    if (total <= 3000000) radix_sort_run_ipt<K, DB, 8>(ctx, ki, ko, vi, vo, seg_off, nseg, passes);
     else radix_sort_run_ipt<K, DB, 16>(ctx, ki, ko, vi, vo, seg_off, nseg, passes);
 }
 
diff --git a/plade_amd/csrc/ransac.h b/plade_amd/csrc/ransac.h
--- a/plade_amd/csrc/ransac.h
+++ b/plade_amd/csrc/ransac.h
@@ -49,6 +49,8 @@
 constexpr int RANSAC_SLOTS = 2 * PLADE_GROUP_MAX;
 
 void ransac_prepare(plade_ctx *ctx, RansacWork &W, const CloudDev *const clouds[RANSAC_SLOTS], int n_clouds);
+void ransac_prepared_download(plade_ctx *ctx, RansacWork &W, int g, float *sorted, uint32_t *codes, uint32_t *orig, float *sub,
+                              uint32_t *sub_index, float *tile_box);
 
 void ransac_spacing_enqueue(plade_ctx *ctx, RansacWork &W, const int *slots, int count, int k, uint32_t samples);
 bool ransac_spacing_finish(plade_ctx *ctx, RansacWork &W, int slot, float *spacing_out);
diff --git a/plade_amd/csrc/ransac.hip b/plade_amd/csrc/ransac.hip
--- a/plade_amd/csrc/ransac.hip
+++ b/plade_amd/csrc/ransac.hip
@@ -230,72 +230,133 @@
     uint32_t n;
     float mnx, mny, mnz, inv_cube;
 };
-struct MortonArgs { MortonIn c[R_G]; uint32_t ng; uint32_t start[R_G + 1]; };
-
-__global__ void k_morton(const MortonArgs A, uint32_t *__restrict__ keys, uint32_t *__restrict__ vals) {
-    const uint32_t t = blockIdx.x * blockDim.x + threadIdx.x;
+struct MortonArgs { MortonIn c[R_G]; uint32_t ng; uint32_t start[R_G + 1]; uint32_t quad_start[R_G + 1]; };
+
+__device__ __forceinline__ uint32_t morton_axis(float v, float mn, float inv_cube) { return min(255u, (uint32_t)max(0.f, (v - mn) * inv_cube * 256.f)); }
+
+__global__ __launch_bounds__(256) void k_morton(const MortonArgs A, uint32_t *__restrict__ keys, uint32_t *__restrict__ vals) {
+    const uint32_t lq = blockIdx.x * blockDim.x + threadIdx.x;
+    if (lq >= A.quad_start[R_G]) return;
     int g = 0;
 #pragma unroll
-    for (int q = 1; q < R_G; ++q) g += (q < (int)A.ng && t >= A.start[q]) ? 1 : 0;
+    for (int q = 1; q < R_G; ++q) g += (q < (int)A.ng && lq >= A.quad_start[q]) ? 1 : 0;
     const MortonIn &C = A.c[g];
-    const uint32_t i = t - A.start[g];
-    if (i >= C.n) return;
-    const uint32_t qx = min(255u, (uint32_t)max(0.f, (C.x[i] - C.mnx) * C.inv_cube * 256.f));
-    const uint32_t qy = min(255u, (uint32_t)max(0.f, (C.y[i] - C.mny) * C.inv_cube * 256.f));
-    const uint32_t qz = min(255u, (uint32_t)max(0.f, (C.z[i] - C.mnz) * C.inv_cube * 256.f));
-    keys[t] = ((uint32_t)g << 24) | (spread3(qz) << 2) | (spread3(qy) << 1) | spread3(qx);
-    vals[t] = t;
+    const uint32_t i0 = 4 * (lq - A.quad_start[g]), n = C.n;
+    if (i0 >= n) return;
+    const uint32_t t0 = A.start[g] + i0;
+    const bool full = i0 + 3 < n;
+    const bool in16 = ((reinterpret_cast<uintptr_t>(C.x) | reinterpret_cast<uintptr_t>(C.y) | reinterpret_cast<uintptr_t>(C.z)) & 15u) == 0;
+    float x[4], y[4], z[4];
+    if (full && in16) {
+        const float4 vx = *reinterpret_cast<const float4 *>(C.x + i0), vy = *reinterpret_cast<const float4 *>(C.y + i0),
+                     vz = *reinterpret_cast<const float4 *>(C.z + i0);
+        x[0] = vx.x; x[1] = vx.y; x[2] = vx.z; x[3] = vx.w;
+        y[0] = vy.x; y[1] = vy.y; y[2] = vy.z; y[3] = vy.w;
+        z[0] = vz.x; z[1] = vz.y; z[2] = vz.z; z[3] = vz.w;
+    } else {
+#pragma unroll
+        for (int q = 0; q < 4; ++q) {
+            const uint32_t i = min(i0 + q, n - 1);
+            x[q] = C.x[i]; y[q] = C.y[i]; z[q] = C.z[i];
+        }
+    }
+    uint32_t k[4];
+#pragma unroll
+    for (int q = 0; q < 4; ++q)
+        k[q] = ((uint32_t)g << 24) | (spread3(morton_axis(z[q], C.mnz, C.inv_cube)) << 2) | (spread3(morton_axis(y[q], C.mny, C.inv_cube)) << 1) |
+               spread3(morton_axis(x[q], C.mnx, C.inv_cube));
+    if (full && (t0 & 3u) == 0) {
+        *reinterpret_cast<uint4 *>(keys + t0) = make_uint4(k[0], k[1], k[2], k[3]);
+        *reinterpret_cast<uint4 *>(vals + t0) = make_uint4(t0, t0 + 1, t0 + 2, t0 + 3);
+    } else {
+#pragma unroll
+        for (int q = 0; q < 4; ++q)
+            if (i0 + q < n) { keys[t0 + q] = k[q]; vals[t0 + q] = t0 + q; }
+    }
 }
 
 struct GatherOut {
     const float *aos;
     float *dst; uint32_t pitch;
     uint32_t *codes, *orig;
-    int32_t *assigned;
+    float *box;
     float *sub; uint32_t sub_pitch, n_sub, stride; uint32_t *sub_index;
     uint32_t n;
 };
-struct GatherArgs { GatherOut c[R_G]; uint32_t ng; uint32_t start[R_G + 1]; };
-
-__global__ void k_gather_cloud(const GatherArgs A, const uint32_t *__restrict__ keys, const uint32_t *__restrict__ perm) {
-    const uint32_t t = blockIdx.x * blockDim.x + threadIdx.x;
-    int g = 0;
-#pragma unroll
-    for (int q = 1; q < R_G; ++q) g += (q < (int)A.ng && t >= A.start[q]) ? 1 : 0;
-    const GatherOut &C = A.c[g];
-    const uint32_t i = t - A.start[g];
-    if (i >= C.n) return;
-    const uint32_t src = perm[t] - A.start[g];
-    const float2 *p = reinterpret_cast<const float2 *>(C.aos + 6 * (size_t)src);
-    const float2 a = p[0], b = p[1], c = p[2];
-    const size_t pitch = C.pitch;
-    C.dst[i] = a.x; C.dst[pitch + i] = a.y; C.dst[2 * pitch + i] = b.x;
-    C.dst[3 * pitch + i] = b.y; C.dst[4 * pitch + i] = c.x; C.dst[5 * pitch + i] = c.y;
-    C.codes[i] = keys[t] & 0xffffffu;
-    C.orig[i] = src;
-    if (i % C.stride == 0) {
-        const uint32_t s = i / C.stride;
-        if (s < C.n_sub) {
-            const size_t sp = C.sub_pitch;
-            C.sub_index[s] = i;
-            C.sub[s] = a.x; C.sub[sp + s] = a.y; C.sub[2 * sp + s] = b.x;
-            C.sub[3 * sp + s] = b.y; C.sub[4 * sp + s] = c.x; C.sub[5 * sp + s] = c.y;
-        }
-    }
-}
-
-struct TileBoxArgs { const float *x[R_G], *y[R_G], *z[R_G]; float *box[R_G]; uint32_t n[R_G]; uint32_t ng; uint32_t tile_start[R_G + 1]; };
-__global__ __launch_bounds__(K1_TPB) void k_tile_boxes(const TileBoxArgs A) {
+struct GatherArgs { GatherOut c[R_G]; uint32_t ng; uint32_t start[R_G + 1]; uint32_t tile_start[R_G + 1]; };
+
+__global__ __launch_bounds__(K1_TPB) void k_gather_tiles(const GatherArgs A, const uint32_t *__restrict__ keys, const uint32_t *__restrict__ perm) {
+    static_assert(K1_PPT == 4, "a lane owns one 16-byte quad of every array");
     __shared__ float s_v[6][K1_TPB / 64];
     int g = 0;
 #pragma unroll
     for (int q = 1; q < R_G; ++q) g += (q < (int)A.ng && blockIdx.x >= A.tile_start[q]) ? 1 : 0;
-    const uint32_t tile = blockIdx.x - A.tile_start[g], n = A.n[g];
+    const GatherOut &C = A.c[g];
+    const uint32_t tile = blockIdx.x - A.tile_start[g], n = C.n, first = A.start[g];
+    const uint32_t base = tile * K1_TILE + threadIdx.x * K1_PPT;
+    const uint32_t t0 = first + base;
+    const bool full = base + 3 < n;
+    uint32_t src[4] = {0, 0, 0, 0}, key[4] = {0, 0, 0, 0};
+    if (full && (t0 & 3u) == 0) {
+        const uint4 p = *reinterpret_cast<const uint4 *>(perm + t0), k = *reinterpret_cast<const uint4 *>(keys + t0);
+        src[0] = p.x; src[1] = p.y; src[2] = p.z; src[3] = p.w;
+        key[0] = k.x; key[1] = k.y; key[2] = k.z; key[3] = k.w;
+    } else {
+#pragma unroll
+        for (int q = 0; q < 4; ++q)
+            if (base + q < n) { src[q] = perm[t0 + q]; key[q] = keys[t0 + q]; }
+    }
+    float2 a[4], b[4], c[4];
+#pragma unroll
+    for (int q = 0; q < 4; ++q) {
+        src[q] = base + q < n ? src[q] - first : 0u;
+        a[q] = b[q] = c[q] = make_float2(0.f, 0.f);
+        if (base + q < n) {
+            const float2 *p = reinterpret_cast<const float2 *>(C.aos + 6 * (size_t)src[q]);
+            a[q] = p[0]; b[q] = p[1]; c[q] = p[2];
+        }
+    }
+    const size_t pitch = C.pitch;
+    if (full) {
+        float4 *d = reinterpret_cast<float4 *>(C.dst + base);
+        const size_t p4 = pitch >> 2;
+        d[0] = make_float4(a[0].x, a[1].x, a[2].x, a[3].x);
+        d[p4] = make_float4(a[0].y, a[1].y, a[2].y, a[3].y);
+        d[2 * p4] = make_float4(b[0].x, b[1].x, b[2].x, b[3].x);
+        d[3 * p4] = make_float4(b[0].y, b[1].y, b[2].y, b[3].y);
+        d[4 * p4] = make_float4(c[0].x, c[1].x, c[2].x, c[3].x);
+        d[5 * p4] = make_float4(c[0].y, c[1].y, c[2].y, c[3].y);
+        *reinterpret_cast<uint4 *>(C.codes + base) = make_uint4(key[0] & 0xffffffu, key[1] & 0xffffffu, key[2] & 0xffffffu, key[3] & 0xffffffu);
+        *reinterpret_cast<uint4 *>(C.orig + base) = make_uint4(src[0], src[1], src[2], src[3]);
+    } else {
+#pragma unroll
+        for (int q = 0; q < 4; ++q)
+            if (base + q < n) {
+                const uint32_t i = base + q;
+                C.dst[i] = a[q].x; C.dst[pitch + i] = a[q].y; C.dst[2 * pitch + i] = b[q].x;
+                C.dst[3 * pitch + i] = b[q].y; C.dst[4 * pitch + i] = c[q].x; C.dst[5 * pitch + i] = c[q].y;
+                C.codes[i] = key[q] & 0xffffffu;
+                C.orig[i] = src[q];
+            }
+    }
+    if (base < n) {
+        const uint32_t stride = C.stride;
+        uint32_t s = base / stride, r = base - s * stride;
+        const size_t sp = C.sub_pitch;
+#pragma unroll
+        for (int q = 0; q < 4; ++q) {
+            if (r == 0 && base + q < n && s < C.n_sub) {
+                C.sub_index[s] = base + q;
+                C.sub[s] = a[q].x; C.sub[sp + s] = a[q].y; C.sub[2 * sp + s] = b[q].x;
+                C.sub[3 * sp + s] = b[q].y; C.sub[4 * sp + s] = c[q].x; C.sub[5 * sp + s] = c[q].y;
+            }
+            if (++r == stride) { r = 0; ++s; }
+        }
+    }
     float mn[3] = {INFINITY, INFINITY, INFINITY}, mx[3] = {-INFINITY, -INFINITY, -INFINITY};
-    const uint32_t base = tile * K1_TILE + threadIdx.x * K1_PPT;
     for (int q = 0; q < K1_PPT; ++q)
         if (base + q < n) {
-            const float v[3] = {A.x[g][base + q], A.y[g][base + q], A.z[g][base + q]};
+            const float v[3] = {a[q].x, a[q].y, b[q].x};
             for (int k = 0; k < 3; ++k) { mn[k] = fminf(mn[k], v[k]); mx[k] = fmaxf(mx[k], v[k]); }
         }
     for (int k = 0; k < 3; ++k)
@@ -306,7 +367,7 @@
     if (threadIdx.x < 6) {
         float v = s_v[threadIdx.x][0];
         for (int w = 1; w < K1_TPB / 64; ++w) v = threadIdx.x < 3 ? fminf(v, s_v[threadIdx.x][w]) : fmaxf(v, s_v[threadIdx.x][w]);
-        A.box[g][8 * (size_t)tile + threadIdx.x] = v;
+        C.box[8 * (size_t)tile + threadIdx.x] = v;
     }
 }
 
@@ -2276,6 +2337,9 @@
         s.cloud = clouds[g];
         slot_buffers(ctx, s, c.n);
         M.start[g] = G.start[g] = (uint32_t)total;
+        M.quad_start[g + 1] = M.quad_start[g] + cdiv(c.n, 4);
+        G.tile_start[g + 1] = G.tile_start[g] + s.L.nb;
+        s.tile_box.ensure(8 * (size_t)s.L.nb + 8);
         total += c.n;
         const float cube = std::max({c.bbmax[0] - c.bbmin[0], c.bbmax[1] - c.bbmin[1], c.bbmax[2] - c.bbmin[2], 1e-30f});
         M.c[g] = MortonIn{c.x(), c.y(), c.z(), c.n, c.bbmin[0], c.bbmin[1], c.bbmin[2], 1.f / cube};
@@ -2292,15 +2356,16 @@
         s.sub_index.ensure((size_t)s.sub_pitch + 4);
         s.sub_assigned.ensure((size_t)s.sub_pitch + 8);
         s.sub_stride = stride;
-        G.c[g] = GatherOut{c.aos.p, s.sorted.soa.p, (uint32_t)c.pitch, s.codes.p, s.orig.p, nullptr, s.sub.p, s.sub_pitch, s.n_sub,
+        G.c[g] = GatherOut{c.aos.p, s.sorted.soa.p, (uint32_t)c.pitch, s.codes.p, s.orig.p, s.tile_box.p, s.sub.p, s.sub_pitch, s.n_sub,
                            stride, s.sub_index.p, c.n};
     }
     PLADE_REQUIRE(total < (1ull << 31), PLADE_ELIMIT, "ransac: too many points");
     if (total == 0) return;
     for (int g = n_clouds; g < R_G; ++g) { M.c[g] = M.c[0]; G.c[g] = G.c[0]; }
     for (int g = n_clouds; g <= R_G; ++g) M.start[g] = G.start[g] = (uint32_t)total;
+    for (int g = n_clouds; g < R_G; ++g) { M.quad_start[g + 1] = M.quad_start[g]; G.tile_start[g + 1] = G.tile_start[g]; }
     W.keys_in.ensure(total); W.vals_in.ensure(total); W.keys.ensure(total); W.perm.ensure(total);
-    hipLaunchKernelGGL(k_morton, dim3(cdiv(total, 256)), dim3(256), 0, ctx->stream, M, W.keys_in.p, W.vals_in.p);
+    hipLaunchKernelGGL(k_morton, dim3(cdiv(M.quad_start[R_G], 256)), dim3(256), 0, ctx->stream, M, W.keys_in.p, W.vals_in.p);
     {
         uint32_t seg_off[R_G + 1];
         int nseg = 0;
@@ -2311,7 +2376,7 @@
         }
         if (nseg) radix_sort_segments_u32(ctx, W.keys_in.p, W.keys.p, W.vals_in.p, W.perm.p, seg_off, nseg, 24);
     }
-    hipLaunchKernelGGL(k_gather_cloud, dim3(cdiv(total, 256)), dim3(256), 0, ctx->stream, G, W.keys.p, W.perm.p);
+    hipLaunchKernelGGL(k_gather_tiles, dim3(G.tile_start[R_G]), dim3(K1_TPB), 0, ctx->stream, G, W.keys.p, W.perm.p);
     Cells6Args C6;
     memset(&C6, 0, sizeof(C6));
     for (int g = 0; g < n_clouds; ++g) {
@@ -2320,17 +2385,22 @@
         C6.codes[g] = s.codes.p; C6.n[g] = s.n; C6.table[g] = s.cells6.p;
     }
     hipLaunchKernelGGL(k_cells6, dim3(cdiv((1u << 18) + 1, 256), n_clouds), dim3(256), 0, ctx->stream, C6);
-    TileBoxArgs TB;
-    memset(&TB, 0, sizeof(TB));
-    TB.ng = (uint32_t)n_clouds;
-    for (int g = 0; g < R_G; ++g) {
-        RansacSlot &s = W.slot[g < n_clouds ? g : 0];
-        if (g < n_clouds) s.tile_box.ensure(8 * (size_t)s.L.nb + 8);
-        TB.x[g] = s.sorted.x(); TB.y[g] = s.sorted.y(); TB.z[g] = s.sorted.z(); TB.box[g] = s.tile_box.p; TB.n[g] = s.n;
-        TB.tile_start[g + 1] = TB.tile_start[g] + (g < n_clouds ? s.L.nb : 0u);
-    }
-    if (TB.tile_start[R_G]) hipLaunchKernelGGL(k_tile_boxes, dim3(TB.tile_start[R_G]), dim3(K1_TPB), 0, ctx->stream, TB);
     HIP_TRY(hipGetLastError());
+}
+
+void ransac_prepared_download(plade_ctx *ctx, RansacWork &W, int g, float *sorted, uint32_t *codes, uint32_t *orig, float *sub,
+                              uint32_t *sub_index, float *tile_box) {
+    PLADE_REQUIRE(g >= 0 && g < W.ng, PLADE_EINVAL, "ransac: no such prepared cloud");
+    ctx->sync();
+    const RansacSlot &s = W.slot[g];
+    const size_t n = s.n;
+    if (!n) return;
+    if (sorted) HIP_TRY(hipMemcpy2D(sorted, n * 4, s.sorted.soa.p, s.sorted.pitch * 4, n * 4, 6, hipMemcpyDeviceToHost));
+    if (codes) HIP_TRY(hipMemcpy(codes, s.codes.p, n * 4, hipMemcpyDeviceToHost));
+    if (orig) HIP_TRY(hipMemcpy(orig, s.orig.p, n * 4, hipMemcpyDeviceToHost));
+    if (sub) HIP_TRY(hipMemcpy2D(sub, (size_t)s.n_sub * 4, s.sub.p, (size_t)s.sub_pitch * 4, (size_t)s.n_sub * 4, 6, hipMemcpyDeviceToHost));
+    if (sub_index) HIP_TRY(hipMemcpy(sub_index, s.sub_index.p, (size_t)s.n_sub * 4, hipMemcpyDeviceToHost));
+    if (tile_box) HIP_TRY(hipMemcpy2D(tile_box, 24, s.tile_box.p, 32, 24, s.L.nb, hipMemcpyDeviceToHost));
 }
 
 void ransac_detect_prepared(plade_ctx *ctx, RansacWork &W, RansacJob jobs[RANSAC_SLOTS]) {
```

After: 800.4, median of 5. 1.03x the previous value.
